# lyd405121/ti-raytrace

Measured on AMD Instinct MI355X. Metric: Mrays/s (primary+secondary) at 1024² 100k-tri, 1/2/4/8 GPU + HBM GB/s, higher is better.
Workload: dtype f32

## Files before the change

ti_raytrace_amd/csrc/tirt_api.hip:

```cpp
#include "tirt_internal.h"
#include "tirt_spectral.h"
#include <stddef.h>
#include <algorithm>
#include <mutex>
#include <string.h>

namespace tirt {

static thread_local std::string g_error;
void set_error(const std::string &msg) { g_error = msg; }

SceneView scene_view(const tirt_ctx *c)
{
    SceneView s;
    s.vertex = c->vertex.as<float>(); s.primitive = c->primitive.as<int>(); s.material = c->material.as<float>();
    s.shape = c->shape.as<float>(); s.light = c->light.as<int>(); s.env = c->env.as<int>();
    s.mat_lrgb = c->mat_lrgb.as<float>(); s.shade_rec = c->shade_rec.as<float4>(); s.light_rec = c->light_rec.as<float4>();
    s.tex = c->tex_count > 0 ? c->tex.as<int>() : nullptr;
    s.n = c->n; s.light_count = c->light_count; s.env_w = c->env_w; s.env_h = c->env_h; s.env_power = c->env_power;
    return s;
}
BvhView bvh_view(const tirt_ctx *c)
{
    BvhView b;
// ... 314 lines not shown
        float suc; v3 r = refract_(V(a[0], a[1], a[2]), V(a[3], a[4], a[5]), a[6], suc); o[0] = r.x; o[1] = r.y; o[2] = r.z; o[3] = suc;
    } else if (which == 12) {
        o[0] = schlick(a[0], a[1]);
    } else if (which == 13) {
        o[0] = gtr2(a[0], a[1]);
    } else if (which == 14) {
        o[0] = smithg_ggx(a[0], a[1]);
    } else if (which == 15) {
        o[0] = schlick_fresnel(a[0]);
    } else if (which == 16) {
        float fb; v3 r = glass_sample_lambda(V(a[0], a[1], a[2]), V(a[3], a[4], a[5]), a[6], a[7], fb); o[0] = r.x; o[1] = r.y; o[2] = r.z; o[3] = fb;
    } else if (which == 17) {
        CameraView cv; for (int k = 0; k < 12; k++) cv.view_inv[k] = a[k];
        cv.eye[0] = cv.eye[1] = cv.eye[2] = 0.0f; cv.fx = a[16]; cv.fy = a[17]; cv.cx = a[18]; cv.cy = a[19];
        v3 r = camera_ray_direction(cv, (int)a[20], (int)a[21], a[22], a[23]); o[0] = r.x; o[1] = r.y; o[2] = r.z;
    } else if (which == 18) {
        const RayCtx r = make_ray(V(a[0], a[1], a[2]), V(a[3], a[4], a[5])); float tn;
        const int full = slabs(r, a[6], a[7], a[8], a[9], a[10], a[11], tn);
        o[0] = (float)full;
        o[1] = ray_has_parallel_axis(r) ? (float)full : (float)slabs_fast(r, a[6], a[7], a[8], a[9], a[10], a[11], tn);
    }
}

__global__ void k_kat_shade_tables(SceneView s, int which, float *out, int n)
{
    const int i = blockIdx.x * blockDim.x + threadIdx.x;
    if (i >= n) return;
    if (which == 0) {
        float *o = out + (size_t)i * 4;
        v3 g = V(0.0f, 0.0f, 0.0f);
        if (s.primitive[(size_t)i * PRI_VEC] == PRIMITIVE_TRI) g = hit_attributes(s, g, V(0.0f, 0.0f, 1.0f), i, 1.0f, 0.25f, 0.25f).gnor;
        o[0] = g.x; o[1] = g.y; o[2] = g.z; o[3] = get_prim_area(s, i);
    } else {
        float *o = out + (size_t)i * 5;
        const int light_prim = s.light[i];
        const float *lm = s.material + (size_t)s.primitive[(size_t)light_prim * PRI_VEC + 2] * MAT_VEC;
        const float light_area = get_prim_area(s, light_prim);
        float light_choice_pdf = 1.0f / ((float)s.light_count * light_area);
        (void)light_shape_visible(s, light_prim, V(0.0f, 0.0f, 1.0f), V(0.0f, 0.0f, 1.0f), 1.0f, light_choice_pdf);
        o[0] = light_area; o[1] = light_choice_pdf; o[2] = lm[2]; o[3] = lm[3]; o[4] = lm[4];
    }
}
TD void kat_nee_store(float *o, v3 pos, v3 nor, v3 em, float area, float pdf, float dist)
{ o[0] = pos.x; o[1] = pos.y; o[2] = pos.z; o[3] = nor.x; o[4] = nor.y; o[5] = nor.z; o[6] = em.x; o[7] = em.y; o[8] = em.z; o[9] = area; o[10] = pdf; o[11] = dist; }
__global__ void k_kat_light_sample(SceneView s, const float *in, float *out, int n)
{
    const int i = blockIdx.x * blockDim.x + threadIdx.x;
    if (i >= n) return;
    const float *a = in + (size_t)i * 6;
    float *o = out + (size_t)i * 24;
    int lidx = (int)(a[0] * (float)s.light_count);
    if (lidx >= s.light_count) lidx = s.light_count - 1;
    if (lidx < 0) lidx = 0;
    const v3 p = V(a[3], a[4], a[5]);
    {
        const int light_prim = s.light[lidx];
        v3 light_pos, light_normal;
        get_prim_random_point_normal(s, light_prim, a[1], a[2], light_pos, light_normal);
        const float *lm = s.material + (size_t)s.primitive[(size_t)light_prim * PRI_VEC + 2] * MAT_VEC;
        const float light_area = get_prim_area(s, light_prim);
        float light_choice_pdf = 1.0f / ((float)s.light_count * light_area);
        light_normal = normalized(light_normal);
        v3 light_dir = p - light_pos;
        const float light_dist = norm(light_dir);
        light_dir = light_dir / light_dist;
        const v3 em = V(lm[2], lm[3], lm[4]) * light_shape_visible(s, light_prim, light_dir, light_normal, light_dist, light_choice_pdf);
        kat_nee_store(o, light_pos, light_normal, em, light_area, light_choice_pdf, light_dist);
    }
    {
        v3 light_pos, light_normal;
        const LightRec lr = light_sample_rec(s.light_rec, lidx, a[1], a[2], light_pos, light_normal);
        light_normal = normalized(light_normal);
        v3 light_dir = p - light_pos;
        const float light_dist = norm(light_dir);
        light_dir = light_dir / light_dist;
        const v3 em = lr.emission * light_shape_visible_rec(lr, light_dir, light_normal, light_dist);
        kat_nee_store(o + 12, light_pos, light_normal, em, lr.area, lr.choice_pdf, light_dist);
    }
}

TD uint32_t mg_mix(uint32_t x) { x ^= x >> 16; x *= 0x7feb352du; x ^= x >> 15; x *= 0x846ca68bu; x ^= x >> 16; return x; }
__global__ __launch_bounds__(256) void k_micro_gather(const float4 *rec, uint32_t nrec, int iters, float *out)
{
    uint32_t s = mg_mix(blockIdx.x * 256 + threadIdx.x + 1);
    float acc = 0.0f;
    for (int it = 0; it < iters; it++) {
        s = mg_mix(s + it);
        const uint32_t idx = (uint32_t)(((unsigned long long)s * nrec) >> 32);
        const float4 *p = rec + (size_t)idx * 4;
        const float4 a = p[0], b = p[1], c = p[2], d = p[3];
        acc += a.x + b.y + c.z + d.w;
    }
    out[blockIdx.x * 256 + threadIdx.x] = acc;
}

static int upload(DevBuf &b, const void *src, size_t bytes, hipStream_t st)
{
    if (b.ensure(bytes)) return TIRT_ERR_HIP;
    if (bytes) TIRT_HIP(hipMemcpyAsync(b.p, src, bytes, hipMemcpyHostToDevice, st));
    return 0;
}

static void drain_render_events(tirt_ctx *c)
{
    for (auto &pr : c->ev_pool) {
        float ms = 0.0f;
        if (hipEventElapsedTime(&ms, pr.first, pr.second) == hipSuccess) c->ms_render += ms;
        (void)hipEventDestroy(pr.first); (void)hipEventDestroy(pr.second);
    }
    c->ev_pool.clear();
}

__global__ void k_kat_texture(const int *tex, const float *in, int in_stride, float *out, int out_stride, int n)
{
    const int i = blockIdx.x * blockDim.x + threadIdx.x;
    if (i >= n) return;
    const float *a = in + (size_t)i * in_stride;
    float *o = out + (size_t)i * out_stride;
    const v3 c = tex_albedo(tex, __float_as_int(a[0]), a[1], a[2]);
    const v3 l = srgb_to_lrgb(c);
    o[0] = c.x; o[1] = c.y; o[2] = c.z; o[3] = l.x; o[4] = l.y; o[5] = l.z;
}

__global__ void k_kat_material_maps(SceneView sc, const float *in, int in_stride, float *out, int out_stride, int n)
{
    const int i = blockIdx.x * blockDim.x + threadIdx.x;
    if (i >= n) return;
    const float *a = in + (size_t)i * in_stride;
    float *o = out + (size_t)i * out_stride;
    const int prim = __float_as_int(a[0]);
    const int *pr = sc.primitive + (size_t)prim * PRI_VEC;
    const float *m = sc.material + (size_t)pr[2] * MAT_VEC;
    v3 uv = V(0.0f, 0.0f, 0.0f), N = uv;
    if (pr[0] == PRIMITIVE_TRI) {
        const int vi = pr[1];
        const float u = a[1], v = a[2], ba = 1.0f - u - v;
        uv = (vtx_uv(sc, vi) * ba + vtx_uv(sc, vi + 1) * u) + vtx_uv(sc, vi + 2) * v;
        N = normalized((vtx_nor(sc, vi) * ba + vtx_nor(sc, vi + 1) * u) + vtx_nor(sc, vi + 2) * v);
    }
    float rough = m[6], metal = m[5];
    const int ri = material_map(m, 7), mi = material_map(m, 8);
    if (ri >= 0) rough = tex_roughness(sc.tex, ri, uv.x, uv.y);
    if (mi >= 0) metal = tex_metallic(sc.tex, mi, uv.x, uv.y);
    const v3 Np = shading_normal_rows(sc, m, prim, uv, N);
    o[0] = uv.x; o[1] = uv.y; o[2] = rough; o[3] = metal; o[4] = Np.x; o[5] = Np.y; o[6] = Np.z; o[7] = 0.0f;
}

}

using namespace tirt;

extern "C" {

const char *tirt_last_error(void) { return g_error.c_str(); }
int tirt_version(void) { return 101; }

int tirt_device_count(int *out)
{
    TIRT_REQUIRE(out, "tirt_device_count: null out");
    TIRT_HIP(hipGetDeviceCount(out));
    return TIRT_OK;
}

int tirt_create(int device_id, tirt_ctx **out)
{
    TIRT_REQUIRE(out, "tirt_create: null out");
    int ndev = 0;
    TIRT_HIP(hipGetDeviceCount(&ndev));
    if (device_id < 0 || device_id >= ndev) { set_error("tirt_create: device " + std::to_string(device_id) + " of " + std::to_string(ndev)); return TIRT_ERR_ARG; }
    TIRT_HIP(hipSetDevice(device_id));
    tirt_ctx *c = new tirt_ctx();
    c->device = device_id;
    TIRT_HIP(hipStreamCreateWithFlags(&c->stream, hipStreamNonBlocking));
    TIRT_HIP(hipEventCreate(&c->ev0));
    TIRT_HIP(hipEventCreate(&c->ev1));
    TIRT_HIP(hipEventCreateWithFlags(&c->ev_main, hipEventDisableTiming));
    for (Lane &L : c->lanes) {
        TIRT_HIP(hipStreamCreateWithFlags(&L.stream, hipStreamNonBlocking));
        TIRT_HIP(hipEventCreateWithFlags(&L.film_done, hipEventDisableTiming));
        TIRT_HIP(hipEventCreateWithFlags(&L.aov_done, hipEventDisableTiming));
    }
    memset(&c->cam, 0, sizeof(c->cam));
    int optin = 0;
    if (hipDeviceGetAttribute(&optin, hipDeviceAttributeSharedMemPerBlockOptin, device_id) == hipSuccess && optin > 0) c->lds_optin = (size_t)optin;
    else { (void)hipGetLastError(); if (hipDeviceGetAttribute(&optin, hipDeviceAttributeMaxSharedMemoryPerBlock, device_id) == hipSuccess && optin > 0) c->lds_optin = (size_t)optin; }
    int cus = 0;
    if (hipDeviceGetAttribute(&cus, hipDeviceAttributeMultiprocessorCount, device_id) == hipSuccess && cus > 0) {
        const int g = 5 * cus < 2048 ? 5 * cus : 2048;
        c->tr_grid = g; c->tr_grid_alone = g; c->cu_count = cus;
    } else (void)hipGetLastError();
    *out = c;
    return TIRT_OK;
}

void tirt_destroy(tirt_ctx *c)
{
    if (!c) return;
    if (c->comm) { tirt_ctx *one[1] = {c}; (void)tirt_comm_destroy(one, 1); }
    (void)hipSetDevice(c->device);
    (void)sync_all(c);
    drain_render_events(c);
    DevBuf *bufs[] = {&c->vertex, &c->primitive, &c->material, &c->shape, &c->light, &c->env, &c->tex, &c->mat_lrgb, &c->shade_rec, &c->light_rec, &c->morton_unsorted, &c->keys_a,
                      &c->keys_b, &c->vals_a, &c->vals_b, &c->hist, &c->morton_sorted, &c->bvh_node, &c->compact, &c->parent,
                      &c->flag, &c->subtree, &c->build_status, &c->leaf_compact, &c->wnode, &c->tri, &c->prim_slot, &c->cnode, &c->cparent, &c->csize, &c->wide_queue, &c->wide_levels, &c->sah_compact, &c->sah_csize, &c->sah_parent, &c->wide_dp, &c->sah_box, &c->sah_idx, &c->sah_tasks, &c->sah_counts, &c->hdr, &c->rgb, &c->aov, &c->mom, &c->mom_cnt, &c->pixset, &c->pixset_tmp, &c->tp_mem, &c->mv_rec, &c->mv_snap, &c->dn_mem, &c->dn_out,
                      &c->counters_mem, &c->spill, &c->trace_stage, &c->debug_mem, &c->query_mem, &c->dyn_mem, &c->dev_counters, &c->bdpt_px, &c->timeline, &c->pvb_set[0].count, &c->pvb_set[0].cand, &c->pvb_set[0].bound, &c->pvb_set[1].count, &c->pvb_set[1].cand, &c->pvb_set[1].bound, &c->pvb_stat, &c->pvb_tmp};
    for (DevBuf *b : bufs) b->release();
    for (auto &bl : c->bd) {
        DevBuf *bb[] = {&bl.items, &bl.state, &bl.rays, &bl.hits, &bl.qidx, &bl.ctr, &bl.rad};
        for (DevBuf *b : bb) b->release();
        if (bl.delta_done) (void)hipEventDestroy(bl.delta_done);
        if (bl.film_done) (void)hipEventDestroy(bl.film_done);
    }
    for (Lane &L : c->lanes) {
        DevBuf *lb[] = {&L.path_mem, &L.counters_mem, &L.spill};
        for (DevBuf *b : lb) b->release();
        if (L.film_done) (void)hipEventDestroy(L.film_done);
        if (L.aov_done) (void)hipEventDestroy(L.aov_done);
        if (L.stream) (void)hipStreamDestroy(L.stream);
    }
    c->spec_mem.release(); c->spec_dev.release();
    if (c->spec_view) { delete (SpecView *)c->spec_view; c->spec_view = nullptr; }
    if (c->ev_main) (void)hipEventDestroy(c->ev_main);
    if (c->query_ev_in) (void)hipEventDestroy(c->query_ev_in);
    if (c->query_ev_out) (void)hipEventDestroy(c->query_ev_out);
    (void)hipEventDestroy(c->ev0); (void)hipEventDestroy(c->ev1);
    (void)hipStreamDestroy(c->stream);
    delete c;
}

#define AFTER_RENDER(c)                                                            \
    do { if ((c)->last_film) TIRT_HIP(hipStreamWaitEvent((c)->stream, (c)->last_film, 0)); } while (0)

#define AFTER_AOV(c)                                                               \
    do { if ((c)->last_aov) TIRT_HIP(hipStreamWaitEvent((c)->stream, (c)->last_aov, 0)); } while (0)

#define CTX_NOFLUSH(c)                                                             \
    TIRT_REQUIRE(c, "null context");                                               \
    TIRT_HIP(hipSetDevice((c)->device))
#define CTX(c)                                                                     \
    CTX_NOFLUSH(c);                                                                \
    do { if (int rc__ = flush_pending(c)) return rc__; } while (0)

int tirt_sync(tirt_ctx *c)
{
    CTX(c);
    if (sync_all(c)) return TIRT_ERR_HIP;
    TIRT_HIP(hipGetLastError());
    return TIRT_OK;
}

int tirt_set_option(tirt_ctx *c, const char *name, double value)
{
    CTX(c);
    TIRT_REQUIRE(name, "tirt_set_option: null name");
    if (!strcmp(name, "time_kernels")) { c->time_kernels = value != 0.0; return TIRT_OK; }
    if (!strcmp(name, "overlap_lanes")) { TIRT_REQUIRE(value >= 1.0 && value <= (double)TIRT_MAX_LANES, "overlap_lanes: 1..8"); if (sync_all(c)) return TIRT_ERR_HIP; c->n_lanes = (int)value; return TIRT_OK; }
#ifndef TIRT_EXPERIMENTS
    if (!strcmp(name, "wide_collapse")) {
        TIRT_REQUIRE(value == 0.0, "this option is an experiment (cost-optimal wide collapse): build with -DTIRT_EXPERIMENTS (make experiments)");
        return TIRT_OK;
    }
#endif
    if (!strcmp(name, "split_lone_batch")) { TIRT_REQUIRE(value >= 0.0 && value <= 8.0, "split_lone_batch: 0 (off) or the number of parts, 2..8"); c->split_lone = (int)value; return TIRT_OK; }
    if (!strcmp(name, "wide_collapse")) { TIRT_REQUIRE(value == 0.0 || value == 1.0, "wide_collapse: 0 (greedy) or 1 (cost-optimal)"); c->wide_dp_on = (int)value; return TIRT_OK; }
    if (!strcmp(name, "traversal_tree")) {
        TIRT_REQUIRE(value == 0.0 || value == 1.0, "traversal_tree: 0 (the reference's LBVH) or 1 (binned SAH)");
        c->use_sah = (int)value; return TIRT_OK;
    }
    if (!strcmp(name, "plan_batches")) { TIRT_REQUIRE(value >= 0.0 && value <= 64.0, "plan_batches: 0 (automatic) .. 64"); if (flush_pending(c)) return TIRT_ERR_HIP; c->plan_nb = (int)value; return TIRT_OK; }
    if (!strcmp(name, "plan_lanes")) { TIRT_REQUIRE(value >= 0.0 && value <= TIRT_MAX_LANES, "plan_lanes: 0 (automatic) .. the lane count"); if (flush_pending(c)) return TIRT_ERR_HIP; c->plan_lanes = (int)value; return TIRT_OK; }
    if (!strcmp(name, "job_frames")) { TIRT_REQUIRE(value >= 0.0 && value <= 1.0e9, "job_frames out of range"); c->job_frames = (long)value; return TIRT_OK; }
    if (!strcmp(name, "merge_paths")) { TIRT_REQUIRE(value >= 0.0 && value <= 1.0e9, "merge_paths out of range"); c->merge_paths = (size_t)value; c->merge_user = true; return TIRT_OK; }
    if (!strcmp(name, "batch_paths")) {
        TIRT_REQUIRE(value >= 1.0 && value <= 1.0e9, "tirt_set_option: batch_paths out of range");
        c->batch_paths = (size_t)value; c->batch_user = true; return TIRT_OK;
    }
    if (!strcmp(name, "trace_lds_depth")) {
        TIRT_REQUIRE(value >= 12 && value <= 64, "trace_lds_depth: 12..64");
        TIRT_REQUIRE(trace_lds_bytes((int)value) <= c->lds_optin, "trace_lds_depth: stacks + tree top exceed the LDS a block can have on this device");
        c->tr_lds_depth = (int)value; return TIRT_OK;
    }
    if (!strcmp(name, "bdpt_stack_size")) { TIRT_REQUIRE(value >= 16 && value <= 4096, "bdpt_stack_size: 16..4096"); c->bdpt_stack = (int)value; return TIRT_OK; }
    if (!strcmp(name, "trace_timeline")) { c->timeline_arm = (int)value; c->timeline_waves = 0; return TIRT_OK; }
    if (!strcmp(name, "trace_refill_min")) { TIRT_REQUIRE(value >= 1 && value <= 64, "trace_refill_min: 1..64"); c->tr_refill_min = (int)value; return TIRT_OK; }
    if (!strcmp(name, "trace_node_min")) { TIRT_REQUIRE(value >= 1 && value <= 64, "trace_node_min: 1..64"); c->tr_node_min = (int)value; return TIRT_OK; }
    if (!strcmp(name, "bdpt_bounded")) { c->bdpt_bounded = value != 0.0 ? 1 : 0; return TIRT_OK; }
    if (!strcmp(name, "bdpt_state_fill")) { TIRT_REQUIRE(value == 0.0 || value == 1.0 || value == 2.0, "bdpt_state_fill: 0 (none), 1 (zeros) or 2 (poison)"); c->bdpt_state_fill = (int)value; return TIRT_OK; }
    if (!strcmp(name, "primary_beams")) { TIRT_REQUIRE(value == 0.0 || value == 1.0, "primary_beams: 0 or 1"); if (flush_pending(c)) return TIRT_ERR_HIP; c->primary_beams = (int)value; return TIRT_OK; }
    if (!strcmp(name, "primary_beams_rebuild")) { if (flush_pending(c)) return TIRT_ERR_HIP; c->pvb_valid = false; return TIRT_OK; }
    if (!strcmp(name, "primary_beams_diag")) { if (flush_pending(c)) return TIRT_ERR_HIP; c->pvb_diag = value != 0.0; return TIRT_OK; }
    if (!strcmp(name, "primary_beams_min_frames")) { TIRT_REQUIRE(value >= 1.0 && value <= 1.0e6, "primary_beams_min_frames out of range"); if (flush_pending(c)) return TIRT_ERR_HIP; c->primary_beams_min_frames = (int)value; return TIRT_OK; }
    if (!strcmp(name, "bdpt_lanes")) { TIRT_REQUIRE(value >= 1.0 && value <= 4.0, "bdpt_lanes: 1..4"); if (sync_all(c)) return TIRT_ERR_HIP; c->bdpt_lanes = (int)value; return TIRT_OK; }
    if (!strcmp(name, "bdpt_batch_items")) { TIRT_REQUIRE(value >= 1.0 && value <= 1.0e9, "bdpt_batch_items out of range"); c->bdpt_batch_items = (size_t)value; return TIRT_OK; }
    if (!strcmp(name, "bdpt_mem_budget")) { TIRT_REQUIRE(value >= 0, "bdpt_mem_budget: bytes >= 0"); c->bdpt_mem_budget = (size_t)value; return TIRT_OK; }
    if (!strcmp(name, "trace_slices")) {
        const int iv = (int)value;
        TIRT_REQUIRE(iv >= 1 && iv <= 64 && (iv & (iv - 1)) == 0, "trace_slices: power of two, 1..64");
        int l = 0; while ((1 << l) < iv) l++;
        c->tr_slice_log2 = l; return TIRT_OK;
    }
    if (!strcmp(name, "shade_specialize")) { TIRT_REQUIRE(value == 0.0 || value == 1.0, "shade_specialize: 0 (generic kernel) or 1"); if (flush_pending(c)) return TIRT_ERR_HIP; c->shade_specialize = (int)value; return TIRT_OK; }
    if (!strcmp(name, "shade_grid")) { TIRT_REQUIRE(value >= 1 && value <= 65536, "shade_grid: 1..65536"); c->sh_grid = (int)value; c->grid_user = true; return TIRT_OK; }
    if (!strcmp(name, "path_order_blocks")) { c->path_order_blocks = value != 0.0; return TIRT_OK; }
    if (!strcmp(name, "slices_contiguous")) { c->slices_contiguous = value != 0.0; return TIRT_OK; }
    if (!strcmp(name, "trace_grid_alone")) { TIRT_REQUIRE(value >= 1 && value <= 16384, "trace_grid_alone: 1..16384"); c->tr_grid_alone = (int)value; return TIRT_OK; }
    if (!strcmp(name, "query_chunk_rays")) {
        TIRT_REQUIRE(value >= 256.0 && value <= (double)(1 << 27), "query_chunk_rays: 256 .. 2^27");
        c->query_chunk = (size_t)value; return TIRT_OK;
    }
    if (!strcmp(name, "trace_grid")) { TIRT_REQUIRE(value >= 1 && value <= 16384, "trace_grid: 1..16384"); c->tr_grid = (int)value; c->grid_user = true; return TIRT_OK; }
    set_error(std::string("tirt_set_option: unknown option ") + name);
    return TIRT_ERR_ARG;
}

int tirt_scene_upload(tirt_ctx *c, const float *vertex, int nv, const int32_t *primitive, int n, const float *material, int nm,
                      const float *shape, int ns, const int32_t *light, int nl, int light_count, const float bmin[3], const float bmax[3])
{
    CTX(c);
    if (sync_all(c)) return TIRT_ERR_HIP;
    TIRT_REQUIRE(n >= 1 && nv >= 0 && nm >= 1 && ns >= 1 && nl >= 1, "tirt_scene_upload: need n,nm,ns,nl >= 1");
    TIRT_REQUIRE(vertex && primitive && material && shape && light && bmin && bmax, "tirt_scene_upload: null pointer");
    TIRT_REQUIRE(light_count >= 0 && light_count <= nl, "tirt_scene_upload: light_count out of range");
    TIRT_REQUIRE((long long)2 * n - 1 < (1ll << 24), "tirt_scene_upload: node indices are stored as f32 (exact below 2^24 nodes)");
    for (int i = 0; i < n; i++) {
        const int32_t *pr = primitive + (size_t)i * 3;
        if (pr[0] == PRIMITIVE_TRI) { TIRT_REQUIRE(pr[1] >= 0 && pr[1] + 2 < nv, "tirt_scene_upload: vertex index out of range"); }
        else { TIRT_REQUIRE(pr[1] >= 0 && pr[1] < ns, "tirt_scene_upload: shape index out of range"); }
        TIRT_REQUIRE(pr[2] >= 0 && pr[2] < nm, "tirt_scene_upload: material index out of range");
    }
    for (int i = 0; i < nl; i++) TIRT_REQUIRE(light[i] >= 0 && light[i] < n, "tirt_scene_upload: light index out of range");
    if (int rc = check_material_textures("tirt_scene_upload", material, nm, c->tex_count)) return rc;
    c->sphere_prims.clear(); c->sphere_geom.clear();
    for (int i = 0; i < n; i++) {
        const int32_t *pr = primitive + (size_t)i * 3;
        if (pr[0] != PRIMITIVE_TRI && (int)shape[(size_t)pr[1] * 10] == SHAPE_SPHERE) {
            c->sphere_prims.push_back(i);
            for (int k = 1; k <= 4; k++) c->sphere_geom.push_back(shape[(size_t)pr[1] * 10 + k]);
        }
    }
    hipStream_t st = c->stream;
    c->built = false;
    c->tp_valid = false; c->mv_moved = false;
    if (upload(c->vertex, vertex, sizeof(float) * 9 * (size_t)nv, st)) return TIRT_ERR_HIP;
    if (upload(c->primitive, primitive, sizeof(int) * 3 * (size_t)n, st)) return TIRT_ERR_HIP;
    if (upload(c->material, material, sizeof(float) * 10 * (size_t)nm, st)) return TIRT_ERR_HIP;
    if (upload(c->shape, shape, sizeof(float) * 10 * (size_t)ns, st)) return TIRT_ERR_HIP;
    if (upload(c->light, light, sizeof(int) * (size_t)nl, st)) return TIRT_ERR_HIP;
    c->nv = nv; c->n = n; c->nm = nm; c->ns = ns; c->nl = nl; c->light_count = light_count; c->shade_rec_valid = false; c->light_rec_valid = false;
    for (int k = 0; k < 3; k++) { c->bmin[k] = bmin[k]; c->bmax[k] = bmax[k]; }
    if (refresh_material_table(c)) return TIRT_ERR_HIP;
    if (!c->env.p) {
        int32_t z = 0;
        if (upload(c->env, &z, sizeof(int32_t), st)) return TIRT_ERR_HIP;
        c->env_w = 1; c->env_h = 1; c->env_power = 0.0f; c->env_lit = false;
    }
    c->h_material.assign(material, material + (size_t)MAT_VEC * nm);
    light_kinds(primitive, shape, light, light_count, c->h_light_kind);
    refresh_shade_features(c);
    TIRT_HIP(hipStreamSynchronize(st));
    return TIRT_OK;
}

int tirt_material_upload(tirt_ctx *c, const float *material, int nm)
{
    CTX(c);
    if (sync_all(c)) return TIRT_ERR_HIP;
    TIRT_REQUIRE(material && nm == c->nm, "tirt_material_upload: material count differs from the uploaded scene");
    if (int rc = check_material_textures("tirt_material_upload", material, nm, c->tex_count)) return rc;
    if (upload(c->material, material, sizeof(float) * 10 * (size_t)nm, c->stream)) return TIRT_ERR_HIP;
    if (refresh_material_table(c)) return TIRT_ERR_HIP;
    c->light_rec_valid = false;
    c->shade_rec_valid = false;
    c->h_material.assign(material, material + (size_t)MAT_VEC * nm);
    refresh_shade_features(c);
    TIRT_HIP(hipStreamSynchronize(c->stream));
    return TIRT_OK;
}

int tirt_env_upload(tirt_ctx *c, const int32_t *rgb_packed, int w, int h, float power)
{
    CTX(c);
    if (sync_all(c)) return TIRT_ERR_HIP;
    TIRT_REQUIRE(rgb_packed && w >= 1 && h >= 1, "tirt_env_upload: bad image");
    if (upload(c->env, rgb_packed, sizeof(int32_t) * (size_t)w * h, c->stream)) return TIRT_ERR_HIP;
    c->env_w = w; c->env_h = h; c->env_power = power;
    c->env_lit = env_is_lit(rgb_packed, (size_t)w * h, power);
    refresh_shade_features(c);
    TIRT_HIP(hipStreamSynchronize(c->stream));
    return TIRT_OK;
}

int tirt_texture_upload(tirt_ctx *c, int count, const int32_t *texels, int64_t total, const int64_t *offset, const int32_t *w, const int32_t *h, const int32_t *wrap)
{
    TIRT_REQUIRE(count >= 0 && count <= (1 << 20), "tirt_texture_upload: count outside 0 .. 2^20");
    TIRT_REQUIRE(count == 0 || (texels && offset && w && h && wrap), "tirt_texture_upload: null pointer");
    TIRT_REQUIRE(total >= 0 && total < ((int64_t)1 << 31) - 4 * (int64_t)count, "tirt_texture_upload: total outside 0 .. 2^31 - 4 * count (texels are indexed by int)");
    std::vector<std::pair<int64_t, int64_t>> span((size_t)count);
    for (int i = 0; i < count; i++) {
        const std::string t = "tirt_texture_upload: texture " + std::to_string(i);
        TIRT_REQUIRE(w[i] >= 1 && h[i] >= 1, t + ": w and h must be >= 1");
        TIRT_REQUIRE(wrap[i] == 0 || wrap[i] == 1, t + ": wrap is 0 (clamp) or 1 (repeat)");
        const int64_t sz = (int64_t)w[i] * h[i];
        TIRT_REQUIRE(offset[i] >= 0 && offset[i] <= total && sz <= total - offset[i], t + ": its texels run past `total`");
        span[(size_t)i] = {offset[i], offset[i] + sz};
    }
    std::sort(span.begin(), span.end());
    for (int i = 1; i < count; i++) TIRT_REQUIRE(span[(size_t)i].first >= span[(size_t)i - 1].second, "tirt_texture_upload: two textures overlap");
    CTX(c);
    if (sync_all(c)) return TIRT_ERR_HIP;
    if (!c->h_material.empty())
        if (int rc = check_material_textures("tirt_texture_upload", c->h_material.data(), c->nm, count)) return rc;
    if (count > 0) {
        std::vector<int32_t> table(4 * (size_t)count);
        for (int i = 0; i < count; i++) {
            table[4 * (size_t)i] = (int32_t)(4 * (int64_t)count + offset[i]); table[4 * (size_t)i + 1] = w[i];
            table[4 * (size_t)i + 2] = h[i]; table[4 * (size_t)i + 3] = wrap[i];
        }
        const size_t tb = sizeof(int32_t) * table.size(), xb = sizeof(int32_t) * (size_t)total;
        if (c->tex.ensure(tb + xb)) return TIRT_ERR_HIP;
        TIRT_HIP(hipMemcpyAsync(c->tex.p, table.data(), tb, hipMemcpyHostToDevice, c->stream));
        if (xb) TIRT_HIP(hipMemcpyAsync((char *)c->tex.p + tb, texels, xb, hipMemcpyHostToDevice, c->stream));
        TIRT_HIP(hipStreamSynchronize(c->stream));
    } else c->tex.release();
    c->tex_count = count;
    c->shade_rec_valid = false;
    refresh_shade_features(c);
    return TIRT_OK;
}

int tirt_kat_texture(tirt_ctx *c, const float *in, int in_stride, float *out, int out_stride, int n)
{
    TIRT_REQUIRE(in && out && n >= 0, "tirt_kat_texture: null pointer or negative n");
    TIRT_REQUIRE(in_stride >= 3 && out_stride >= 6, "tirt_kat_texture: stride too small (3 words in, 6 out)");
    CTX(c);
    TIRT_REQUIRE(c->tex_count > 0, "tirt_kat_texture: no textures uploaded (tirt_texture_upload)");
    for (int i = 0; i < n; i++) {
        const int32_t id = ((const int32_t *)in)[(size_t)i * in_stride];
        TIRT_REQUIRE(id >= 0 && id < c->tex_count, "tirt_kat_texture: row " + std::to_string(i) + ": texture number outside [0, count)");
    }
    if (n == 0) return TIRT_OK;
    DevBuf din, dout;
    int rc = TIRT_OK;
    if (upload(din, in, sizeof(float) * (size_t)n * in_stride, c->stream) || dout.ensure(sizeof(float) * (size_t)n * out_stride)) rc = TIRT_ERR_HIP;
    if (rc == TIRT_OK) {
        hipError_t e = hipMemsetAsync(dout.p, 0, sizeof(float) * (size_t)n * out_stride, c->stream);
        if (e == hipSuccess) {
            hipLaunchKernelGGL(k_kat_texture, dim3((n + 255) / 256), dim3(256), 0, c->stream, c->tex.as<int>(), din.as<float>(), in_stride, dout.as<float>(), out_stride, n);
            e = hipMemcpyAsync(out, dout.p, sizeof(float) * (size_t)n * out_stride, hipMemcpyDeviceToHost, c->stream);
        }
        if (e == hipSuccess) e = hipStreamSynchronize(c->stream);
        if (e != hipSuccess) { set_error(std::string("tirt_kat_texture: ") + hipGetErrorString(e)); rc = TIRT_ERR_HIP; }
    }
    din.release(); dout.release();
    return rc;
}

int tirt_kat_material_maps(tirt_ctx *c, const float *in, int in_stride, float *out, int out_stride, int n)
{
    TIRT_REQUIRE(in && out && n >= 0, "tirt_kat_material_maps: null pointer or negative n");
    TIRT_REQUIRE(in_stride >= 3 && out_stride >= 8, "tirt_kat_material_maps: stride too small (3 words in, 8 out)");
    CTX(c);
    TIRT_REQUIRE(c->n >= 1, "tirt_kat_material_maps: no scene");
    TIRT_REQUIRE(c->tex_count > 0, "tirt_kat_material_maps: no textures uploaded (tirt_texture_upload)");
    for (int i = 0; i < n; i++) {
        const int32_t prim = ((const int32_t *)in)[(size_t)i * in_stride];
        TIRT_REQUIRE(prim >= 0 && prim < c->n, "tirt_kat_material_maps: row " + std::to_string(i) + ": prim outside [0, n_prims)");
    }
    if (n == 0) return TIRT_OK;
    if (sync_all(c)) return TIRT_ERR_HIP;
    DevBuf din, dout;
    int rc = TIRT_OK;
    if (upload(din, in, sizeof(float) * (size_t)n * in_stride, c->stream) || dout.ensure(sizeof(float) * (size_t)n * out_stride)) rc = TIRT_ERR_HIP;
    if (rc == TIRT_OK) {
        hipError_t e = hipMemsetAsync(dout.p, 0, sizeof(float) * (size_t)n * out_stride, c->stream);
        if (e == hipSuccess) {
            hipLaunchKernelGGL(k_kat_material_maps, dim3((n + 255) / 256), dim3(256), 0, c->stream, scene_view(c), din.as<float>(), in_stride, dout.as<float>(), out_stride, n);
            e = hipMemcpyAsync(out, dout.p, sizeof(float) * (size_t)n * out_stride, hipMemcpyDeviceToHost, c->stream);
        }
        if (e == hipSuccess) e = hipStreamSynchronize(c->stream);
        if (e != hipSuccess) { set_error(std::string("tirt_kat_material_maps: ") + hipGetErrorString(e)); rc = TIRT_ERR_HIP; }
    }
    din.release(); dout.release();
    return rc;
}

int tirt_shade_features(tirt_ctx *c, uint32_t *out)
{
    TIRT_REQUIRE(c, "null context");
    TIRT_REQUIRE(out, "tirt_shade_features: null pointer");
    out[0] = c->shade_features;
    out[1] = c->shade_specialize ? 1u : 0u;
    return TIRT_OK;
}

int tirt_shade_features_host(const float *material, int nm, const int32_t *primitive, int n, const float *shape, int ns,
                             const int32_t *light, int light_count, const int32_t *env, int env_w, int env_h, float env_power, uint32_t *out)
{
    TIRT_REQUIRE(material && primitive && shape && out && nm >= 1 && n >= 1 && ns >= 1, "tirt_shade_features_host: null pointer or empty table");
    TIRT_REQUIRE(light_count >= 0 && (light_count == 0 || light), "tirt_shade_features_host: bad light list");
    for (int i = 0; i < light_count; i++) {
        TIRT_REQUIRE(light[i] >= 0 && light[i] < n, "tirt_shade_features_host: light index out of range");
        const int32_t *pr = primitive + (size_t)light[i] * 3;
        TIRT_REQUIRE(pr[0] == PRIMITIVE_TRI || (pr[1] >= 0 && pr[1] < ns), "tirt_shade_features_host: shape index out of range");
    }
    std::vector<int> kind;
    light_kinds(primitive, shape, light, light_count, kind);
    const bool lit = env ? env_is_lit(env, (size_t)(env_w > 0 ? env_w : 0) * (size_t)(env_h > 0 ? env_h : 0), env_power) : env_power != 0.0f;
    *out = shade_features_core(material, nm, kind.data(), light_count, lit);
    return TIRT_OK;
}

int tirt_lbvh_build(tirt_ctx *c)
{
    CTX(c);
    if (sync_all(c)) return TIRT_ERR_HIP;
    return lbvh_build(c);
}

#ifdef TIRT_EXPERIMENTS
int tirt_exp_download(tirt_ctx *c, int which, void *out, uint64_t bytes)
{
    CTX(c);
    if (sync_all(c)) return TIRT_ERR_HIP;
    DevBuf *b = which == 0 ? &c->tri : which == 1 ? &c->prim_slot : which == 2 ? &c->leaf_compact : which == 3 ? &c->cnode : which == 5 ? &c->bd[0].qidx : &c->cparent;
    TIRT_REQUIRE(bytes <= b->bytes, "tirt_exp_download: too many bytes");
    TIRT_HIP(hipMemcpy(out, b->p, bytes, hipMemcpyDeviceToHost));
    return TIRT_OK;
}
int tirt_exp_wide_from_tree(tirt_ctx *c, const float *compact_host, const int32_t *csize_host)
{
    CTX(c);
    TIRT_REQUIRE(c->built && c->n >= 2, "tirt_exp_wide_from_tree: LBVH not built");
    if (sync_all(c)) return TIRT_ERR_HIP;
    return exp_wide_from_tree(c, compact_host, csize_host);
}
#endif

int tirt_lbvh_download(tirt_ctx *c, int32_t *morton_sorted, float *bvh_node, float *compact_node)
{
    CTX(c);
    TIRT_REQUIRE(c->built, "tirt_lbvh_download: LBVH not built");
    const size_t n = c->n, N = 2 * n - 1;
    if (morton_sorted) TIRT_HIP(hipMemcpyAsync(morton_sorted, c->morton_sorted.p, sizeof(int) * 2 * n, hipMemcpyDeviceToHost, c->stream));
    if (bvh_node) TIRT_HIP(hipMemcpyAsync(bvh_node, c->bvh_node.p, sizeof(float) * NOD_VEC * N, hipMemcpyDeviceToHost, c->stream));
    if (compact_node) TIRT_HIP(hipMemcpyAsync(compact_node, c->compact.p, sizeof(float) * CPN_VEC * N, hipMemcpyDeviceToHost, c->stream));
    TIRT_HIP(hipStreamSynchronize(c->stream));
    return TIRT_OK;
}

int tirt_traversal_tree_download(tirt_ctx *c, float *rows)
{
    CTX(c);
    TIRT_REQUIRE(c->built && rows, "tirt_traversal_tree_download: LBVH not built / null pointer");
    const size_t N = 2 * (size_t)c->n - 1;
    const bool sah = c->built_sah != 0;
    TIRT_HIP(hipMemcpyAsync(rows, sah ? c->sah_compact.p : c->compact.p, sizeof(float) * N * CPN_VEC, hipMemcpyDeviceToHost, c->stream));
    TIRT_HIP(hipStreamSynchronize(c->stream));
    return TIRT_OK;
}

int tirt_wide_tree_download(tirt_ctx *c, uint32_t *cnode, float *tri, float *wnode, int32_t *prim_slot, float grid[19], int32_t info[6])
{
    CTX(c);
    TIRT_REQUIRE(c->built && grid && info, "tirt_wide_tree_download: LBVH not built / null pointer");
    const size_t n = c->n, N = 2 * n - 1, nodes = (size_t)c->wide_nodes + (size_t)c->n_far_nodes;
    if (cnode && nodes) TIRT_HIP(hipMemcpyAsync(cnode, c->cnode.p, 64 * nodes, hipMemcpyDeviceToHost, c->stream));
    if (tri) TIRT_HIP(hipMemcpyAsync(tri, c->tri.p, sizeof(float4) * TRI_STRIDE * n, hipMemcpyDeviceToHost, c->stream));
    if (wnode) TIRT_HIP(hipMemcpyAsync(wnode, c->wnode.p, sizeof(float4) * 4 * N, hipMemcpyDeviceToHost, c->stream));
    if (prim_slot) TIRT_HIP(hipMemcpyAsync(prim_slot, c->prim_slot.p, sizeof(int) * n, hipMemcpyDeviceToHost, c->stream));
    TIRT_HIP(hipStreamSynchronize(c->stream));
    const BvhView b = bvh_view(c);
    for (int k = 0; k < 3; k++) {
        grid[k] = b.grid_min[k]; grid[3 + k] = b.cell[k]; grid[6 + k] = b.inv_cell[k]; grid[9 + k] = b.inv_extent[k];
        grid[12 + k] = b.root_min[k]; grid[15 + k] = b.root_max[k];
    }
    grid[18] = c->wide_pad;
    info[0] = c->wide_nodes; info[1] = c->n_far_nodes; info[2] = b.root_code; info[3] = b.far_qcode; info[4] = c->built_sah; info[5] = c->shapes_boxed;
    return TIRT_OK;
}

int tirt_morton_download(tirt_ctx *c, int32_t *out)
{
    CTX(c);
    TIRT_REQUIRE(c->built && out, "tirt_morton_download: LBVH not built");
    TIRT_HIP(hipMemcpyAsync(out, c->morton_unsorted.p, sizeof(int) * 2 * (size_t)c->n, hipMemcpyDeviceToHost, c->stream));
    TIRT_HIP(hipStreamSynchronize(c->stream));
    return TIRT_OK;
}

int tirt_process_normal(tirt_ctx *c, const int32_t *vertex_index)
{
    CTX(c);
    if (sync_all(c)) return TIRT_ERR_HIP;
    TIRT_REQUIRE(c->built && vertex_index, "tirt_process_normal: LBVH not built");
    if (c->nv == 0) return TIRT_OK;
    for (int i = 0; i < c->nv; i++) TIRT_REQUIRE(vertex_index[i] >= 0 && vertex_index[i] < c->n, "tirt_process_normal: vertex_index out of range");
    DevBuf vi, smooth;
    if (upload(vi, vertex_index, sizeof(int) * (size_t)c->nv, c->stream)) return TIRT_ERR_HIP;
    if (smooth.ensure(sizeof(float) * 3 * (size_t)c->nv)) { vi.release(); return TIRT_ERR_HIP; }
    const int B = 128, G = (c->nv + B - 1) / B;
    hipLaunchKernelGGL(k_smooth_normal, dim3(G), dim3(B), 0, c->stream, scene_view(c), c->nv, c->compact.as<float>(), vi.as<int>(), smooth.as<float>());
    hipLaunchKernelGGL(k_write_normal, dim3(G), dim3(B), 0, c->stream, c->vertex.as<float>(), c->nv, smooth.as<float>());
    c->shade_rec_valid = false; c->light_rec_valid = false;
    hipError_t e = hipStreamSynchronize(c->stream);
    vi.release(); smooth.release();
    TIRT_HIP(e);
// ... 606 lines not shown
```

ti_raytrace_amd/csrc/tirt_internal.h:

```cpp
#pragma once
#include <hip/hip_runtime.h>
#include <stdint.h>
#include <stdio.h>
#include <string>
#include <vector>
#include "../../include/tirt.h"
#include "tirt_device.h"

namespace tirt {

void set_error(const std::string &msg);

#define TIRT_HIP(call)                                                                          \
    do {                                                                                        \
        hipError_t e__ = (call);                                                                \
        if (e__ != hipSuccess) {                                                                \
            tirt::set_error(std::string(#call) + ": " + hipGetErrorString(e__));                \
            return TIRT_ERR_HIP;                                                                \
        }                                                                                       \
    } while (0)

#define TIRT_REQUIRE(cond, msg)                                                                 \
    do {                                                                                        \
        if (!(cond)) { tirt::set_error(msg); return TIRT_ERR_ARG; }                             \
    } while (0)

struct DevBuf {
    void *p = nullptr; size_t bytes = 0;
    int ensure(size_t want)
    {
        if (want <= bytes && p) return 0;
        if (p) (void)hipFree(p);
        p = nullptr; bytes = 0;
        if (want == 0) want = 16;
        hipError_t e = hipMalloc(&p, want);
        if (e != hipSuccess) { set_error(std::string("hipMalloc: ") + hipGetErrorString(e)); p = nullptr; return TIRT_ERR_HIP; }
        bytes = want;
        return 0;
    }
    void release() { if (p) (void)hipFree(p); p = nullptr; bytes = 0; }
    template <class T> T *as() const { return (T *)p; }
};

#ifndef TRI_STRIDE_N
#define TRI_STRIDE_N 3
#endif
constexpr int TRI_STRIDE = TRI_STRIDE_N;
constexpr int TR_EMPTY = (int)0x80000001;
#ifndef TR_TOP_LEVELS_N
#define TR_TOP_LEVELS_N 5
#endif
constexpr int TR_TOP_LEVELS = TR_TOP_LEVELS_N;
#ifndef TR_TOP_CAP
#define TR_TOP_CAP 224
#endif
constexpr int TR_TOP_FULL = ((1 << (2 * TR_TOP_LEVELS)) - 1) / 3;
constexpr int TR_TOP_SLOTS = TR_TOP_FULL < TR_TOP_CAP ? TR_TOP_FULL : TR_TOP_CAP;
constexpr float TR_GRID_HALF = 30000.0f;
constexpr unsigned TR_H_POS = 0x7b53u, TR_H_NEG = 0xfb53u;
#ifndef TR_BLOCK_SIZE
#define TR_BLOCK_SIZE 256
#endif
constexpr int TR_BLOCK = TR_BLOCK_SIZE;
constexpr int TIRT_MAX_DEVICES = 64;
#ifdef TR_PADG
constexpr size_t TR_LADDER_LDS = 4 * TR_BLOCK;
#else
constexpr size_t TR_LADDER_LDS = 0;
#endif
inline size_t trace_lds_bytes(int depth) { return sizeof(int) * (size_t)depth * TR_BLOCK + (size_t)TR_TOP_SLOTS * 64 + TR_LADDER_LDS; }
struct BvhView {
    const float4 *wnode;
    const float4 *tri;
    const uint4 *cnode;
    int top_count;
    const float *compact;
    const int *cparent;
    float grid_min[3], cell[3], inv_cell[3], inv_extent[3];
    float root_min[3], root_max[3];
    int root_code;
    int root_qcode;
    int far_qcode;
};

constexpr float TR_FAR_RHO = 8.0f;
constexpr float TR_MARGIN_CELLS = 0.25f, TR_MARGIN_PER_RHO = 0.25f, TR_MARGIN_BEAM_EXTRA = 0.05f;
TD float trace_origin_rho(const BvhView &b, float ox, float oy, float oz)
{ return maxf(maxf(absf(b.grid_min[0] - ox) * b.inv_extent[0], absf(b.grid_min[1] - oy) * b.inv_extent[1]), absf(b.grid_min[2] - oz) * b.inv_extent[2]); }
TD float trace_margin_cells(float rho) { return TR_MARGIN_CELLS + TR_MARGIN_PER_RHO * rho; }

template <bool VERIFY>
TD bool trace_leaf_step(const BvhView &b, const RayCtx &r, const bool par, const int code, float &hit_t, float &hit_u, float &hit_v, int &hit_prim, int &hit_leaf)
{
    const float4 *tp = b.tri + (size_t)(code & 0x3fffffff) * TRI_STRIDE;
    const float4 ta = tp[0], tb = tp[1], tc = tp[2];
    int prim = __float_as_int(tc.w);
    const v3 o = V(r.ox, r.oy, r.oz), d = V(r.dx, r.dy, r.dz);
    const bool is_tri = ((code >> 30) & 1) == 0;
    const v3 pa = V(ta.x, ta.y, ta.z), pb = V(tb.x, tb.y, tb.z), pc = V(tc.x, tc.y, tc.z);
    float t, u, v;
    bool sph = false;
    if (is_tri) {
        t = intersect_tri_packed(o, d, pa, pb - pa, pc - pa, u, v);
    } else {
        u = 0.0f; v = 0.0f; t = INF_VALUE;
        if ((int)tb.y == SHAPE_SPHERE) { const v3 oc = pa - o; sph = dot(d, oc) > 0.0f; }
    }
    if (__builtin_amdgcn_ballot_w64(sph) != 0ull) { if (sph) { float cc; t = intersect_sphere(o, d, pa, tb.x, cc); } }
    const int leaf = __float_as_int(ta.w);
    bool cand = (t > 0.0f) & ((t < hit_t) | ((t == hit_t) & (hit_leaf >= 0) & (leaf > hit_leaf)));
    if (VERIFY && cand) {
        v3 bmn, bmx;
        if (is_tri) {
            bmn = V(__builtin_fminf(__builtin_fminf(pa.x, pb.x), pc.x), __builtin_fminf(__builtin_fminf(pa.y, pb.y), pc.y), __builtin_fminf(__builtin_fminf(pa.z, pb.z), pc.z));
            bmx = V(__builtin_fmaxf(__builtin_fmaxf(pa.x, pb.x), pc.x), __builtin_fmaxf(__builtin_fmaxf(pa.y, pb.y), pc.y), __builtin_fmaxf(__builtin_fmaxf(pa.z, pb.z), pc.z));
        } else {
            bmn = V(pa.x - tb.x, pa.y - tb.x, pa.z - tb.x); bmx = V(pa.x + tb.x, pa.y + tb.x, pa.z + tb.x);
        }
        float tn_;
        const int inside = par ? slabs(r, bmn.x, bmn.y, bmn.z, bmx.x, bmx.y, bmx.z, tn_) : slabs_fast(r, bmn.x, bmn.y, bmn.z, bmx.x, bmx.y, bmx.z, tn_);
        if (!inside) {
            for (int an = b.cparent[leaf]; an >= 0; an = b.cparent[an]) {
                const float *ab = b.compact + (size_t)an * CPN_VEC + 2;
                if (!slabs(r, ab[0], ab[1], ab[2], ab[3], ab[4], ab[5], tn_)) { cand = false; break; }
            }
            prim = (int)b.compact[(size_t)leaf * CPN_VEC + 1];
        }
    }
    if (cand) { hit_t = t; hit_u = u; hit_v = v; hit_prim = prim; hit_leaf = leaf; }
    return cand;
}

struct PathSoA {
    float *ox, *oy, *oz, *dx, *dy, *dz;
    float *tr, *tg, *tb;
    float *rr, *rg, *rb;
    float *brdf_pdf; uint32_t *flags;
    int *slot;
};
struct PathState {
    PathSoA st[2];
    float4 *hit;
    float *sox, *soy, *soz, *sdx, *sdy, *sdz;
    float *scr, *scg, *scb; int *sprim;
    float *sdist;
    int *sdst;
    float *fr, *fg, *fb;
    float *scw, *fw;
};

struct TileMap { int tile_rank, tile_count, tile_size, H, blocked, F; const int *pixels; };
TD void slot_to_frame_pixel(const TileMap &m, int P, int slot, int &f, int &k)
{
    if (m.F > 0) { const int c = slot >> 6, kb = c / m.F; f = c - kb * m.F; k = (kb << 6) | (slot & 63); }
    else { f = slot / P; k = slot - f * P; }
}
TD int frame_pixel_to_slot(const TileMap &m, int P, int f, int k)
{ return m.F > 0 ? ((((k >> 6) * m.F + f) << 6) | (k & 63)) : f * P + k; }
TD int local_to_pixel(const TileMap &m, int k)
{
    int lt = k / m.tile_size, within = k - lt * m.tile_size;
    if (m.blocked) {
        const int rows = m.H >> 3;
        const int b = within >> 6, l = within & 63;
        const int bc = b / rows, bj = b - bc * rows;
        within = ((bc << 3) + (l >> 3)) * m.H + (bj << 3) + (l & 7);
    }
    return (lt * m.tile_count + m.tile_rank) * m.tile_size + within;
}

template <bool LIST> TD int mapped_pixel(const TileMap &m, int k) { if constexpr (LIST) return m.pixels[k]; else return local_to_pixel(m, k); }

struct DevCounters {
    unsigned long long rays_closest, rays_shadow, box_closest, leaf_closest, box_shadow, leaf_shadow;
    unsigned long long shaded, paths, stack_overflow;
    unsigned long long it_node, lanes_node, it_leaf, lanes_leaf, refills, it_outer;
    unsigned long long wave_ticks, drain_ticks, waves;
};

#define TIRT_MAX_LANES 8
struct Lane {
    hipStream_t stream = nullptr;
    hipEvent_t film_done = nullptr; bool film_recorded = false;
    hipEvent_t aov_done = nullptr;
    size_t path_capacity = 0;
    DevBuf path_mem, counters_mem, spill;
    PathState ps;
};

}

struct tirt_ctx {
    int device = 0;
    hipStream_t stream = nullptr;
    hipEvent_t ev0 = nullptr, ev1 = nullptr;

    int nv = 0, n = 0, nm = 0, ns = 0, nl = 0, light_count = 0;
    float bmin[3] = {0, 0, 0}, bmax[3] = {0, 0, 0};
    tirt::DevBuf vertex, primitive, material, shape, light, env, mat_lrgb, shade_rec, light_rec;
    bool shade_rec_valid = false;
    bool light_rec_valid = false;
    int env_w = 0, env_h = 0; float env_power = 0.0f;
    tirt::DevBuf tex; int tex_count = 0;
    std::vector<float> h_material; std::vector<int> h_light_kind; bool env_lit = false;
    unsigned shade_features = 127u;
    int shade_specialize = 1;

    bool built = false;
    tirt::DevBuf morton_unsorted;
    tirt::DevBuf keys_a, keys_b, vals_a, vals_b;
    tirt::DevBuf hist;
    tirt::DevBuf morton_sorted;
    tirt::DevBuf bvh_node, compact;
    tirt::DevBuf parent, flag, subtree, build_status, leaf_compact;
    tirt::DevBuf wnode, tri, prim_slot;
    tirt::DevBuf cnode, cparent, csize, wide_queue, wide_levels;
    int wide_nodes = 0;
    tirt::DevBuf sah_compact, sah_csize, sah_parent, wide_dp, sah_box, sah_idx, sah_tasks, sah_counts;
    int use_sah = 1, sah_levels = 0, built_sah = 0;
    std::vector<int> sphere_prims;
    std::vector<float> sphere_geom;
    tirt::DevBuf timeline; int timeline_arm = -1, timeline_waves = 0;
    int n_far_nodes = 0;
    int wide_dp_on = 0;
    float grid_min[3] = {0, 0, 0}, grid_cell[3] = {1, 1, 1}, grid_inv_cell[3] = {1, 1, 1}, grid_inv_extent[3] = {1, 1, 1};
    size_t lds_optin = 65536;
    float root_min[3], root_max[3]; int root_code = 0;
    float wide_pad = 0.0f; int shapes_boxed = 0;

    tirt::CameraView cam; float view[16]; bool cam_set = false;

    int W = 0, H = 0, tile_rank = 0, tile_count = 1, tile_size = 4096, tile_blocked = 0;
    long npix_local = 0;
    tirt::DevBuf hdr, rgb;
    tirt::DevBuf aov;
    hipEvent_t last_aov = nullptr;
    tirt::DevBuf mom, mom_cnt;
    tirt::DevBuf pixset, pixset_tmp; long pixset_n = -1;
    tirt::DevBuf tp_mem; int tp_cur = 0; bool tp_valid = false; tirt_temporal_camera_t tp_cam = {};
    tirt::DevBuf mv_rec, mv_snap; bool mv_moved = false, mv_rec_valid = false;
    tirt::DevBuf dn_mem, dn_out;

    tirt::Lane lanes[TIRT_MAX_LANES];
    int n_lanes = 4;
    unsigned lane_cursor = 0;
    hipEvent_t ev_main = nullptr;
    hipEvent_t last_film = nullptr;
    size_t batch_paths = (size_t)32 << 20;
    size_t merge_paths = (size_t)32 << 20;
    unsigned batches_since_sync = 0;
    int split_lone = 0;
    bool grid_user = false;
    int plan_nb = 0, plan_lanes = 0;
    bool batch_user = false, merge_user = false;
    long job_frames = 0;
    struct { bool valid = false; uint32_t begin = 0; int count = 0; uint32_t seed = 0; int max_depth = 0, stack_size = 0, flags = 0; bool spectral = false; } pend;
    int tr_lds_depth = 16, tr_refill_min = 18, tr_node_min = 38, tr_grid = 1280, tr_slice_log2 = 5, sh_grid = 1024;
    int path_order_blocks = 1, slices_contiguous = 0;
    int tr_grid_alone = 1280;
    tirt::DevBuf counters_mem, spill;
    int cu_count = 256;

    tirt::DevBuf bdpt_px;
    struct BdLane { tirt::DevBuf items, state, rays, hits, qidx, ctr, rad; hipEvent_t delta_done = nullptr, film_done = nullptr; } bd[4];
    int bdpt_lanes = 2;
    int bdpt_state_fill = 0;
    size_t bdpt_batch_items = (size_t)16 << 20;
    size_t bdpt_mem_budget = 0;
    int bdpt_stack = 64;
    int bdpt_bounded = 1;

    struct PvbKey { tirt::CameraView cam; unsigned long long build; int W, H, tile_rank, tile_count, tile_size, tile_blocked, P; } pvb_key;
    bool pvb_valid = false; int primary_beams = 1, primary_beams_min_frames = 16;
    unsigned long long build_serial = 0;
    struct PvbSet { tirt::DevBuf count, cand, bound; hipEvent_t busy = nullptr; } pvb_set[2];
    int pvb_cur = 0;
    int pvb_diag = 0;
    std::vector<std::pair<hipEvent_t, hipEvent_t>> pvb_ev;
    unsigned long long pvb_builds = 0, pvb_build_ns = 0, pvb_skipped = 0;
    tirt::DevBuf pvb_stat, pvb_tmp;

    tirt::DevBuf spec_dev;
    tirt::DevBuf spec_mem; bool spec_set = false; void *spec_view = nullptr;

    tirt::DevBuf trace_stage;
    tirt::DevBuf debug_mem;
    tirt::DevBuf query_mem; size_t query_chunk = (size_t)1 << 21;
    hipEvent_t query_ev_in = nullptr, query_ev_out = nullptr;
    tirt::DevBuf dyn_mem;

    void *comm = nullptr; int comm_rank = 0, comm_size = 0;

    tirt::DevBuf dev_counters;
    double ms_build = 0, ms_render = 0, ms_trace_closest = 0, ms_trace_shadow = 0, ms_shade = 0;
    uint64_t launches_trace_closest = 0, launches_trace_shadow = 0, launches_shade = 0;
    bool time_kernels = false;
    std::vector<std::pair<hipEvent_t, hipEvent_t>> ev_pool;
};

namespace tirt {
SceneView scene_view(const tirt_ctx *c);
BvhView bvh_view(const tirt_ctx *c);
int lbvh_build(tirt_ctx *c);
struct BatchPlan { size_t batch; int lanes; };
inline BatchPlan plan_batches(const tirt_ctx *c)
{
    BatchPlan p = {c->batch_paths, c->n_lanes};
    if (!c->batch_user && c->job_frames > 0 && c->npix_local > 0) {
        const size_t P = (size_t)c->npix_local, J = (size_t)c->job_frames * P, MAXB = (size_t)128 << 20;
        if (J >= ((size_t)24 << 20)) {
            const size_t nb_min = (J + MAXB - 1) / MAXB, L = (size_t)(c->n_lanes > 0 ? c->n_lanes : 1);
            size_t nb = nb_min <= 2 ? 2 : nb_min;
            if (c->plan_nb > 0 && (size_t)c->plan_nb >= nb_min) nb = (size_t)c->plan_nb;
            size_t frames = ((size_t)c->job_frames + nb - 1) / nb;
            p.batch = frames * P;
            p.lanes = (int)(L < 2 ? L : 2);
            if (c->plan_lanes > 0) p.lanes = (int)(L < (size_t)c->plan_lanes ? L : (size_t)c->plan_lanes);
        }
    }
    return p;
}
inline size_t effective_batch_paths(const tirt_ctx *c) { return plan_batches(c).batch; }
inline size_t effective_merge_paths(const tirt_ctx *c) { return (c->merge_user || c->merge_paths == 0) ? c->merge_paths : effective_batch_paths(c); }
int sah_build(tirt_ctx *c, const int *sorted_prims, float sphere_pad_abs);
inline float sphere_pad_abs(float diag) { const float R = 16.0f * diag; return 2.4e-7f * R * R; }
TD float sphere_pad(float r, float pad_abs) { return 1.0e-3f * r + pad_abs / (r > 1.0e-20f ? r : 1.0e-20f); }
#ifdef TIRT_EXPERIMENTS
int exp_wide_from_tree(tirt_ctx *c, const float *compact_host, const int *csize_host);
#endif
struct SpecView;
int pt_render(tirt_ctx *c, uint32_t frame_begin, int frame_count, uint32_t seed, int max_depth, int stack_size, int flags, const SpecView *spec = nullptr);
int bdpt_render(tirt_ctx *c, uint32_t frame_begin, int frame_count, uint32_t seed, bool spectral = false);
struct TraceJob {
    int lane = -1;
    int stack_size = 64;
    int flags = 0;
    bool query = false;
    const float4 *ray4 = nullptr;
    const int *ray_index = nullptr;
    const float *dx = nullptr, *dy = nullptr, *dz = nullptr;
    int count = 0; const int *count_ptr = nullptr;
    float4 *hit = nullptr;
    int2 *per_ray_counts = nullptr;
    bool count_rays = true;
    int grid_cap = 0;
};
int trace_rays(tirt_ctx *c, const TraceJob &j);
int trace_rays_prepare(tirt_ctx *c, int lane);
int debug_render(tirt_ctx *c, uint32_t frame, uint32_t seed, int mode, int stack_size, int flags);
struct DebugRays { float4 *hit; float *dx, *dy, *dz; TileMap tm; };
int debug_trace(tirt_ctx *c, uint32_t frame, uint32_t seed, int stack_size, int flags, DebugRays &r);
inline int render_pixels(const tirt_ctx *c) { return (int)(c->pixset_n >= 0 ? c->pixset_n : c->npix_local); }
inline TileMap render_tile_map(const tirt_ctx *c)
{ return TileMap{c->tile_rank, c->tile_count, c->tile_size, c->H, c->tile_blocked, 0, c->pixset_n >= 0 ? c->pixset.as<int>() : nullptr}; }
int pixel_set_upload(tirt_ctx *c, const int32_t *pixels, int64_t n);
int pixel_set_select(tirt_ctx *c, float t2, int min_samples, int max_samples, long expect_total, int64_t *count, int64_t check[2]);
int pixel_set_clear(tirt_ctx *c);
int render_adaptive(tirt_ctx *c, uint32_t frame_begin, uint32_t seed, int max_depth, int stack_size, int flags, const tirt_adaptive_t *a, tirt_adaptive_result_t *out);
int aov_launch(tirt_ctx *c, Lane &L, const TileMap &tm, int P, int F, uint32_t frame_begin);
int moments_launch(tirt_ctx *c, Lane &L, const TileMap &tm, int P, int F);
int moments_converged(tirt_ctx *c, float t2, uint64_t out[3]);
int query_closest(tirt_ctx *c, const float *rays, int64_t nr, int64_t ray_stride, int stack_size, int flags, float *out_t, int32_t *out_prim,
                  float *out_hit, int64_t hit_stride, int32_t *counts, void *stream);
int query_occluded(tirt_ctx *c, const float *rays, int64_t nr, int64_t ray_stride, const float *tmax, int64_t tmax_stride, float tmax_all,
                   int stack_size, int flags, uint8_t *out_occluded, void *stream);
int require_device_ptr(tirt_ctx *c, const void *p, const char *what);
int query_begin(tirt_ctx *c, void *stream);
int query_end(tirt_ctx *c, void *stream);
int denoise_film(tirt_ctx *c, const tirt_denoise_t *prm, bool var);
int denoise_device(tirt_ctx *c, bool var, const float *hdr, const float *aov, const float *mom, float *out, int W, int H, const tirt_denoise_t *prm, void *stream);
int denoise_into_film_buffer(tirt_ctx *c, const std::string &fn, const float *hdr, const float *aov, const float *mom, const tirt_denoise_t *prm);
int temporal_device(tirt_ctx *c, const float *hdr_c, const float *aov_c, const float *mom_c, const float *hdr_h, const float *aov_h, const float *mom_h,
                    const tirt_temporal_camera_t *cur, const tirt_temporal_camera_t *prev, float *hdr_o, float *mom_o, int W, int H,
                    const tirt_temporal_t *prm, const float *motion, void *stream);
int temporal_enable(tirt_ctx *c, int on);
int motion_enable(tirt_ctx *c, int on);
int motion_copy_out(tirt_ctx *c, const char *fn, void *dst, hipMemcpyKind kind);
int temporal_accumulate(tirt_ctx *c, const tirt_temporal_t *prm);
int temporal_copy_out(tirt_ctx *c, const char *fn, void *hdr_dst, void *mom_dst, hipMemcpyKind kind);
int temporal_denoise_var(tirt_ctx *c, const tirt_denoise_var_t *prm);
int trace_host(tirt_ctx *c, const float *rays, int nr, int stack_size, int flags, bool shadow, float *out_f, int32_t *out_prim, int32_t *counts);
int pvb_prepare(tirt_ctx *c);
void pvb_launch_cand(tirt_ctx *c, hipStream_t st, const BvhView &bv, const float *dx, const float *dy, const float *dz, const TileMap &tm, int P, int S,
                     float4 *hit, int *fb_count, int *fb_slot, float *fb_dx, float *fb_dy, float *fb_dz, DevCounters *ctr);
void pvb_launch_scatter(hipStream_t st, const int *fb_count, const int *fb_slot, const float4 *fb_hit, float4 *hit);
int ensure_counters(tirt_ctx *c);
int ensure_shade_records(tirt_ctx *c);
void refresh_shade_features(tirt_ctx *c);
int sync_all(tirt_ctx *c);
int flush_pending(tirt_ctx *c);
bool kat_shade_step_has_inst(unsigned feat);
int kat_shade_step(tirt_ctx *c, unsigned feat, const float *in, int in_stride, float *out, int out_stride, int n);
}
```

ti_raytrace_amd/csrc/tirt_math.h:

```cpp
#ifndef TIRT_MATH_H
#define TIRT_MATH_H

#include <stdint.h>

#if defined(__HIPCC__)
#define TM_HD __host__ __device__ static inline
#else
#define TM_HD static inline
#endif

TM_HD uint32_t tm_f2u(float f)  { union { float f; uint32_t u; } c; c.f = f; return c.u; }
TM_HD float    tm_u2f(uint32_t u){ union { float f; uint32_t u; } c; c.u = u; return c.f; }
TM_HD uint64_t tm_d2u(double d) { union { double d; uint64_t u; } c; c.d = d; return c.u; }
TM_HD double   tm_u2d(uint64_t u){ union { double d; uint64_t u; } c; c.u = u; return c.d; }

TM_HD float tm_nan(void) { return tm_u2f(0x7fc00000u); }

TM_HD float  tm_sqrt(float x)   { return __builtin_sqrtf(x); }
TM_HD double tm_sqrtd(double x) { return __builtin_sqrt(x); }

TM_HD double tm_pow2i(int k) { return tm_u2d((uint64_t)(k + 1023) << 52); }

TM_HD double tm_expd(double x)
{
    if (x != x) return x;
    if (x > 709.0)  return tm_u2d(0x7ff0000000000000ull);
    if (x < -745.0) return 0.0;
    double kf = x * 1.4426950408889634;
    int k = (int)(kf + (kf >= 0.0 ? 0.5 : -0.5));
    double r = (x - (double)k * 0.6931471803691238) - (double)k * 1.9082149292705877e-10;
    double p = 1.6059043836821613e-10;
    p = p * r + 2.08767569878681e-09;
    p = p * r + 2.505210838544172e-08;
    p = p * r + 2.755731922398589e-07;
    p = p * r + 2.7557319223985893e-06;
    p = p * r + 2.48015873015873e-05;
    p = p * r + 0.0001984126984126984;
    p = p * r + 0.001388888888888889;
    p = p * r + 0.008333333333333333;
    p = p * r + 0.041666666666666664;
    p = p * r + 0.16666666666666666;
    p = p * r + 0.5;
    p = p * r + 1.0;
    p = p * r + 1.0;
    if (k < -1000) return (p * tm_pow2i(k + 1000)) * tm_pow2i(-1000);
    if (k > 1000)  return (p * tm_pow2i(k - 1000)) * tm_pow2i(1000);
    return p * tm_pow2i(k);
}

TM_HD double tm_logd(double x)
{
    uint64_t u = tm_d2u(x);
    int e = (int)((u >> 52) & 0x7ff) - 1023;
    double m = tm_u2d((u & 0x000fffffffffffffull) | 0x3ff0000000000000ull);
    if (m > 1.4142135623730951) { m = m * 0.5; e = e + 1; }
    double s = (m - 1.0) / (m + 1.0);
    double s2 = s * s;
    double p = 0.05263157894736842;
    p = p * s2 + 0.058823529411764705;
    p = p * s2 + 0.06666666666666667;
    p = p * s2 + 0.07692307692307693;
    p = p * s2 + 0.09090909090909091;
    p = p * s2 + 0.1111111111111111;
    p = p * s2 + 0.14285714285714285;
    p = p * s2 + 0.2;
    p = p * s2 + 0.3333333333333333;
    p = p * s2 + 1.0;
    double lm = 2.0 * s * p;
    return ((double)e * 0.6931471803691238 + lm) + (double)e * 1.9082149292705877e-10;
}

TM_HD float tm_exp(float x) { return (float)tm_expd((double)x); }

TM_HD float tm_log(float x)
{
    if (x != x) return x;
    if (x < 0.0f) return tm_nan();
    if (x == 0.0f) return tm_u2f(0xff800000u);
    if (x > 3.4028234e38f) return x;
    return (float)tm_logd((double)x);
}

TM_HD float tm_pow(float x, float y)
{
    if (x != x || y != y) return tm_nan();
    if (y == 0.0f) return 1.0f;
    if (x == 0.0f) return (y > 0.0f) ? 0.0f : tm_u2f(0x7f800000u);
    float ax = x < 0.0f ? -x : x;
    double r;
    if (ax > 3.4028234e38f) r = (y > 0.0f) ? (double)ax : 0.0;
    else r = tm_expd((double)y * tm_logd((double)ax));
    if (x < 0.0f) {
        float ay = y < 0.0f ? -y : y;
        if (ay >= 16777216.0f) return (float)r;
        int iy = (int)ay;
        if ((float)iy != ay) return tm_nan();
        if (iy & 1) r = -r;
    }
    return (float)r;
}

TM_HD double tm_ksin(double r)
{
    double r2 = r * r;
    double p = 2.8114572543455206e-15;
    p = p * r2 + -7.647163731819816e-13;
    p = p * r2 + 1.6059043836821613e-10;
    p = p * r2 + -2.505210838544172e-08;
    p = p * r2 + 2.7557319223985893e-06;
    p = p * r2 + -0.0001984126984126984;
    p = p * r2 + 0.008333333333333333;
    p = p * r2 + -0.16666666666666666;
    return r + r * (r2 * p);
}
TM_HD double tm_kcos(double r)
{
    double r2 = r * r;
    double p = -1.5619206968586225e-16;
    p = p * r2 + 4.779477332387385e-14;
    p = p * r2 + -1.1470745597729725e-11;
    p = p * r2 + 2.08767569878681e-09;
    p = p * r2 + -2.755731922398589e-07;
    p = p * r2 + 2.48015873015873e-05;
    p = p * r2 + -0.001388888888888889;
    p = p * r2 + 0.041666666666666664;
    p = p * r2 + -0.5;
    return 1.0 + r2 * p;
}
TM_HD int tm_reduce(double x, double *r)
{
    double kf = x * 0.6366197723675814;
    int k = (int)(kf + (kf >= 0.0 ? 0.5 : -0.5));
    *r = (x - (double)k * 1.5707963267341256) - (double)k * 6.077100506506192e-11;
    return k;
}
TM_HD float tm_sin(float x)
{
    if (x != x || x > 1.0e6f || x < -1.0e6f) return tm_nan();
    double r; int q = tm_reduce((double)x, &r) & 3;
    double v = (q & 1) ? tm_kcos(r) : tm_ksin(r);
    return (float)((q & 2) ? -v : v);
}
TM_HD float tm_cos(float x)
{
    if (x != x || x > 1.0e6f || x < -1.0e6f) return tm_nan();
    double r; int q = tm_reduce((double)x, &r) & 3;
    double v = (q & 1) ? tm_ksin(r) : tm_kcos(r);
    return (float)(((q + 1) & 2) ? -v : v);
}

TM_HD float tm_tan(float x) { return tm_sin(x) / tm_cos(x); }
TM_HD void tm_sincos(float x, float *s, float *c)
{
    if (x != x || x > 1.0e6f || x < -1.0e6f) { *s = tm_nan(); *c = tm_nan(); return; }
    double r; int q = tm_reduce((double)x, &r) & 3;
    double ks = tm_ksin(r), kc = tm_kcos(r);
    double sv = (q & 1) ? kc : ks;
    double cv = (q & 1) ? ks : kc;
    *s = (float)((q & 2) ? -sv : sv);
    *c = (float)(((q + 1) & 2) ? -cv : cv);
}

TM_HD double tm_atan01(double z)
{
    int k = (int)(z * 8.0 + 0.5);
    double c = (double)k * 0.125;
    double t = (z - c) / (1.0 + z * c);
    double t2 = t * t;
    double p = 0.06666666666666667;
    p = p * t2 + -0.07692307692307693;
    p = p * t2 + 0.09090909090909091;
    p = p * t2 + -0.1111111111111111;
    p = p * t2 + 0.14285714285714285;
    p = p * t2 + -0.2;
    p = p * t2 + 0.3333333333333333;
    double at = t - t * (t2 * p);
    double base;
    switch (k) {
        case 0: base = 0.0; break;
        case 1: base = 0.12435499454676144; break;
        case 2: base = 0.24497866312686414; break;
        case 3: base = 0.35877067027057225; break;
        case 4: base = 0.4636476090008061; break;
        case 5: base = 0.5585993153435624; break;
        case 6: base = 0.6435011087932844; break;
        case 7: base = 0.7188299996216245; break;
        default: base = 0.7853981633974483; break;
    }
    return base + at;
}
TM_HD double tm_atan2d(double y, double x)
{
    double ay = y < 0.0 ? -y : y, ax = x < 0.0 ? -x : x;
    double a;
    if (ax == 0.0 && ay == 0.0) a = 0.0;
    else if (ay <= ax) a = tm_atan01(ay / ax);
    else a = 1.5707963267948966 - tm_atan01(ax / ay);
    if (x < 0.0) a = 3.141592653589793 - a;
    return y < 0.0 ? -a : a;
}
TM_HD float tm_atan2(float y, float x)
{
    if (x != x || y != y) return tm_nan();
    return (float)tm_atan2d((double)y, (double)x);
}
TM_HD float tm_acos(float x)
{
    if (x != x || x > 1.0f || x < -1.0f) return tm_nan();
    double xd = (double)x;
    return (float)tm_atan2d(tm_sqrtd((1.0 - xd) * (1.0 + xd)), xd);
}

TM_HD float tm_floor(float x)
{
    float t = (float)(int)x;
    return (t > x) ? t - 1.0f : t;
}

#define TM_DIM_JX 0
#define TM_DIM_JY 1
#define TM_DIM_BOUNCE0 2
#define TM_DIMS_PER_BOUNCE 8
#define TM_SLOT_LIGHT 0
#define TM_SLOT_GLASS 0
#define TM_SLOT_LA 1
#define TM_SLOT_LB 2
#define TM_SLOT_LOBE 3
#define TM_SLOT_R1 4
#define TM_SLOT_R2 5
#define TM_SLOT_EXT 6

TM_HD uint32_t tm_mix32(uint32_t x)
{
    x ^= x >> 16; x *= 0x7feb352du;
    x ^= x >> 15; x *= 0x846ca68bu;
    x ^= x >> 16;
    return x;
}
TM_HD uint32_t tm_rand_u32(uint32_t seed, uint32_t pixel, uint32_t frame, uint32_t dim)
{
    uint32_t h = tm_mix32(seed ^ 0x9e3779b9u);
    h = tm_mix32(h ^ pixel);
    h = tm_mix32(h + frame * 0x85ebca6bu + 0x68bc21ebu);
    h = tm_mix32(h ^ (dim * 0xc2b2ae35u + 0x02e5be93u));
    return h;
}
TM_HD float tm_rand(uint32_t seed, uint32_t pixel, uint32_t frame, uint32_t dim)
{
    return (float)(tm_rand_u32(seed, pixel, frame, dim) >> 8) * 5.9604644775390625e-08f;
}

#endif
```

ti_raytrace_amd/csrc/tirt_render.hip:

```cpp
#include "tirt_internal.h"
#include "tirt_spectral.h"

namespace tirt {

constexpr int TR_GRID_MAX = 2048;

enum { KIND_CLOSEST = 0, KIND_SHADOW_ACC = 1, KIND_MIXED = 2, KIND_QUERY = 3 };
#if !defined(TIRT_EXPERIMENTS) && (defined(TR_PAD) || defined(TR_PADG))
#error "the bound ladder (TR_PAD / TR_PADG) needs an experiments build: add -DTIRT_EXPERIMENTS"
#endif
struct TraceArgs {
    BvhView bvh;
    const float *ox, *oy, *oz, *dx, *dy, *dz;
    float eye[3];
    const int *count_ptr; int count_fixed;
    float4 *hit;
    const int *sprim, *sdst; const float *sdist, *scr, *scg, *scb; float *rr, *rg, *rb, *fr, *fg, *fb;
    const float *scw; float *rw, *fw;
    int *spill; int spill_depth;
    const float *sox, *soy, *soz, *sdx, *sdy, *sdz; const int *scount_ptr;
    int *fetch; int slice_log2;
    int slices_contig;
    int lds_depth;
    int refill_min;
    int node_min;
    DevCounters *ctr; int2 *per_ray_counts;
    unsigned long long *timeline;
    int no_ray_count;
    const float4 *ray4;
    const int *ray_index;
};

struct ShadeStep {
    bool want_next = false, want_shadow = false, shaded = false;
    v3 next_o = V(0.0f, 0.0f, 0.0f), next_d = next_o, next_thr = next_o, sh_o = next_o, sh_d = next_o, sh_c = next_o;
    float next_pdf = 0.0f, sh_dist = 0.0f; int next_spec = 0, sh_expect = -2;
};
template <unsigned FEAT, bool LIST = false>
TD void shade_path(const SceneView &sc, const TileMap &tm, int P, uint32_t frame_begin, uint32_t seed, int bounce, int last_bounce, int slot,
                   const v3 origin, const v3 direction, const float4 hrec, v3 throughout, v3 &radiance, float brdf_pdf, int perfect_spec, ShadeStep &s)
{
    int f, k; slot_to_frame_pixel(tm, P, slot, f, k);
    const uint32_t pixel = (uint32_t)mapped_pixel<LIST>(tm, k);
    const uint32_t frame = frame_begin + (uint32_t)f;
    const uint32_t dim0 = TM_DIM_BOUNCE0 + TM_DIMS_PER_BOUNCE * (uint32_t)bounce;
    const float t = hrec.x;
    if (t < INF_VALUE) {
        const int prim_id = __float_as_int(hrec.w);
        int mat_id;
        const HitAttr h = hit_attributes_rec<(FEAT & (SF_TEXTURE | SF_TEXTURE_PARAM)) != 0u>(sc.shade_rec, origin, direction, prim_id, t, hrec.y, hrec.z, mat_id);
        v3 normal = h.nor;
        if constexpr ((FEAT & SF_TEXTURE_PARAM) != 0u) {
            const int nor_id = material_map(sc.material + (size_t)mat_id * MAT_VEC, 9);
            if (nor_id >= 0) normal = tex_normal_rec(sc.tex, sc.shade_rec, nor_id, prim_id, h.tex, normal);
        }
        const v3 fnormal = normal * signf(dot(-direction, h.gnor));
        const float *m = sc.material + (size_t)mat_id * MAT_VEC;
        const v3 mat_color = V(m[2], m[3], m[4]);
        const int mat_type = (int)m[0];
        if (mat_type == MAT_LIGHT) {
            const float fCosTheta = absf(dot(direction, h.gnor));
            if (perfect_spec == 1) {
                radiance = radiance + throughout * mat_color;
            } else {
                const float area = h.area * (float)sc.light_count;
                const float light_pdf = (t * t) / (area * fCosTheta);
                radiance = radiance + (throughout * power_heuristic(brdf_pdf, light_pdf)) * mat_color;
            }
        } else {
            s.shaded = true;
            v3 reflect_color;
            const int tex_id = (FEAT & SF_TEXTURE) ? material_texture(m) : -1;
            if ((FEAT & SF_TEXTURE) && tex_id >= 0) reflect_color = srgb_to_lrgb(tex_albedo(sc.tex, tex_id, h.tex.x, h.tex.y));
            else reflect_color = V(sc.mat_lrgb[mat_id * 3], sc.mat_lrgb[mat_id * 3 + 1], sc.mat_lrgb[mat_id * 3 + 2]);
            v3 next_dir; float f_or_b = 1.0f, brdf = 1.0f;
            if ((FEAT & SF_GLASS) && mat_type == MAT_GLASS) {
                perfect_spec = 1;
                next_dir = glass_sample(m, direction, normal, tm_rand(seed, pixel, frame, dim0 + TM_SLOT_GLASS), f_or_b);
                brdf = 1.0f; brdf_pdf = 1.0f;
            } else {
                perfect_spec = 0;
                float mp[MAT_VEC];
                const float *md = m;
                if constexpr ((FEAT & SF_TEXTURE_PARAM) != 0u) {
                    for (int w = 0; w < MAT_VEC; w++) mp[w] = m[w];
                    const int metal_id = material_map(m, 8), rough_id = material_map(m, 7);
                    if (metal_id >= 0) mp[5] = tex_metallic(sc.tex, metal_id, h.tex.x, h.tex.y);
                    if (rough_id >= 0) mp[6] = tex_roughness(sc.tex, rough_id, h.tex.x, h.tex.y);
                    md = mp;
                }
                constexpr bool SHARE_SETUP = !(FEAT & SF_GLASS);
                DisneySetup ds;
                if (SHARE_SETUP) ds = disney_setup(md, fnormal, -direction);
                if (!(FEAT & SF_NO_LIGHT) || sc.light_count > 0) {
                int lidx = (int)(tm_rand(seed, pixel, frame, dim0 + TM_SLOT_LIGHT) * (float)sc.light_count);
                if (lidx >= sc.light_count) lidx = sc.light_count - 1;
                const float ra = tm_rand(seed, pixel, frame, dim0 + TM_SLOT_LA);
                const float rb = tm_rand(seed, pixel, frame, dim0 + TM_SLOT_LB);
                v3 light_pos, light_normal;
                const LightRec lr = light_sample_rec<FEAT>(sc.light_rec, lidx, ra, rb, light_pos, light_normal);
                const float light_choice_pdf = lr.choice_pdf;
                light_normal = normalized(light_normal);
                v3 light_dir = h.pos - light_pos;
                const float light_dist = norm(light_dir);
                light_dir = light_dir / light_dist;
                const v3 light_emission = lr.emission * light_shape_visible_rec<FEAT>(lr, light_dir, light_normal, light_dist);
                const float NdotL_surface = dot(fnormal, light_dir);
                const float NdotL_light = dot(light_normal, light_dir);
                if ((NdotL_surface < 0.0f) & (NdotL_light > 0.0f)) {
                    s.want_shadow = true;
                    float e_pdf;
                    const float e_brdf = SHARE_SETUP ? disney_evaluate_pdf_set(ds, fnormal, -direction, -light_dir, e_pdf)
                                                     : disney_evaluate_pdf(md, fnormal, -direction, -light_dir, e_pdf);
                    const float light_pdf = light_dist * light_dist * light_choice_pdf / NdotL_light;
                    v3 c = V(0.0f, 0.0f, 0.0f);
                    int expect = -2;
                    if (e_pdf > 0.0f) {
                        const float w = power_heuristic(light_pdf, e_pdf) / maxf(0.0001f, light_pdf);
                        c = light_emission * w;
                        c = c * throughout;
                        c = c * reflect_color;
                        c = c * e_brdf;
                        c = c * absf(NdotL_surface);
                        expect = prim_id;
                    }
                    s.sh_o = light_pos; s.sh_d = light_dir; s.sh_c = c; s.sh_expect = expect; s.sh_dist = light_dist;
                }
                }
                const float r_lobe = tm_rand(seed, pixel, frame, dim0 + TM_SLOT_LOBE), r_1 = tm_rand(seed, pixel, frame, dim0 + TM_SLOT_R1),
                            r_2 = tm_rand(seed, pixel, frame, dim0 + TM_SLOT_R2);
                next_dir = SHARE_SETUP ? disney_sample_set(ds, direction, fnormal, r_lobe, r_1, r_2) : disney_sample(md, direction, fnormal, r_lobe, r_1, r_2);
                f_or_b = 1.0f;
                brdf = SHARE_SETUP ? disney_evaluate_pdf_set(ds, fnormal, -direction, next_dir, brdf_pdf)
                                   : disney_evaluate_pdf(md, fnormal, -direction, next_dir, brdf_pdf);
                brdf *= absf(dot(normal, next_dir));
            }
            const v3 next_origin = offset_ray(h.pos, fnormal * signf(f_or_b));
            if (brdf_pdf > 0.0f) {
                bool alive = true;
                if ((FEAT & SF_GLASS) && f_or_b < 0.0f) {
                    const float extinction = m[6];
                    const float R = tm_exp(-t / extinction);
                    if (tm_rand(seed, pixel, frame, dim0 + TM_SLOT_EXT) >= R) alive = false;
                }
                if (alive) {
                    throughout = throughout * (reflect_color * (brdf / brdf_pdf));
                    s.want_next = !last_bounce;
                    s.next_o = next_origin; s.next_d = next_dir; s.next_thr = throughout;
                    s.next_pdf = brdf_pdf; s.next_spec = perfect_spec;
                }
            }
        }
    } else if ((!(FEAT & SF_ENV) || sc.env_power == 0.0f) && (direction.x - direction.x == 0.0f) && (direction.y - direction.y == 0.0f) &&
               (direction.z - direction.z == 0.0f)) {
        radiance = radiance + throughout * sc.env_power;
    } else if (!(FEAT & SF_ENV)) {
        const float dis = tm_sqrt(direction.x * direction.x + direction.z * direction.z);
        const float big = 3.4028234e38f;
        const bool e_nan = direction.x != direction.x || direction.y != direction.y || direction.z != direction.z ||
                           (absf(direction.x) > big && absf(direction.z) > big) || (absf(direction.y) > big && dis > big);
        const float e1 = e_nan ? tm_nan() : 0.0f;
        radiance = radiance + (V(e1, e1, e1) * throughout) * sc.env_power;
    } else {
        const float dis = tm_sqrt(direction.x * direction.x + direction.z * direction.z);
        const float tx = (tm_atan2(direction.z, direction.x) + PI_SCENE) / PI_SCENE / 2.0f;
        const float ty = tm_atan2(direction.y, dis) / PI_SCENE + 0.5f;
        const v3 e = srgb_to_lrgb(texture2d(sc.env, sc.env_w, sc.env_h, tx, ty));
        radiance = radiance + (e * throughout) * sc.env_power;
    }
}

constexpr int TR_FETCH_STRIDE = 32;
constexpr int TR_SLICES_MAX = 64;
constexpr int TR_FETCH_LINES = TR_SLICES_MAX + 1;
typedef float f2 __attribute__((ext_vector_type(2)));
typedef _Float16 h2v __attribute__((ext_vector_type(2)));
typedef __attribute__((address_space(3))) int lds_int;
constexpr int TR_PAGE = 8;
constexpr int TR_SENT = (int)0x80000000;

TD unsigned long long ballot64(bool p) { return __builtin_amdgcn_ballot_w64(p); }
TD bool wave_any(bool p) { return __builtin_amdgcn_ballot_w64(p) != 0ull; }

TD unsigned long long wave_sum(unsigned long long v)
{
#pragma unroll
    for (int o = 32; o > 0; o >>= 1) v += __shfl_down(v, o, 64);
    return v;
}

constexpr int TR_MIN_WAVES = 6;
typedef const __attribute__((address_space(4))) TraceArgs *cold_args_t;
#define TR_COLD(ca) cold_args_t ca = (cold_args_t)__builtin_amdgcn_kernarg_segment_ptr(); asm volatile("" : "+s"(ca))

#if defined(TR_PAD) || defined(TR_PADG)
#ifndef TR_PAD
#define TR_PAD 0
#endif
#ifndef TR_PADG
#define TR_PADG 0
#endif
#ifdef TR_PAD_LATE
#define TR_PAD_WHERE 1
#else
#define TR_PAD_WHERE 0
#endif
#ifdef TR_PAD_MAX
#define TR_PAD1(reg) asm volatile("v_max_f32 %0, %0, %0" : "+v"(reg))
#else
#define TR_PAD1(reg) asm volatile("v_fma_f32 %0, %0, 1.0, 0" : "+v"(reg))
#endif
#define TR_LADDER_PADS(where)                                                                        \
    do {                                                                                             \
        if ((where) == TR_PAD_WHERE) {                                                               \
            _Pragma("unroll") for (int p__ = 0; p__ < TR_PAD; p__++) {                               \
                switch (p__ % 9) {                                                                   \
                case 0: TR_PAD1(gAx); break; case 1: TR_PAD1(gAy); break; case 2: TR_PAD1(gAz); break;      \
                case 3: TR_PAD1(gBnx); break; case 4: TR_PAD1(gBny); break; case 5: TR_PAD1(gBnz); break;   \
                case 6: TR_PAD1(gBfx); break; case 7: TR_PAD1(gBfy); break; default: TR_PAD1(gBfz); break;  \
                }                                                                                    \
            }                                                                                        \
        }                                                                                            \
        if ((where) == 0) {                                                                          \
            _Pragma("unroll") for (int g__ = 0; g__ < TR_PADG; g__++) {                              \
                const unsigned dn__ = ((unsigned)cur + 977u * (unsigned)(g__ + 1)) & 32767u;         \
                __builtin_amdgcn_global_load_lds((const __attribute__((address_space(1))) void *)((const char *)b.cnode + (dn__ << 6)), \
                    (__attribute__((address_space(3))) void *)(size_t)(top_base + (unsigned)TR_TOP_SLOTS * 64u + (unsigned)(tid & ~63) * 4u), 4, 0, 0); \
            }                                                                                        \
        }                                                                                            \
    } while (0)
#else
#define TR_LADDER_PADS(where) do { } while (0)
#endif

template <int MODE, bool COUNT, int KIND>
__global__ __launch_bounds__(TR_BLOCK, TR_MIN_WAVES) void k_trace(TraceArgs a)
{
    extern __shared__ __attribute__((aligned(16))) int lds_stack[];
    const int TR_LDS_DEPTH = a.lds_depth;
    constexpr bool MAY_SHADOW = (KIND != KIND_CLOSEST);
    constexpr bool STASH = (MODE != TIRT_TRAVERSE_EXHAUSTIVE);
    constexpr bool BOUNDED = MAY_SHADOW && (MODE != TIRT_TRAVERSE_EXHAUSTIVE);
    const int count_c = (KIND == KIND_SHADOW_ACC || KIND == KIND_QUERY) ? 0 : (a.count_ptr ? *a.count_ptr : a.count_fixed);
    const int count_s = (KIND == KIND_CLOSEST) ? 0 : (KIND == KIND_MIXED ? *a.scount_ptr : (a.count_ptr ? *a.count_ptr : a.count_fixed));
    const int count = count_c + count_s;
    const int tid = threadIdx.x, lane = tid & 63;
    const size_t gstride = (size_t)gridDim.x * TR_BLOCK, gtid = (size_t)blockIdx.x * TR_BLOCK + tid;
    const unsigned long long lt_mask = (lane == 0) ? 0ull : (~0ull >> (64 - lane));
    const BvhView &b = a.bvh;

    bool have = false, par = false, is_sh = (KIND == KIND_SHADOW_ACC || KIND == KIND_QUERY);
    int q = 0, cur = TR_SENT, hit_prim = -1, hit_leaf = -1, expect = -3;
    int pend = 0;
    unsigned n_overflow = 0;
    float hit_t = INF_VALUE, hit_u = 0.0f, hit_v = 0.0f, cull_far = 3.0e38f, settle = -1.0f;
    float lim = INF_VALUE;
    unsigned nbox = 0, nleaf = 0;
    RayCtx r = {};
    float gAx = 0.0f, gAy = 0.0f, gAz = 0.0f, gBnx = 0.0f, gBny = 0.0f, gBnz = 0.0f, gBfx = 0.0f, gBfy = 0.0f, gBfz = 0.0f;
    int grotx = 0, groty = 0, grotz = 0;
    bool exhausted = false;
    unsigned long long tk_start = 0, tk_exh = 0;
    if (COUNT) tk_start = wall_clock64();
    const int S_LOG = a.slice_log2, S_MASK = (1 << S_LOG) - 1;
    int home = (int)((blockIdx.x * (TR_BLOCK / 64) + (tid >> 6)) & S_MASK), tried = 0;
    const int full_chunks = count >> 6;
    unsigned long long sum_box = 0, sum_leaf = 0, sum_box_s = 0, sum_leaf_s = 0, n_over = 0;
    unsigned long long d_it_node = 0, d_lanes_node = 0, d_it_leaf = 0, d_lanes_leaf = 0, d_refills = 0, d_outer = 0;

    constexpr unsigned ENTRY = TR_BLOCK * 4u;
    const unsigned sa_bottom = (unsigned)(size_t)(lds_int *)lds_stack + (unsigned)tid * 4u;
    const unsigned sa_hi = (unsigned)(TR_LDS_DEPTH - 3) * ENTRY + sa_bottom;
    unsigned sa = sa_bottom;
    int paged = 0;
#define LDS_AT(addr) (*(lds_int *)(size_t)(addr))
    LDS_AT(sa_bottom) = TR_SENT;
    const unsigned top_base = (unsigned)(size_t)(lds_int *)lds_stack + (unsigned)TR_LDS_DEPTH * ENTRY;
    typedef unsigned u4v __attribute__((ext_vector_type(4)));
    typedef __attribute__((address_space(3))) u4v lds_u4;
    if (MODE != TIRT_TRAVERSE_EXHAUSTIVE) {
        for (int k = tid; k < b.top_count * 4; k += TR_BLOCK)
        { const uint4 g = b.cnode[k]; *(lds_u4 *)(size_t)(top_base + (unsigned)k * 16u) = u4v{g.x, g.y, g.z, g.w}; }
        __syncthreads();
    }
#define TR_PAGE_OUT()                                                                                \
    do {                                                                                             \
        TR_COLD(ca);                                                                                 \
        if ((paged + 1) * TR_PAGE <= ca->spill_depth) {                                                \
            for (int k__ = 0; k__ < TR_PAGE; k__++)                                                  \
                ca->spill[(size_t)(paged * TR_PAGE + k__) * gstride + gtid] = LDS_AT(sa_bottom + (unsigned)(k__ + 1) * ENTRY); \
            for (unsigned e__ = sa_bottom + (TR_PAGE + 1) * ENTRY; e__ <= sa; e__ += ENTRY)          \
                LDS_AT(e__ - TR_PAGE * ENTRY) = LDS_AT(e__);                                         \
            sa -= TR_PAGE * ENTRY; paged++;                                                          \
        } else { n_overflow++; sa -= ENTRY; }       \
    } while (0)
#define TR_PAGE_IN()                                                                                 \
    do {                                                                                             \
        TR_COLD(ca);                                                                                 \
        paged--;                                                                                     \
        for (int k__ = 0; k__ < TR_PAGE; k__++)                                                      \
            LDS_AT(sa_bottom + (unsigned)(k__ + 1) * ENTRY) = ca->spill[(size_t)(paged * TR_PAGE + k__) * gstride + gtid]; \
        sa = sa_bottom + TR_PAGE * ENTRY;                                                            \
    } while (0)
#define TR_POP(dst) do { dst = LDS_AT(sa); sa -= ENTRY; } while (0)

    for (;;) {
        const unsigned long long idle = ballot64(!have);
        if (idle != 0ull && !exhausted && (__popcll(idle) >= a.refill_min || idle == ~0ull)) {
            TR_COLD(ca);
            int *const c_fetch = ca->fetch;
            const float *const c_ox = ca->ox, *const c_oy = ca->oy, *const c_oz = ca->oz, *const c_dx = ca->dx, *const c_dy = ca->dy, *const c_dz = ca->dz;
            const float *const c_sox = MAY_SHADOW ? ca->sox : nullptr, *const c_soy = MAY_SHADOW ? ca->soy : nullptr, *const c_soz = MAY_SHADOW ? ca->soz : nullptr;
            const float *const c_sdx = MAY_SHADOW ? ca->sdx : nullptr, *const c_sdy = MAY_SHADOW ? ca->sdy : nullptr, *const c_sdz = MAY_SHADOW ? ca->sdz : nullptr;
            const int *const c_sprim = MAY_SHADOW ? ca->sprim : nullptr; const float *const c_sdist = MAY_SHADOW ? ca->sdist : nullptr;
            const float4 *const c_ray4 = (KIND == KIND_CLOSEST || KIND == KIND_QUERY) ? ca->ray4 : nullptr;
            const int *const c_rindex = (KIND == KIND_QUERY) ? ca->ray_index : nullptr;
            const float c_gm0 = ca->bvh.grid_min[0], c_gm1 = ca->bvh.grid_min[1], c_gm2 = ca->bvh.grid_min[2];
            const float c_ie0 = ca->bvh.inv_extent[0], c_ie1 = ca->bvh.inv_extent[1], c_ie2 = ca->bvh.inv_extent[2];
            const float c_ic0 = ca->bvh.inv_cell[0], c_ic1 = ca->bvh.inv_cell[1], c_ic2 = ca->bvh.inv_cell[2];
            const float c_ce0 = ca->bvh.cell[0], c_ce1 = ca->bvh.cell[1], c_ce2 = ca->bvh.cell[2];
            const float c_rn0 = ca->bvh.root_min[0], c_rn1 = ca->bvh.root_min[1], c_rn2 = ca->bvh.root_min[2];
            const float c_rx0 = ca->bvh.root_max[0], c_rx1 = ca->bvh.root_max[1], c_rx2 = ca->bvh.root_max[2];
            const int c_root = ca->bvh.root_code, c_rootq = ca->bvh.root_qcode, c_farq = ca->bvh.far_qcode;
            asm volatile("" :: "s"(c_fetch), "s"(c_ox), "s"(c_oy), "s"(c_oz), "s"(c_dx), "s"(c_dy), "s"(c_dz), "s"(c_gm0), "s"(c_gm1), "s"(c_gm2), "s"(c_ie0), "s"(c_ie1), "s"(c_ie2),
                         "s"(c_ic0), "s"(c_ic1), "s"(c_ic2), "s"(c_ce0), "s"(c_ce1), "s"(c_ce2), "s"(c_rn0), "s"(c_rn1), "s"(c_rn2), "s"(c_rx0), "s"(c_rx1), "s"(c_rx2));
            if (MAY_SHADOW) asm volatile("" :: "s"(c_sox), "s"(c_soy), "s"(c_soz), "s"(c_sdx), "s"(c_sdy), "s"(c_sdz), "s"(c_sprim), "s"(c_sdist));
            if (KIND == KIND_CLOSEST || KIND == KIND_QUERY) asm volatile("" :: "s"(c_ray4), "s"(c_rindex));
            const unsigned long long fm = idle;
            int my = count;
            if (fm != 0ull && !exhausted) {
            const int n_idle = __popcll(fm);
            if (COUNT) d_refills++;
            const int leader = __ffsll((long long)fm) - 1;
            const bool contig = ca->slices_contig != 0;
            const int Lc__ = ((((count_c + 63) >> 6) + S_MASK) >> S_LOG) << 6, Ls__ = ((((count_s + 63) >> 6) + S_MASK) >> S_LOG) << 6;
            int lenc__ = count_c - home * Lc__; lenc__ = lenc__ < 0 ? 0 : (lenc__ > Lc__ ? Lc__ : lenc__);
            int lens__ = count_s - home * Ls__; lens__ = lens__ < 0 ? 0 : (lens__ > Ls__ ? Ls__ : lens__);
            const int len = contig ? lenc__ + lens__
                                   : (((full_chunks >> S_LOG) + (home < (full_chunks & S_MASK) ? 1 : 0)) << 6) + (home == (full_chunks & S_MASK) ? (count & 63) : 0);
            int base = 0;
            if (lane == leader) base = atomicAdd(c_fetch + home * TR_FETCH_STRIDE, n_idle);
            base = __shfl(base, leader, 64);
            const int v = base + __popcll(fm & lt_mask);
            if (contig) my = v < lenc__ ? home * Lc__ + v : (v < len ? count_c + home * Ls__ + (v - lenc__) : count);
            else my = v < len ? (((((v >> 6) << S_LOG) + home) << 6) | (v & 63)) : count;
            if (base + n_idle >= len) {
                int *const c_drained = c_fetch + TR_SLICES_MAX * TR_FETCH_STRIDE;
                if (lane == leader && base < (len > 0 ? len : 1)) atomicAdd(c_drained, 1);
                if (__hip_atomic_load(c_drained, __ATOMIC_RELAXED, __HIP_MEMORY_SCOPE_AGENT) > S_MASK) tried = S_MASK;
                home = (home + 1) & S_MASK;
                if (++tried > S_MASK) { exhausted = true; if (COUNT) tk_exh = wall_clock64(); }
            }
            }
            const bool setup_now = !have && my < count;
            if (setup_now) {
                q = my;
                if (KIND == KIND_MIXED) { is_sh = my >= count_c; if (is_sh) q = my - count_c; }
                const bool mixed_sh = (KIND == KIND_MIXED) && is_sh;
                v3 o, d; int rec_expect = -3; float rec_bound = -1.0f;
                const bool from_rec = (KIND == KIND_CLOSEST || KIND == KIND_QUERY) && c_ray4 != nullptr;
                if (from_rec) {
                    const size_t ri = (KIND == KIND_QUERY && c_rindex) ? (size_t)c_rindex[q] : (size_t)q;
                    const float4 r0 = c_ray4[2 * ri], r1 = c_ray4[2 * ri + 1];
                    o = V(r0.x, r0.y, r0.z); d = V(r0.w, r1.x, r1.y); rec_expect = __float_as_int(r1.z); rec_bound = r1.w;
                } else {
#define TR_LDS_(p) __builtin_nontemporal_load(&(p))
                    o = mixed_sh ? V(TR_LDS_(c_sox[q]), TR_LDS_(c_soy[q]), TR_LDS_(c_soz[q]))
                                 : ((KIND == KIND_CLOSEST && c_ox == nullptr) ? V(ca->eye[0], ca->eye[1], ca->eye[2]) : V(TR_LDS_(c_ox[q]), TR_LDS_(c_oy[q]), TR_LDS_(c_oz[q])));
                    d = mixed_sh ? V(TR_LDS_(c_sdx[q]), TR_LDS_(c_sdy[q]), TR_LDS_(c_sdz[q])) : V(TR_LDS_(c_dx[q]), TR_LDS_(c_dy[q]), TR_LDS_(c_dz[q]));
                }
                r = make_ray(o, d);
                par = ray_has_parallel_axis(r);
                hit_t = INF_VALUE; hit_u = 0.0f; hit_v = 0.0f; hit_prim = -1; hit_leaf = -1;
                nbox = 1; nleaf = 0; sa = sa_bottom; paged = 0; n_overflow = 0; pend = 0;
                cull_far = 3.0e38f; settle = -1.0f; expect = -3;
                float t_bound = -1.0f;
                if (MAY_SHADOW && is_sh) {
                    expect = from_rec ? rec_expect : TR_LDS_(c_sprim[q]);
                    if (BOUNDED) t_bound = from_rec ? rec_bound : TR_LDS_(c_sdist[q]);
                }
                if (MODE != TIRT_TRAVERSE_EXHAUSTIVE) {
                    const float relx__ = c_gm0 - o.x, rely__ = c_gm1 - o.y, relz__ = c_gm2 - o.z;
                    const float rho__ = maxf(maxf(absf(relx__) * c_ie0, absf(rely__) * c_ie1), absf(relz__) * c_ie2);
                    const float mc__ = trace_margin_cells(rho__);
                    if (rho__ > TR_FAR_RHO) cull_far = -3.0e38f;
#define TR_GRID_AXIS(rel, dd, idd, k, gA, gBn, gBf, grot)                                            \
                    do {                                                                             \
                        if (absf(dd) < 0.000001f) {       \
                            const float og__ = -(rel) * (k == 0 ? c_ic0 : (k == 1 ? c_ic1 : c_ic2));                               \
                            gA = 1.0e30f; gBn = (-og__ - (mc__ + 1.0f)) * 1.0e30f; gBf = (-og__ + (mc__ + 1.0f)) * 1.0e30f; grot = 0; \
                        } else {                                                                     \
                            gA = (k == 0 ? c_ce0 : (k == 1 ? c_ce1 : c_ce2)) * (idd);                                                  \
                            const float gB__ = (rel) * (idd);                                        \
                            const float m__ = mc__ * absf(gA);                                       \
                            gBn = gB__ - m__; gBf = gB__ + m__; grot = gA < 0.0f ? 16 : 0;           \
                        }                                                                            \
                    } while (0)
                    TR_GRID_AXIS(relx__, d.x, r.idx, 0, gAx, gBnx, gBfx, grotx);
                    TR_GRID_AXIS(rely__, d.y, r.idy, 1, gAy, gBny, gBfy, groty);
                    TR_GRID_AXIS(relz__, d.z, r.idz, 2, gAz, gBnz, gBfz, grotz);
                }
                if (BOUNDED && t_bound > 0.0f && cull_far > 0.0f) { cull_far = t_bound * 1.01f; settle = t_bound * 0.99f; }
                lim = __builtin_fminf(__builtin_fminf(hit_t * 1.0001f, __builtin_fabsf(cull_far)), INF_VALUE);
                cur = (MODE == TIRT_TRAVERSE_EXHAUSTIVE) ? c_root : (cull_far < 0.0f ? c_farq : c_rootq);
                if ((MODE == TIRT_TRAVERSE_EXHAUSTIVE || KIND == KIND_CLOSEST) && cur >= 0) {
                    float tn;
                    if (!slabs(r, c_rn0, c_rn1, c_rn2, c_rx0, c_rx1, c_rx2, tn)) cur = TR_SENT;
                }
                if (MODE != TIRT_TRAVERSE_EXHAUSTIVE &&
                    !((o.x == o.x) & (o.y == o.y) & (o.z == o.z) & (d.x == d.x) & (d.y == d.y) & (d.z == d.z))) cur = TR_SENT;
                have = true;
            }
        }
        if (ballot64(have) == 0ull) { if (exhausted) break; continue; }

        if (STASH) { if (have && cur < 0 && cur != TR_SENT && pend == 0) { pend = cur; TR_POP(cur); } }
        const int lim_i = __float_as_int(lim);
        constexpr int TR_NODE_FRAC = 6;
        int node_min_w = (__popcll(ballot64(have)) * TR_NODE_FRAC) >> 3; node_min_w = node_min_w < a.node_min ? node_min_w : a.node_min;
        for (;;) {
            const bool act = cur >= 0;
            const unsigned long long am = ballot64(act);
            if (am == 0ull) break;
            const int n_act = __popcll(am);
            if (n_act < node_min_w && ballot64(have && cur < 0) != 0ull) break;
            if (wave_any((int)sa >= (int)sa_hi)) break;
            if (COUNT) { d_it_node++; d_lanes_node += (unsigned long long)n_act; }
            if (act) {
                if (MODE == TIRT_TRAVERSE_EXHAUSTIVE) {
                    const float4 *w = (const float4 *)((const char *)b.wnode + ((unsigned)cur << 6));
                    const float4 q0 = w[0], q1 = w[1], q2 = w[2], q3 = w[3];
                    const int cl = __float_as_int(q3.x), cr = __float_as_int(q3.y);
                    if (COUNT) nbox += 2;
                    float tl, tr;
                    int pl, pr;
                    if (!par) {
                        pl = slabs_fast(r, q0.x, q0.y, q0.z, q0.w, q1.x, q1.y, tl);
                        pr = slabs_fast(r, q1.z, q1.w, q2.x, q2.y, q2.z, q2.w, tr);
                    } else {
                        pl = slabs(r, q0.x, q0.y, q0.z, q0.w, q1.x, q1.y, tl);
                        pr = slabs(r, q1.z, q1.w, q2.x, q2.y, q2.z, q2.w, tr);
                    }
                    const bool hl = (pl != 0) || (cl < 0), hr = (pr != 0) || (cr < 0);
                    if (hl && hr) { sa += ENTRY; LDS_AT(sa) = cr; }
                    int next = hl ? cl : cr;
                    if (!(hl || hr)) TR_POP(next);
                    cur = next;
                } else {
                    uint4 q0, q1, q2, q3;
#define TR_U4(v) make_uint4((v).x, (v).y, (v).z, (v).w)
                    const unsigned top_addr = top_base + ((unsigned)cur << 6);
                    {
                        u4v r0__, r1__, r2__, r3__;
                        unsigned long long sv__;
                        const unsigned long long topm__ = ballot64(cur < TR_TOP_SLOTS);
                        const unsigned goff__ = (unsigned)cur << 6;
                        asm volatile(
                            "s_mov_b64 %4, exec\n\t"
                            "s_and_b64 exec, %4, %8\n\t"
                            "s_cbranch_execz .Ltr_fetch_g%=\n\t"
                            "ds_read_b128 %0, %5\n\t"
                            "ds_read_b128 %1, %5 offset:16\n\t"
                            "ds_read_b128 %2, %5 offset:32\n\t"
                            "ds_read_b128 %3, %5 offset:48\n"
                            ".Ltr_fetch_g%=:\n\t"
                            "s_andn2_b64 exec, %4, %8\n\t"
                            "s_cbranch_execz .Ltr_fetch_e%=\n\t"
                            "global_load_dwordx4 %0, %6, %7\n\t"
                            "global_load_dwordx4 %1, %6, %7 offset:16\n\t"
                            "global_load_dwordx4 %2, %6, %7 offset:32\n\t"
                            "global_load_dwordx4 %3, %6, %7 offset:48\n"
                            ".Ltr_fetch_e%=:\n\t"
                            "s_mov_b64 exec, %4\n\t"
                            "s_waitcnt vmcnt(0) lgkmcnt(0)"
                            : "=&v"(r0__), "=&v"(r1__), "=&v"(r2__), "=&v"(r3__), "=&s"(sv__)
                            : "v"(top_addr), "v"(goff__), "s"(b.cnode), "s"(topm__)
                            : "memory");
                        q0 = TR_U4(r0__); q1 = TR_U4(r1__); q2 = TR_U4(r2__); q3 = TR_U4(r3__);
                        if (COUNT) { if (cur < TR_TOP_SLOTS) d_outer++; }
                    }
                    TR_LADDER_PADS(0);
                    int c0 = (int)q3.x, c1 = (int)q3.y, c2 = (int)q3.z, c3 = (int)q3.w;
                    if (COUNT) nbox += 4;
                    constexpr float MISS = 3.0e38f;
                    float d0, d1, d2, d3;
#define TR_CBOX(X, Y, Z, dist)                                                                       \
                    do {                                                                             \
                        const unsigned ux__ = __builtin_amdgcn_alignbit((X), (X), grotx);            \
                        const unsigned uy__ = __builtin_amdgcn_alignbit((Y), (Y), groty);            \
                        const unsigned uz__ = __builtin_amdgcn_alignbit((Z), (Z), grotz);            \
                        const h2v hx__ = __builtin_bit_cast(h2v, ux__), hy__ = __builtin_bit_cast(h2v, uy__), hz__ = __builtin_bit_cast(h2v, uz__); \
                        const float nx__ = __builtin_fmaf((float)hx__.x, gAx, gBnx), fx__ = __builtin_fmaf((float)hx__.y, gAx, gBfx); \
                        const float ny__ = __builtin_fmaf((float)hy__.x, gAy, gBny), fy__ = __builtin_fmaf((float)hy__.y, gAy, gBfy); \
                        const float nz__ = __builtin_fmaf((float)hz__.x, gAz, gBnz), fz__ = __builtin_fmaf((float)hz__.y, gAz, gBfz); \
                        const float tn__ = __builtin_fmaxf(__builtin_fmaxf(nx__, ny__), __builtin_fmaxf(nz__, 0.0f)); \
                              \
                        const int tfi__ = min(min(__float_as_int(fx__), __float_as_int(fy__)), min(__float_as_int(fz__), lim_i));     \
                        const float tf__ = __int_as_float(tfi__);                                    \
                        dist = (tn__ <= tf__) ? tn__ : MISS;                                         \
                    } while (0)
                    TR_CBOX(q0.x, q0.y, q0.z, d0);
                    TR_CBOX(q0.w, q1.x, q1.y, d1);
                    TR_CBOX(q1.z, q1.w, q2.x, d2);
                    TR_CBOX(q2.y, q2.z, q2.w, d3);
#define TR_CE(da, ca, db, cb)                                                                        \
                    do {                                                                             \
                        const bool s__ = (db) < (da);                                                \
                        const float lo__ = s__ ? (db) : (da), hi__ = s__ ? (da) : (db);              \
                        const int clo__ = s__ ? (cb) : (ca), chi__ = s__ ? (ca) : (cb);              \
                        da = lo__; db = hi__; ca = clo__; cb = chi__;                                \
                    } while (0)
                    TR_CE(d0, c0, d1, c1); TR_CE(d2, c2, d3, c3); TR_CE(d0, c0, d2, c2); TR_CE(d1, c1, d3, c3); TR_CE(d1, c1, d2, c2);
                    TR_LADDER_PADS(1);
                    if (d3 < MISS) { sa += ENTRY; LDS_AT(sa) = c3; }
                    if (d2 < MISS) { sa += ENTRY; LDS_AT(sa) = c2; }
                    if (d1 < MISS) { sa += ENTRY; LDS_AT(sa) = c1; }
                    int next = c0;
                    if (!(d0 < MISS)) TR_POP(next);
                    if (STASH) { if ((next < 0) & (next != TR_SENT) & (pend == 0)) { pend = next; TR_POP(next); } }
                    cur = next;
                }
            }
        }

        if (wave_any(have && (int)sa >= (int)sa_hi)) {
            if (have && (int)sa >= (int)sa_hi) TR_PAGE_OUT();
        }

        const bool from_pend = STASH && pend != 0;
        const bool leaf_now = have && (from_pend || (cur < 0 && cur != TR_SENT));
        if (COUNT) {
            const int n_l = __popcll(ballot64(leaf_now));
            if (n_l) { d_it_leaf++; d_lanes_leaf += (unsigned long long)n_l; }
        }
        if (leaf_now) {
            const int code = ~(from_pend ? pend : cur);
            if (COUNT) nleaf += 1;
            const bool accepted = trace_leaf_step<MODE != TIRT_TRAVERSE_EXHAUSTIVE>(b, r, par, code, hit_t, hit_u, hit_v, hit_prim, hit_leaf);
            if (from_pend) pend = 0; else TR_POP(cur);
            if (accepted) {
                lim = __builtin_fminf(__builtin_fminf(cull_far < 0.0f ? INF_VALUE : hit_t * 1.0001f, __builtin_fabsf(cull_far)), INF_VALUE);
                if (BOUNDED && hit_prim != expect && hit_t < settle) { cur = TR_SENT; paged = 0; pend = 0; }
            }
        }

        if (ballot64(have && cur == TR_SENT && paged > 0) != 0ull) {
            if (have && cur == TR_SENT && paged > 0) { TR_PAGE_IN(); TR_POP(cur); }
        }

        if (have && cur == TR_SENT && pend == 0) {
            TR_COLD(ca);
            float4 *const c_hit = ca->hit;
            const int *const c_sdst = MAY_SHADOW ? ca->sdst : nullptr;
            float *const c_rr = MAY_SHADOW ? ca->rr : nullptr, *const c_rg = MAY_SHADOW ? ca->rg : nullptr, *const c_rb = MAY_SHADOW ? ca->rb : nullptr;
            float *const c_fr = MAY_SHADOW ? ca->fr : nullptr, *const c_fg = MAY_SHADOW ? ca->fg : nullptr, *const c_fb = MAY_SHADOW ? ca->fb : nullptr;
            const float *const c_scr = MAY_SHADOW ? ca->scr : nullptr, *const c_scg = MAY_SHADOW ? ca->scg : nullptr, *const c_scb = MAY_SHADOW ? ca->scb : nullptr;
            const float *const c_scw = MAY_SHADOW ? ca->scw : nullptr;
            if (MAY_SHADOW) asm volatile("" :: "s"(c_hit), "s"(c_sdst), "s"(c_rr), "s"(c_rg), "s"(c_rb), "s"(c_fr), "s"(c_fg), "s"(c_fb), "s"(c_scr), "s"(c_scg), "s"(c_scb), "s"(c_scw));
            if (!(MAY_SHADOW && is_sh) || KIND == KIND_QUERY) {
                { typedef float f4n __attribute__((ext_vector_type(4))); f4n hv__ = {hit_t, hit_u, hit_v, __int_as_float(hit_prim)}; __builtin_nontemporal_store(hv__, (f4n *)&c_hit[q]); }
            } else if (hit_prim == expect) {
                const int dst = TR_LDS_(c_sdst[q]);
                float *pr = dst >= 0 ? c_rr + dst : c_fr + ~dst;
                float *pg = dst >= 0 ? c_rg + dst : c_fg + ~dst;
                float *pb = dst >= 0 ? c_rb + dst : c_fb + ~dst;
                *pr = *pr + TR_LDS_(c_scr[q]); *pg = *pg + TR_LDS_(c_scg[q]); *pb = *pb + TR_LDS_(c_scb[q]);
                if (c_scw) { float *pw = dst >= 0 ? ca->rw + dst : ca->fw + ~dst; *pw = *pw + c_scw[q]; }
            }
            if (COUNT) {
                if (MAY_SHADOW && is_sh) { sum_box_s += nbox; sum_leaf_s += nleaf; }
                else { sum_box += nbox; sum_leaf += nleaf; }
                if (ca->per_ray_counts) ca->per_ray_counts[q] = make_int2((int)nbox, (int)nleaf);
            }
            if (n_overflow) n_over++;
            have = false; sa = sa_bottom;
        }
    }
    TR_COLD(ca);
    if (ca->ctr) {
        if (COUNT) {
            sum_box = wave_sum(sum_box); sum_leaf = wave_sum(sum_leaf);
            sum_box_s = wave_sum(sum_box_s); sum_leaf_s = wave_sum(sum_leaf_s);
            if (lane == 0 && (sum_box | sum_leaf)) { atomicAdd(&ca->ctr->box_closest, sum_box); atomicAdd(&ca->ctr->leaf_closest, sum_leaf); }
            if (lane == 0 && (sum_box_s | sum_leaf_s)) { atomicAdd(&ca->ctr->box_shadow, sum_box_s); atomicAdd(&ca->ctr->leaf_shadow, sum_leaf_s); }
        }
        if (COUNT) { d_outer = wave_sum(d_outer); if (lane == 0) atomicAdd(&ca->ctr->it_outer, d_outer); }
        if (COUNT && lane == 0) {
            atomicAdd(&ca->ctr->it_node, d_it_node); atomicAdd(&ca->ctr->lanes_node, d_lanes_node);
            atomicAdd(&ca->ctr->it_leaf, d_it_leaf); atomicAdd(&ca->ctr->lanes_leaf, d_lanes_leaf);
            atomicAdd(&ca->ctr->refills, d_refills);
            const unsigned long long tk_end = wall_clock64();
            atomicAdd(&ca->ctr->wave_ticks, tk_end - tk_start); atomicAdd(&ca->ctr->drain_ticks, tk_end - (tk_exh ? tk_exh : tk_end)); atomicAdd(&ca->ctr->waves, 1ull);
            if (ca->timeline) {
                const unsigned hw = __builtin_amdgcn_s_getreg((31 << 11) | 4), xcc = __builtin_amdgcn_s_getreg((31 << 11) | 20);
                unsigned long long *rec = ca->timeline + (size_t)(gtid >> 6) * 4;
                rec[0] = tk_start; rec[1] = tk_exh; rec[2] = tk_end; rec[3] = (unsigned long long)hw | ((unsigned long long)xcc << 32);
            }
        }
        if (n_over) atomicAdd(&ca->ctr->stack_overflow, n_over);
        if (gtid == 0 && !ca->no_ray_count) {
            if (count_c) atomicAdd(&ca->ctr->rays_closest, (unsigned long long)count_c);
            if (count_s) atomicAdd(&ca->ctr->rays_shadow, (unsigned long long)count_s);
        }
    }
}

static unsigned long long *timeline_for(tirt_ctx *c, int flags, int grid)
{
    if (c->timeline_arm < 0 || !(flags & TIRT_COUNT_NODES)) return nullptr;
    if (c->timeline_arm-- != 0) return nullptr;
    c->timeline_waves = grid * (TR_BLOCK / 64);
    if (c->timeline.ensure(sizeof(unsigned long long) * 4 * (size_t)c->timeline_waves)) { c->timeline_waves = 0; return nullptr; }
    if (hipMemsetAsync(c->timeline.p, 0, sizeof(unsigned long long) * 4 * (size_t)c->timeline_waves, c->stream) != hipSuccess ||
        hipStreamSynchronize(c->stream) != hipSuccess) { (void)hipGetLastError(); c->timeline_waves = 0; return nullptr; }
    return c->timeline.as<unsigned long long>();
}

template <int MODE, bool COUNT, int KIND>
static int launch_trace_as(tirt_ctx *c, hipStream_t stream, const TraceArgs &a, dim3 g, dim3 b, size_t lds)
{
    static size_t allowed[TIRT_MAX_DEVICES] = {};
    TIRT_REQUIRE(lds <= c->lds_optin, "k_trace: trace_lds_depth needs more LDS than the device has per block");
    const int dev = (c->device >= 0 && c->device < TIRT_MAX_DEVICES) ? c->device : 0;
    if (lds > allowed[dev] || c->device >= TIRT_MAX_DEVICES) {
        TIRT_HIP(hipFuncSetAttribute(reinterpret_cast<const void *>(&k_trace<MODE, COUNT, KIND>), hipFuncAttributeMaxDynamicSharedMemorySize, (int)lds));
        allowed[dev] = lds;
    }
    hipLaunchKernelGGL((k_trace<MODE, COUNT, KIND>), g, b, lds, stream, a);
    return TIRT_OK;
}
template <int KIND>
static int launch_trace(tirt_ctx *c, hipStream_t stream, const TraceArgs &a, int flags, int grid)
{
    const bool exh = (flags & TIRT_TRAVERSE_EXHAUSTIVE) != 0, cnt = (flags & TIRT_COUNT_NODES) != 0;
    dim3 g(grid), b(TR_BLOCK);
    const size_t lds = trace_lds_bytes(a.lds_depth);
    if (exh && cnt) return launch_trace_as<TIRT_TRAVERSE_EXHAUSTIVE, true, KIND>(c, stream, a, g, b, lds);
    if (exh) return launch_trace_as<TIRT_TRAVERSE_EXHAUSTIVE, false, KIND>(c, stream, a, g, b, lds);
    if (cnt) return launch_trace_as<TIRT_TRAVERSE_ORDERED, true, KIND>(c, stream, a, g, b, lds);
    return launch_trace_as<TIRT_TRAVERSE_ORDERED, false, KIND>(c, stream, a, g, b, lds);
}

static int ensure_spill(tirt_ctx *c, DevBuf &spill, int stack_size, int &spill_depth)
{
    int cap = stack_size > 64 ? stack_size : 64;
    spill_depth = cap - (c->tr_lds_depth - 1);
    if (spill_depth < 0) spill_depth = 0;
    spill_depth = (spill_depth + TR_PAGE - 1) / TR_PAGE * TR_PAGE;
    return spill.ensure(sizeof(int) * (size_t)(spill_depth > 0 ? spill_depth : 1) * TR_GRID_MAX * TR_BLOCK);
}
static void fill_tunables(const tirt_ctx *c, TraceArgs &a)
{ a.lds_depth = c->tr_lds_depth; a.refill_min = c->tr_refill_min; a.node_min = c->tr_node_min; a.slice_log2 = c->tr_slice_log2; a.slices_contig = c->slices_contiguous; }

static int trace_buffers(tirt_ctx *c, int lane, int stack_size, TraceArgs &a)
{
    DevBuf &spill = lane < 0 ? c->spill : c->lanes[lane].spill;
    DevBuf &fetch = lane < 0 ? c->counters_mem : c->lanes[lane].counters_mem;
    if (ensure_spill(c, spill, stack_size, a.spill_depth)) return TIRT_ERR_HIP;
    if (fetch.ensure(sizeof(int) * TR_FETCH_STRIDE * TR_FETCH_LINES)) return TIRT_ERR_HIP;
    a.spill = spill.as<int>(); a.fetch = fetch.as<int>();
    return TIRT_OK;
}

int trace_rays_prepare(tirt_ctx *c, int lane)
{
    TraceArgs a = {};
    return trace_buffers(c, lane, c->bdpt_stack, a);
}

int trace_rays(tirt_ctx *c, const TraceJob &j)
{
    if (j.count <= 0) return TIRT_OK;
    hipStream_t st = j.lane < 0 ? c->stream : c->lanes[j.lane].stream;
    TraceArgs a = {};
    if (int rc = trace_buffers(c, j.lane, j.stack_size, a)) return rc;
    TIRT_HIP(hipMemsetAsync(a.fetch, 0, sizeof(int) * TR_FETCH_STRIDE * TR_FETCH_LINES, st));
    a.bvh = bvh_view(c);
    a.ray4 = j.ray4; a.ray_index = j.ray_index;
    if (!j.ray4) { a.dx = j.dx; a.dy = j.dy; a.dz = j.dz; for (int k = 0; k < 3; k++) a.eye[k] = c->cam.eye[k]; }
    a.count_ptr = j.count_ptr; a.count_fixed = j.count; a.hit = j.hit;
    a.ctr = c->dev_counters.as<DevCounters>(); a.no_ray_count = j.count_rays ? 0 : 1;
    a.per_ray_counts = (j.flags & TIRT_COUNT_NODES) ? j.per_ray_counts : nullptr;
    fill_tunables(c, a);
    int grid = (j.count + TR_BLOCK - 1) / TR_BLOCK; if (grid > j.grid_cap) grid = j.grid_cap;
    a.timeline = timeline_for(c, j.flags, grid);
    if (!j.query) return launch_trace<KIND_CLOSEST>(c, st, a, j.flags, grid);
    return launch_trace<KIND_QUERY>(c, st, a, j.flags, grid);
}

template <bool LIST>
__global__ void k_generate(PathSoA ps, CameraView cam, TileMap tm, int P, int S, uint32_t frame_begin, uint32_t seed,
                           DevCounters *ctr)
{
    int s = blockIdx.x * blockDim.x + threadIdx.x;
    if (s >= S) return;
    int f, k; slot_to_frame_pixel(tm, P, s, f, k);
    int p = mapped_pixel<LIST>(tm, k);
    int i = p / tm.H, j = p - i * tm.H;
    uint32_t frame = frame_begin + (uint32_t)f;
    float jx = 0.0f, jy = 0.0f;
    if (frame != 0) {
        jx = tm_rand(seed, (uint32_t)p, frame, TM_DIM_JX) - 0.5f;
        jy = tm_rand(seed, (uint32_t)p, frame, TM_DIM_JY) - 0.5f;
    }
    v3 d = camera_ray_direction(cam, i, j, jx, jy);
    __builtin_nontemporal_store(d.x, &ps.dx[s]); __builtin_nontemporal_store(d.y, &ps.dy[s]); __builtin_nontemporal_store(d.z, &ps.dz[s]);
    if (s == 0) atomicAdd(&ctr->paths, (unsigned long long)S);
}

#ifndef SH_BLOCK
#define SH_BLOCK 256
#endif
#ifndef SH_MIN_WAVES
#define SH_MIN_WAVES 5
#endif
#ifndef SH_MIN_WAVES_NARROW
#define SH_MIN_WAVES_NARROW 5
#endif
#ifndef SH_MIN_WAVES_MAPS
#define SH_MIN_WAVES_MAPS 4
#endif
struct ShadeArgs { PathState ps; PathSoA in, out; };
typedef const __attribute__((address_space(4))) ShadeArgs *cold_shade_t;
#define SH_COLD(ca) cold_shade_t ca = (cold_shade_t)__builtin_amdgcn_kernarg_segment_ptr(); asm volatile("" : "+s"(ca))
#define SH_LD(x) __builtin_nontemporal_load(&(x))
#define SH_ST(x, v) __builtin_nontemporal_store((v), &(x))
template <unsigned FEAT, int MIN_WAVES, bool LIST = false>
__global__ __launch_bounds__(SH_BLOCK, MIN_WAVES) void k_shade(ShadeArgs paths_in_kernarg_segment, SceneView sc, TileMap tm, int P,
                                                   uint32_t frame_begin, uint32_t seed, int bounce, int last_bounce,
                                                   const int *count_ptr, int count_fixed, unsigned long long *append_ctr,
                                                   DevCounters *ctr, v3 eye)
{
    __shared__ unsigned s_wcnt[2][SH_BLOCK / 64];
    __shared__ unsigned long long s_base[2];
    const int lane = threadIdx.x & 63, wid = threadIdx.x >> 6;
    const unsigned long long lt_mask = (lane == 0) ? 0ull : (~0ull >> (64 - lane));
    const int count = count_ptr ? *count_ptr : count_fixed;
    const int total = gridDim.x * blockDim.x;
    const int rounds = (count + total - 1) / total;
    unsigned long long n_shaded = 0;
    for (int it = 0; it < rounds; it++) {
        const int q = it * total + blockIdx.x * blockDim.x + threadIdx.x;
        bool live = q < count, want_next = false, want_shadow = false;
        int slot = 0;
        v3 radiance = V(0.0f, 0.0f, 0.0f), next_o = radiance, next_d = radiance, next_thr = radiance;
        v3 sh_o = radiance, sh_d = radiance, sh_c = radiance;
        float next_pdf = 0.0f, sh_dist = 0.0f; int next_spec = 0, sh_expect = -2;
        if (live) {
            const bool first = bounce == 0;
            SH_COLD(ca);
            const int *const c_slot = ca->in.slot; const uint32_t *const c_flags = ca->in.flags; const float4 *const c_hit = ca->ps.hit;
            const float *const c_ox = ca->in.ox, *const c_oy = ca->in.oy, *const c_oz = ca->in.oz, *const c_dx = ca->in.dx, *const c_dy = ca->in.dy, *const c_dz = ca->in.dz;
            const float *const c_tr = ca->in.tr, *const c_tg = ca->in.tg, *const c_tb = ca->in.tb, *const c_rr = ca->in.rr, *const c_rg = ca->in.rg, *const c_rb = ca->in.rb;
            const float *const c_pdf = ca->in.brdf_pdf;
            asm volatile("" :: "s"(c_slot), "s"(c_flags), "s"(c_hit), "s"(c_ox), "s"(c_oy), "s"(c_oz), "s"(c_dx), "s"(c_dy), "s"(c_dz), "s"(c_tr), "s"(c_tg), "s"(c_tb),
                         "s"(c_rr), "s"(c_rg), "s"(c_rb), "s"(c_pdf));
            slot = first ? q : SH_LD(c_slot[q]);
            const v3 origin = first ? eye : V(SH_LD(c_ox[q]), SH_LD(c_oy[q]), SH_LD(c_oz[q]));
            const v3 direction = V(SH_LD(c_dx[q]), SH_LD(c_dy[q]), SH_LD(c_dz[q]));
            typedef float f4nt__ __attribute__((ext_vector_type(4)));
            const f4nt__ hnt__ = __builtin_nontemporal_load((const f4nt__ *)&c_hit[q]);
            const float4 hrec = make_float4(hnt__.x, hnt__.y, hnt__.z, hnt__.w);
            v3 throughout = first ? V(1.0f, 1.0f, 1.0f) : V(SH_LD(c_tr[q]), SH_LD(c_tg[q]), SH_LD(c_tb[q]));
            radiance = first ? V(0.0f, 0.0f, 0.0f) : V(SH_LD(c_rr[q]), SH_LD(c_rg[q]), SH_LD(c_rb[q]));
            float brdf_pdf = first ? 1.0f : SH_LD(c_pdf[q]);
            int perfect_spec = first ? 1 : (int)(SH_LD(c_flags[q]) & 1u);
            ShadeStep ss;
            shade_path<FEAT, LIST>(sc, tm, P, frame_begin, seed, bounce, last_bounce, slot, origin, direction, hrec, throughout, radiance, brdf_pdf, perfect_spec, ss);
            want_next = ss.want_next; want_shadow = ss.want_shadow; if (ss.shaded) n_shaded++;
            next_o = ss.next_o; next_d = ss.next_d; next_thr = ss.next_thr; next_pdf = ss.next_pdf; next_spec = ss.next_spec;
            sh_o = ss.sh_o; sh_d = ss.sh_d; sh_c = ss.sh_c; sh_expect = ss.sh_expect; sh_dist = ss.sh_dist;
        }
        const int par = it & 1;
        const unsigned long long nmask = __ballot(want_next), smask = __ballot(want_shadow);
        if (lane == 0) s_wcnt[par][wid] = (unsigned)__popcll(nmask) | ((unsigned)__popcll(smask) << 16);
        __syncthreads();
        if (threadIdx.x == 0) {
            unsigned tn = 0, tsd = 0;
#pragma unroll
            for (int w = 0; w < SH_BLOCK / 64; w++) { tn += s_wcnt[par][w] & 0xffffu; tsd += s_wcnt[par][w] >> 16; }
            s_base[par] = (tn | tsd) ? atomicAdd(append_ctr, (unsigned long long)tn | ((unsigned long long)tsd << 32)) : 0ull;
        }
        __syncthreads();
        unsigned pn = 0, psd = 0;
#pragma unroll
        for (int w = 0; w < SH_BLOCK / 64; w++) if (w < wid) { pn += s_wcnt[par][w] & 0xffffu; psd += s_wcnt[par][w] >> 16; }
        const unsigned long long bb = s_base[par];
        const int qn = (int)(unsigned)(bb & 0xffffffffull) + (int)pn + __popcll(nmask & lt_mask);
        const int qs = (int)(unsigned)(bb >> 32) + (int)psd + __popcll(smask & lt_mask);
        if (want_next) {
            SH_COLD(ca);
            float *const o_ox = ca->out.ox, *const o_oy = ca->out.oy, *const o_oz = ca->out.oz, *const o_dx = ca->out.dx, *const o_dy = ca->out.dy, *const o_dz = ca->out.dz;
            float *const o_tr = ca->out.tr, *const o_tg = ca->out.tg, *const o_tb = ca->out.tb, *const o_rr = ca->out.rr, *const o_rg = ca->out.rg, *const o_rb = ca->out.rb;
            float *const o_pdf = ca->out.brdf_pdf; uint32_t *const o_flags = ca->out.flags; int *const o_slot = ca->out.slot;
            asm volatile("" :: "s"(o_ox), "s"(o_oy), "s"(o_oz), "s"(o_dx), "s"(o_dy), "s"(o_dz), "s"(o_tr), "s"(o_tg), "s"(o_tb), "s"(o_rr), "s"(o_rg), "s"(o_rb),
                         "s"(o_pdf), "s"(o_flags), "s"(o_slot));
            SH_ST(o_ox[qn], next_o.x); SH_ST(o_oy[qn], next_o.y); SH_ST(o_oz[qn], next_o.z);
            SH_ST(o_dx[qn], next_d.x); SH_ST(o_dy[qn], next_d.y); SH_ST(o_dz[qn], next_d.z);
            SH_ST(o_tr[qn], next_thr.x); SH_ST(o_tg[qn], next_thr.y); SH_ST(o_tb[qn], next_thr.z);
            SH_ST(o_rr[qn], radiance.x); SH_ST(o_rg[qn], radiance.y); SH_ST(o_rb[qn], radiance.z);
            SH_ST(o_pdf[qn], next_pdf); SH_ST(o_flags[qn], (uint32_t)next_spec); SH_ST(o_slot[qn], slot);
        } else if (live) {
            SH_COLD(ca);
            float *const f_r = ca->ps.fr, *const f_g = ca->ps.fg, *const f_b = ca->ps.fb;
            asm volatile("" :: "s"(f_r), "s"(f_g), "s"(f_b));
            SH_ST(f_r[slot], radiance.x); SH_ST(f_g[slot], radiance.y); SH_ST(f_b[slot], radiance.z);
        }
        if (want_shadow) {
            SH_COLD(ca);
            float *const s_ox = ca->ps.sox, *const s_oy = ca->ps.soy, *const s_oz = ca->ps.soz, *const s_dx = ca->ps.sdx, *const s_dy = ca->ps.sdy, *const s_dz = ca->ps.sdz;
            float *const s_cr = ca->ps.scr, *const s_cg = ca->ps.scg, *const s_cb = ca->ps.scb, *const s_dist = ca->ps.sdist;
            int *const s_prim = ca->ps.sprim, *const s_dst = ca->ps.sdst;
            asm volatile("" :: "s"(s_ox), "s"(s_oy), "s"(s_oz), "s"(s_dx), "s"(s_dy), "s"(s_dz), "s"(s_cr), "s"(s_cg), "s"(s_cb), "s"(s_dist), "s"(s_prim), "s"(s_dst));
            SH_ST(s_ox[qs], sh_o.x); SH_ST(s_oy[qs], sh_o.y); SH_ST(s_oz[qs], sh_o.z);
            SH_ST(s_dx[qs], sh_d.x); SH_ST(s_dy[qs], sh_d.y); SH_ST(s_dz[qs], sh_d.z);
            SH_ST(s_cr[qs], sh_c.x); SH_ST(s_cg[qs], sh_c.y); SH_ST(s_cb[qs], sh_c.z);
            SH_ST(s_prim[qs], sh_expect); SH_ST(s_dist[qs], sh_dist);
            SH_ST(s_dst[qs], want_next ? qn : ~slot);
        }
    }
    __shared__ unsigned long long s_shaded;
    if (threadIdx.x == 0) s_shaded = 0ull;
    __syncthreads();
    n_shaded = wave_sum(n_shaded);
    if ((threadIdx.x & 63) == 0 && n_shaded) atomicAdd(&s_shaded, n_shaded);
    __syncthreads();
    if (threadIdx.x == 0 && s_shaded) atomicAdd(&ctr->shaded, s_shaded);
}

template <bool LIST>
__global__ void k_film(PathState ps, TileMap tm, int P, int F, uint32_t frame_begin, float *hdr)
{
    int k = blockIdx.x * blockDim.x + threadIdx.x;
    if (k >= P) return;
    int p = mapped_pixel<LIST>(tm, k);
    float *px = hdr + (size_t)p * 3;
    float r = px[0], g = px[1], b = px[2];
    for (int f = 0; f < F; f++) {
        int s = frame_pixel_to_slot(tm, P, f, k);
        float frame = (float)(int)(frame_begin + (uint32_t)f);
        float coff = 1.0f / (frame + 1.0f);
        r = __builtin_nontemporal_load(&ps.fr[s]) * coff + r * (1.0f - coff);
        g = __builtin_nontemporal_load(&ps.fg[s]) * coff + g * (1.0f - coff);
        b = __builtin_nontemporal_load(&ps.fb[s]) * coff + b * (1.0f - coff);
    }
    px[0] = r; px[1] = g; px[2] = b;
}

template <unsigned FEAT>
__global__ __launch_bounds__(SH_BLOCK, 4) void k_shade_spec(ShadeArgs paths_in_kernarg_segment, SceneView sc, SpecView sp, TileMap tm, int P,
                                                   uint32_t frame_begin, uint32_t seed, int bounce, int last_bounce,
                                                   const int *count_ptr, int count_fixed, unsigned long long *append_ctr,
                                                   DevCounters *ctr, v3 eye)
{
    __shared__ unsigned s_wcnt[2][SH_BLOCK / 64];
    __shared__ unsigned long long s_base[2];
    const int lane = threadIdx.x & 63, wid = threadIdx.x >> 6;
    const unsigned long long lt_mask = (lane == 0) ? 0ull : (~0ull >> (64 - lane));
    const int count = count_ptr ? *count_ptr : count_fixed;
    const int total = gridDim.x * blockDim.x;
    const int rounds = (count + total - 1) / total;
    unsigned long long n_shaded = 0;
    for (int it = 0; it < rounds; it++) {
        const int q = it * total + blockIdx.x * blockDim.x + threadIdx.x;
        bool live = q < count, want_next = false, want_shadow = false;
        int slot = 0;
        f4s radiance = f4_set(0.0f), next_thr = radiance, sh_c = radiance;
        v3 next_o = V(0.0f, 0.0f, 0.0f), next_d = next_o, sh_o = next_o, sh_d = next_o;
        float sh_dist = 0.0f; int sh_expect = -2;
        if (live) {
            const bool first = bounce == 0;
            SH_COLD(ca);
            const int *const c_slot = ca->in.slot; const float4 *const c_hit = ca->ps.hit;
            const float *const c_ox = ca->in.ox, *const c_oy = ca->in.oy, *const c_oz = ca->in.oz, *const c_dx = ca->in.dx, *const c_dy = ca->in.dy, *const c_dz = ca->in.dz;
            const float *const c_tr = ca->in.tr, *const c_tg = ca->in.tg, *const c_tb = ca->in.tb, *const c_rr = ca->in.rr, *const c_rg = ca->in.rg, *const c_rb = ca->in.rb;
            const float *const c_tw = ca->in.brdf_pdf, *const c_rw = (const float *)ca->in.flags;
            asm volatile("" :: "s"(c_slot), "s"(c_hit), "s"(c_ox), "s"(c_oy), "s"(c_oz), "s"(c_dx), "s"(c_dy), "s"(c_dz), "s"(c_tr), "s"(c_tg), "s"(c_tb),
                         "s"(c_rr), "s"(c_rg), "s"(c_rb), "s"(c_tw), "s"(c_rw));
            slot = first ? q : c_slot[q];
            int f, k; slot_to_frame_pixel(tm, P, slot, f, k);
            const uint32_t pixel = (uint32_t)local_to_pixel(tm, k);
            const uint32_t frame = frame_begin + (uint32_t)f;
            const uint32_t dim0 = TM_DIM_BOUNCE0 + TM_DIMS_PER_BOUNCE * (uint32_t)bounce;
            const float Lambda = HERO_LAMBDA_MIN + HERO_LAMBDA_STEP * tm_rand(seed, pixel, frame, TM_DIM_SPEC_LAMBDA);
            const v3 origin = first ? eye : V(c_ox[q], c_oy[q], c_oz[q]);
            const v3 direction = V(c_dx[q], c_dy[q], c_dz[q]);
            typedef float f4nt__ __attribute__((ext_vector_type(4)));
            const f4nt__ hnt__ = __builtin_nontemporal_load((const f4nt__ *)&c_hit[q]);
            const float4 hrec = make_float4(hnt__.x, hnt__.y, hnt__.z, hnt__.w);
            const float t = hrec.x;
            f4s throughout = f4_set(1.0f);
            if (!first) {
                throughout.v[0] = c_tr[q]; throughout.v[1] = c_tg[q]; throughout.v[2] = c_tb[q]; throughout.v[3] = c_tw[q];
                radiance.v[0] = c_rr[q]; radiance.v[1] = c_rg[q]; radiance.v[2] = c_rb[q]; radiance.v[3] = c_rw[q];
            }
            const f4s light_rad = hero_sample(sp.spd[0], Lambda);
            if (t < INF_VALUE) {
                const int prim_id = __float_as_int(hrec.w);
                int mat_id;
                const HitAttr h = hit_attributes_rec(sc.shade_rec, origin, direction, prim_id, t, hrec.y, hrec.z, mat_id);
                const v3 normal = h.nor;
                const v3 fnormal = normal * signf(dot(-direction, h.gnor));
                const float *m = sc.material + (size_t)mat_id * MAT_VEC;
                const v3 mat_color = V(m[2], m[3], m[4]);
                const int mat_type = (int)m[0];
                const f4s light_tint = emission_to_rad(sp, mat_color, Lambda);
                if (mat_type == MAT_LIGHT) {
                    const float fCosTheta = dot(direction, normal);
                    if (fCosTheta < 0.0f) radiance = radiance + ((throughout * light_rad) * light_tint);
                } else {
                    n_shaded++;
                    const f4s reflect_spec = get_spec_power(sp, m, Lambda);
                    v3 next_dir; float f_or_b = 1.0f, brdf = 1.0f, brdf_pdf = 1.0f;
                    if ((FEAT & SF_GLASS) && mat_type == MAT_GLASS) {
                        const int index = (int)(tm_rand(seed, pixel, frame, dim0 + TM_SLOT_HERO) * (float)HERO_N);
                        const float rnd_lambda = Lambda + (float)index * HERO_LAMBDA_STEP;
                        next_dir = glass_sample_lambda(direction, normal, rnd_lambda, tm_rand(seed, pixel, frame, dim0 + TM_SLOT_GLASS), f_or_b);
                    } else {
                        if (!(FEAT & SF_NO_LIGHT) || sc.light_count > 0) {
                            int lidx = (int)(tm_rand(seed, pixel, frame, dim0 + TM_SLOT_LIGHT) * (float)sc.light_count);
                            if (lidx >= sc.light_count) lidx = sc.light_count - 1;
                            const float ra = tm_rand(seed, pixel, frame, dim0 + TM_SLOT_LA);
                            const float rb = tm_rand(seed, pixel, frame, dim0 + TM_SLOT_LB);
                            v3 light_pos, light_normal;
                            const LightRec lr = light_sample_rec<FEAT>(sc.light_rec, lidx, ra, rb, light_pos, light_normal);
                            const float light_choice_pdf = lr.choice_pdf;
                            light_normal = normalized(light_normal);
                            v3 light_dir = h.pos - light_pos;
                            const float light_dist = norm(light_dir);
                            light_dir = light_dir / light_dist;
                            const float NdotL_surface = dot(fnormal, light_dir);
                            const float NdotL_light = dot(light_normal, light_dir);
                            if ((NdotL_surface < 0.0f) & (NdotL_light > 0.0f)) {
                                want_shadow = true;
                                float e_pdf;
                                const float e_brdf = disney_evaluate_pdf(m, fnormal, -direction, -light_dir, e_pdf);
                                const float light_pdf = light_dist * light_dist * light_choice_pdf / NdotL_light;
                                f4s c = f4_set(0.0f);
                                int expect = -2;
                                if (e_pdf > 0.0f) {
                                    const float w = power_heuristic(light_pdf, e_pdf) / maxf(0.0001f, light_pdf);
                                    c = light_rad * w;
                                    c = c * light_tint;
                                    c = c * throughout;
                                    c = c * reflect_spec;
                                    c = c * e_brdf;
                                    c = c * absf(NdotL_surface);
                                    expect = prim_id;
                                }
                                sh_o = light_pos; sh_d = light_dir; sh_c = c; sh_expect = expect; sh_dist = light_dist;
                            }
                        }
                        next_dir = disney_sample(m, direction, fnormal, tm_rand(seed, pixel, frame, dim0 + TM_SLOT_LOBE),
                                                 tm_rand(seed, pixel, frame, dim0 + TM_SLOT_R1), tm_rand(seed, pixel, frame, dim0 + TM_SLOT_R2));
                        f_or_b = 1.0f;
                        brdf = disney_evaluate_pdf(m, fnormal, next_dir, -direction, brdf_pdf);
                        brdf *= absf(dot(normal, next_dir));
                    }
                    const v3 next_origin = offset_ray(h.pos, fnormal * signf(f_or_b));
                    if ((brdf_pdf > 0.0f) & (maxf(throughout.v[2], maxf(throughout.v[0], throughout.v[1])) > 0.0f)) {
                        throughout = throughout * ((reflect_spec * brdf) / brdf_pdf);
                        want_next = !last_bounce;
                        next_o = next_origin; next_d = next_dir; next_thr = throughout;
                    }
                }
            } else {
                const float dis = tm_sqrt(direction.x * direction.x + direction.z * direction.z);
                const float beta = tm_atan2(direction.y, dis);
                const float gamma = tm_acos(dot(direction, V(sp.sun_dir[0], sp.sun_dir[1], sp.sun_dir[2])));
                const float theta = clampf(0.5f * PI_SCENE - beta, 0.0f, 0.5f * PI_SCENE);
                f4s ibl;
                for (int w = 0; w < HERO_N; w++) ibl.v[w] = sky_radiance(sp, theta, gamma, Lambda + (float)w * HERO_LAMBDA_STEP);
                radiance = radiance + ((throughout * ibl) * light_rad);
            }
        }
        const int par = it & 1;
        const unsigned long long nmask = __ballot(want_next), smask = __ballot(want_shadow);
        if (lane == 0) s_wcnt[par][wid] = (unsigned)__popcll(nmask) | ((unsigned)__popcll(smask) << 16);
        __syncthreads();
        if (threadIdx.x == 0) {
            unsigned tn = 0, tsd = 0;
#pragma unroll
            for (int w = 0; w < SH_BLOCK / 64; w++) { tn += s_wcnt[par][w] & 0xffffu; tsd += s_wcnt[par][w] >> 16; }
            s_base[par] = (tn | tsd) ? atomicAdd(append_ctr, (unsigned long long)tn | ((unsigned long long)tsd << 32)) : 0ull;
        }
        __syncthreads();
        unsigned pn = 0, psd = 0;
#pragma unroll
        for (int w = 0; w < SH_BLOCK / 64; w++) if (w < wid) { pn += s_wcnt[par][w] & 0xffffu; psd += s_wcnt[par][w] >> 16; }
        const unsigned long long bb = s_base[par];
        const int qn = (int)(unsigned)(bb & 0xffffffffull) + (int)pn + __popcll(nmask & lt_mask);
        const int qs = (int)(unsigned)(bb >> 32) + (int)psd + __popcll(smask & lt_mask);
        if (want_next) {
            SH_COLD(ca);
            float *const o_ox = ca->out.ox, *const o_oy = ca->out.oy, *const o_oz = ca->out.oz, *const o_dx = ca->out.dx, *const o_dy = ca->out.dy, *const o_dz = ca->out.dz;
            float *const o_tr = ca->out.tr, *const o_tg = ca->out.tg, *const o_tb = ca->out.tb, *const o_rr = ca->out.rr, *const o_rg = ca->out.rg, *const o_rb = ca->out.rb;
            float *const o_tw = ca->out.brdf_pdf, *const o_rw = (float *)ca->out.flags; int *const o_slot = ca->out.slot;
            asm volatile("" :: "s"(o_ox), "s"(o_oy), "s"(o_oz), "s"(o_dx), "s"(o_dy), "s"(o_dz), "s"(o_tr), "s"(o_tg), "s"(o_tb), "s"(o_rr), "s"(o_rg), "s"(o_rb),
                         "s"(o_tw), "s"(o_rw), "s"(o_slot));
            o_ox[qn] = next_o.x; o_oy[qn] = next_o.y; o_oz[qn] = next_o.z;
            o_dx[qn] = next_d.x; o_dy[qn] = next_d.y; o_dz[qn] = next_d.z;
            o_tr[qn] = next_thr.v[0]; o_tg[qn] = next_thr.v[1]; o_tb[qn] = next_thr.v[2]; o_tw[qn] = next_thr.v[3];
            o_rr[qn] = radiance.v[0]; o_rg[qn] = radiance.v[1]; o_rb[qn] = radiance.v[2]; o_rw[qn] = radiance.v[3];
            o_slot[qn] = slot;
        } else if (live) {
            SH_COLD(ca);
            float *const f_r = ca->ps.fr, *const f_g = ca->ps.fg, *const f_b = ca->ps.fb, *const f_w = ca->ps.fw;
            asm volatile("" :: "s"(f_r), "s"(f_g), "s"(f_b), "s"(f_w));
            f_r[slot] = radiance.v[0]; f_g[slot] = radiance.v[1]; f_b[slot] = radiance.v[2]; f_w[slot] = radiance.v[3];
        }
        if (want_shadow) {
            SH_COLD(ca);
            float *const s_ox = ca->ps.sox, *const s_oy = ca->ps.soy, *const s_oz = ca->ps.soz, *const s_dx = ca->ps.sdx, *const s_dy = ca->ps.sdy, *const s_dz = ca->ps.sdz;
            float *const s_cr = ca->ps.scr, *const s_cg = ca->ps.scg, *const s_cb = ca->ps.scb, *const s_cw = ca->ps.scw, *const s_dist = ca->ps.sdist;
            int *const s_prim = ca->ps.sprim, *const s_dst = ca->ps.sdst;
            asm volatile("" :: "s"(s_ox), "s"(s_oy), "s"(s_oz), "s"(s_dx), "s"(s_dy), "s"(s_dz), "s"(s_cr), "s"(s_cg), "s"(s_cb), "s"(s_cw), "s"(s_dist), "s"(s_prim), "s"(s_dst));
            s_ox[qs] = sh_o.x; s_oy[qs] = sh_o.y; s_oz[qs] = sh_o.z;
            s_dx[qs] = sh_d.x; s_dy[qs] = sh_d.y; s_dz[qs] = sh_d.z;
            s_cr[qs] = sh_c.v[0]; s_cg[qs] = sh_c.v[1]; s_cb[qs] = sh_c.v[2]; s_cw[qs] = sh_c.v[3];
            s_prim[qs] = sh_expect; s_dist[qs] = sh_dist;
            s_dst[qs] = want_next ? qn : ~slot;
        }
    }
    __shared__ unsigned long long s_shaded;
    if (threadIdx.x == 0) s_shaded = 0ull;
    __syncthreads();
    n_shaded = wave_sum(n_shaded);
    if ((threadIdx.x & 63) == 0 && n_shaded) atomicAdd(&s_shaded, n_shaded);
    __syncthreads();
    if (threadIdx.x == 0 && s_shaded) atomicAdd(&ctr->shaded, s_shaded);
}

typedef void (*shade_fn_t)(ShadeArgs, SceneView, TileMap, int, uint32_t, uint32_t, int, int, const int *, int, unsigned long long *, DevCounters *, v3);
typedef void (*shade_spec_fn_t)(ShadeArgs, SceneView, SpecView, TileMap, int, uint32_t, uint32_t, int, int, const int *, int, unsigned long long *, DevCounters *, v3);
struct ShadeInst { unsigned feat; shade_fn_t fn, fn_list; };
struct ShadeSpecInst { unsigned feat; shade_spec_fn_t fn; };
constexpr unsigned SF_I_SPHERE = SF_LIGHT_SPHERE;
constexpr unsigned SF_I_MESH = SF_LIGHT_TRI;
constexpr unsigned SF_I_MAPS = SF_ALL | SF_TEXTURE | SF_TEXTURE_PARAM;
static const ShadeInst SHADE_INST[] = {
    {SF_I_SPHERE, k_shade<SF_I_SPHERE, SH_MIN_WAVES_NARROW>, k_shade<SF_I_SPHERE, SH_MIN_WAVES_NARROW, true>},
    {SF_I_MESH, k_shade<SF_I_MESH, SH_MIN_WAVES_NARROW>, k_shade<SF_I_MESH, SH_MIN_WAVES_NARROW, true>},
    {SF_ALL, k_shade<SF_ALL, SH_MIN_WAVES>, k_shade<SF_ALL, SH_MIN_WAVES, true>},
    {SF_ALL | SF_TEXTURE, k_shade<SF_ALL | SF_TEXTURE, SH_MIN_WAVES>, k_shade<SF_ALL | SF_TEXTURE, SH_MIN_WAVES, true>},
    {SF_I_MAPS, k_shade<SF_I_MAPS, SH_MIN_WAVES_MAPS>, k_shade<SF_I_MAPS, SH_MIN_WAVES_MAPS, true>}};
static const ShadeSpecInst SHADE_SPEC_INST[] = {
    {SF_I_SPHERE, k_shade_spec<SF_I_SPHERE>}, {SF_I_MESH, k_shade_spec<SF_I_MESH>}, {SF_ALL, k_shade_spec<SF_ALL>}};
template <class T, size_t N>
static const T &pick_shade_inst(const T (&tab)[N], const tirt_ctx *c)
{
    size_t k = 0;
    if (!c->shade_specialize) while (k + 1 < N && tab[k].feat != SF_ALL) k++;
    for (; k + 1 < N; k++) if ((c->shade_features & ~tab[k].feat) == 0u) return tab[k];
    return tab[N - 1];
}

[[maybe_unused]] constexpr int KAT_STEP_IN = 23, KAT_STEP_OUT = 28;
template <unsigned FEAT, int MIN_WAVES>
__global__ __launch_bounds__(SH_BLOCK, MIN_WAVES) void k_kat_shade_step(SceneView sc, const float *in, int in_stride, float *out, int out_stride, int n)
{
    const int i = blockIdx.x * blockDim.x + threadIdx.x;
    if (i >= n) return;
    const float *a = in + (size_t)i * in_stride;
    float *o = out + (size_t)i * out_stride;
    const TileMap tm = {0, 1, 0x7fffffff, 1, 0, 0};
    v3 radiance = V(a[18], a[19], a[20]);
    ShadeStep ss;
    shade_path<FEAT>(sc, tm, 0x7fffffff, (uint32_t)__float_as_int(a[2]), (uint32_t)__float_as_int(a[0]), __float_as_int(a[3]), __float_as_int(a[4]) != 0, __float_as_int(a[1]),
                     V(a[5], a[6], a[7]), V(a[8], a[9], a[10]), make_float4(a[11], a[12], a[13], a[14]), V(a[15], a[16], a[17]), radiance, a[21], __float_as_int(a[22]), ss);
    o[0] = radiance.x; o[1] = radiance.y; o[2] = radiance.z; o[3] = __int_as_float(ss.shaded ? 1 : 0); o[4] = __int_as_float(ss.want_next ? 1 : 0);
    o[5] = ss.next_o.x; o[6] = ss.next_o.y; o[7] = ss.next_o.z; o[8] = ss.next_d.x; o[9] = ss.next_d.y; o[10] = ss.next_d.z;
    o[11] = ss.next_thr.x; o[12] = ss.next_thr.y; o[13] = ss.next_thr.z; o[14] = ss.next_pdf; o[15] = __int_as_float(ss.next_spec); o[16] = __int_as_float(ss.want_shadow ? 1 : 0);
    o[17] = ss.sh_o.x; o[18] = ss.sh_o.y; o[19] = ss.sh_o.z; o[20] = ss.sh_d.x; o[21] = ss.sh_d.y; o[22] = ss.sh_d.z;
    o[23] = ss.sh_c.x; o[24] = ss.sh_c.y; o[25] = ss.sh_c.z; o[26] = __int_as_float(ss.sh_expect); o[27] = ss.sh_dist;
}
typedef void (*kat_step_fn_t)(SceneView, const float *, int, float *, int, int);
struct KatStepInst { unsigned feat; kat_step_fn_t fn; };
static const KatStepInst KAT_STEP_INST[] = {
    {SF_I_SPHERE, k_kat_shade_step<SF_I_SPHERE, SH_MIN_WAVES_NARROW>}, {SF_I_MESH, k_kat_shade_step<SF_I_MESH, SH_MIN_WAVES_NARROW>},
    {SF_ALL, k_kat_shade_step<SF_ALL, SH_MIN_WAVES>}, {SF_ALL | SF_TEXTURE, k_kat_shade_step<SF_ALL | SF_TEXTURE, SH_MIN_WAVES>},
    {SF_I_MAPS, k_kat_shade_step<SF_I_MAPS, SH_MIN_WAVES_MAPS>}};
static_assert(sizeof(KAT_STEP_INST) / sizeof(KAT_STEP_INST[0]) == sizeof(SHADE_INST) / sizeof(SHADE_INST[0]), "one known-answer kernel per instantiation of k_shade");

static kat_step_fn_t kat_step_inst(unsigned feat)
{
    for (const KatStepInst &k : KAT_STEP_INST) if (k.feat == feat) return k.fn;
    return nullptr;
}
bool kat_shade_step_has_inst(unsigned feat) { return kat_step_inst(feat) != nullptr; }
int kat_shade_step(tirt_ctx *c, unsigned feat, const float *in, int in_stride, float *out, int out_stride, int n)
{
    TIRT_REQUIRE(c->n >= 1, "tirt_kat_shade_step: no scene");
    TIRT_REQUIRE((c->shade_features & ~feat) == 0u, "tirt_kat_shade_step: feat does not cover the scene's feature word (tirt_shade_features)");
    const kat_step_fn_t fn = kat_step_inst(feat);
    TIRT_REQUIRE(fn, "tirt_kat_shade_step: feat is not an instantiation of k_shade");
    TIRT_REQUIRE(!(feat & (SF_TEXTURE | SF_TEXTURE_PARAM)) || c->tex_count > 0, "tirt_kat_shade_step: the textured instantiation needs uploaded textures (tirt_texture_upload): without them no material row's slot is checked");
    for (int i = 0; i < n; i++) {
        const float *a = in + (size_t)i * in_stride;
        const int32_t *w = (const int32_t *)a; const int32_t prim = w[14], pixel = w[1];
        TIRT_REQUIRE(!(a[11] < INF_VALUE) || (prim >= 0 && prim < c->n), "tirt_kat_shade_step: row " + std::to_string(i) + ": prim outside [0, n_prims) of a hit (t < INF)");
        TIRT_REQUIRE(pixel >= 0 && pixel < 0x7fffffff, "tirt_kat_shade_step: row " + std::to_string(i) + ": pixel outside [0, 2^31 - 1)");
    }
    if (n == 0) return TIRT_OK;
    if (sync_all(c)) return TIRT_ERR_HIP;
    if (ensure_shade_records(c)) return TIRT_ERR_HIP;
    DevBuf din, dout;
    int rc = TIRT_OK;
    const size_t in_bytes = sizeof(float) * (size_t)n * in_stride, out_bytes = sizeof(float) * (size_t)n * out_stride;
    if (din.ensure(in_bytes) || dout.ensure(out_bytes)) rc = TIRT_ERR_HIP;
    if (rc == TIRT_OK) {
        hipError_t e = hipMemcpyAsync(din.p, in, in_bytes, hipMemcpyHostToDevice, c->stream);
        if (e == hipSuccess) e = hipMemsetAsync(dout.p, 0, out_bytes, c->stream);
        if (e == hipSuccess) {
            hipLaunchKernelGGL(fn, dim3((n + SH_BLOCK - 1) / SH_BLOCK), dim3(SH_BLOCK), 0, c->stream, scene_view(c), din.as<float>(), in_stride, dout.as<float>(), out_stride, n);
            e = hipGetLastError();
        }
        if (e == hipSuccess) e = hipMemcpyAsync(out, dout.p, out_bytes, hipMemcpyDeviceToHost, c->stream);
        if (e == hipSuccess) e = hipStreamSynchronize(c->stream);
        if (e != hipSuccess) { set_error(std::string("tirt_kat_shade_step: ") + hipGetErrorString(e)); rc = TIRT_ERR_HIP; }
    }
    din.release(); dout.release();
    return rc;
}

__global__ void k_film_spec(PathState ps, const float *fw, SpecView sp, TileMap tm, int P, int F, uint32_t frame_begin, uint32_t seed, float *hdr)
{
    int k = blockIdx.x * blockDim.x + threadIdx.x;
    if (k >= P) return;
    const int p = local_to_pixel(tm, k);
    float *px = hdr + (size_t)p * 3;
    float r = px[0], g = px[1], b = px[2];
    for (int f = 0; f < F; f++) {
        const int s = frame_pixel_to_slot(tm, P, f, k);
        const uint32_t frame = frame_begin + (uint32_t)f;
        const float coff = 1.0f / ((float)(int)frame + 1.0f);
        const float Lambda = HERO_LAMBDA_MIN + HERO_LAMBDA_STEP * tm_rand(seed, (uint32_t)p, frame, TM_DIM_SPEC_LAMBDA);
        f4s spec; spec.v[0] = ps.fr[s]; spec.v[1] = ps.fg[s]; spec.v[2] = ps.fb[s]; spec.v[3] = fw[s];
        spec_add_splat(sp, spec, Lambda, coff, r, g, b);
    }
    px[0] = r; px[1] = g; px[2] = b;
}

constexpr size_t LINE = 128;
static size_t lane_counter_bytes(int max_depth)
{ return LINE * (size_t)(max_depth + 1) + sizeof(int) * TR_FETCH_STRIDE * TR_FETCH_LINES * (size_t)(max_depth + 1); }

constexpr int PATH_WORDS = 2 * 15 + 4 + 12 + 3 + 2;
static size_t path_state_bytes(size_t S) { return sizeof(float) * PATH_WORDS * ((S + 3) & ~(size_t)3); }
static int ensure_paths(Lane &L, size_t S, int max_depth)
{
    if (S > L.path_capacity || !L.path_mem.p) {
        if (L.path_mem.ensure(path_state_bytes(S))) return TIRT_ERR_HIP;
        const size_t S_user = S;
        S = (S + 3) & ~(size_t)3;
        float *w = L.path_mem.as<float>();
        PathState &p = L.ps;
        auto nxt = [&]() { float *r = w; w += S; return r; };
        for (int k = 0; k < 2; k++) {
            PathSoA &q = p.st[k];
            q.ox = nxt(); q.oy = nxt(); q.oz = nxt(); q.dx = nxt(); q.dy = nxt(); q.dz = nxt();
            q.tr = nxt(); q.tg = nxt(); q.tb = nxt(); q.rr = nxt(); q.rg = nxt(); q.rb = nxt();
            q.brdf_pdf = nxt(); q.flags = (uint32_t *)nxt(); q.slot = (int *)nxt();
        }
        p.hit = (float4 *)w; w += 4 * S;
        p.sox = nxt(); p.soy = nxt(); p.soz = nxt(); p.sdx = nxt(); p.sdy = nxt(); p.sdz = nxt();
        p.scr = nxt(); p.scg = nxt(); p.scb = nxt(); p.sprim = (int *)nxt(); p.sdist = nxt(); p.sdst = (int *)nxt();
        p.fr = nxt(); p.fg = nxt(); p.fb = nxt();
        p.scw = nxt(); p.fw = nxt();
        L.path_capacity = S_user;
    }
    if (L.counters_mem.ensure(lane_counter_bytes(max_depth))) return TIRT_ERR_HIP;
    return 0;
}

int pt_render(tirt_ctx *c, uint32_t frame_begin, int frame_count, uint32_t seed, int max_depth, int stack_size, int flags, const SpecView *spec)
{
    TIRT_REQUIRE(c->built, "tirt_pt_rgb_render: LBVH not built");
    TIRT_REQUIRE(c->cam_set, "tirt_pt_rgb_render: camera not set");
    TIRT_REQUIRE(c->hdr.p && c->npix_local >= 0, "tirt_pt_rgb_render: film not created");
    TIRT_REQUIRE(frame_count >= 0 && max_depth >= 1 && max_depth <= 4096, "tirt_pt_rgb_render: bad frame_count/max_depth");
    const bool list = c->pixset_n >= 0;
    TIRT_REQUIRE(!(list && spec), "tirt_pt_spec_render: a pixel set is installed (PT_RGB only): tirt_pixel_set_clear first");
    if (frame_count == 0 || c->npix_local == 0 || c->pixset_n == 0) return TIRT_OK;
    if (ensure_counters(c)) return TIRT_ERR_HIP;
    if (ensure_shade_records(c)) return TIRT_ERR_HIP;
    const int P = render_pixels(c);
    const size_t batch_paths = effective_batch_paths(c), merge_paths = effective_merge_paths(c);
    int FB;
    { size_t nb = ((size_t)frame_count * P + batch_paths / 2) / batch_paths; if (nb < 1) nb = 1; FB = (int)((frame_count + nb - 1) / nb); }
    if (c->split_lone >= 2 && c->tile_count >= 6 && c->batches_since_sync == 0 && FB == frame_count && frame_count >= 2 && c->n_lanes >= 2 &&
        !c->time_kernels && (size_t)frame_count * P >= ((size_t)12 << 20))
        { int parts = c->split_lone < c->n_lanes ? c->split_lone : c->n_lanes; if (parts > frame_count) parts = frame_count; FB = (frame_count + parts - 1) / parts; }
    const SceneView sv = scene_view(c);
    const BvhView bv = bvh_view(c);
    TileMap tm = render_tile_map(c);
    DevCounters *ctr = c->dev_counters.as<DevCounters>();
    const int B = 256;
    bool beams_ready = false;
    if (!list && c->primary_beams && FB >= c->primary_beams_min_frames && !(flags & TIRT_TRAVERSE_EXHAUSTIVE)) {
        if (int rc = pvb_prepare(c)) return rc;
        beams_ready = c->pvb_valid;
    }
    TIRT_HIP(hipEventRecord(c->ev_main, c->stream));
    int n_lanes = c->time_kernels ? 1 : c->n_lanes;
    { const int need = plan_batches(c).lanes + 1; if (need < n_lanes) n_lanes = need; }

    int spill_depth = 0;
    size_t cap = (size_t)FB * P;
    if (merge_paths > 0 && P >= 65536) {
        size_t want = batch_paths + batch_paths / 2;
        if (c->job_frames > 0 && want > (size_t)c->job_frames * P) want = (size_t)c->job_frames * P;
        want = (want / P) * P;
        if (want > cap) cap = want;
    }
    for (int k = 0; k < n_lanes; k++) {
        if (k > 0 && cap > c->lanes[k].path_capacity) {
            size_t free_b = 0, total_b = 0;
            if (hipMemGetInfo(&free_b, &total_b) == hipSuccess && free_b < path_state_bytes(cap) + ((size_t)2 << 30)) { n_lanes = k; break; }
        }
        if (ensure_paths(c->lanes[k], cap, max_depth)) return TIRT_ERR_HIP;
        if (ensure_spill(c, c->lanes[k].spill, stack_size, spill_depth)) return TIRT_ERR_HIP;
    }

    for (int fb = 0; fb < frame_count; fb += FB) {
        Lane &L = c->lanes[n_lanes == 1 ? 0 : (c->lane_cursor++ % (unsigned)n_lanes)];
        c->batches_since_sync++;
        hipStream_t st = L.stream;
        const int F = (frame_count - fb < FB) ? frame_count - fb : FB;
        const int S = F * P;
        tm.F = (c->path_order_blocks && (P & 63) == 0) ? F : 0;
        const bool use_beams = beams_ready && F >= c->primary_beams_min_frames;
        const uint32_t f0 = frame_begin + (uint32_t)fb;
        char *cm = L.counters_mem.as<char>();
        auto append_ctr = [&](int b) { return (unsigned long long *)(cm + LINE * (size_t)b); };
        auto cnt_path = [&](int b) { return (const int *)append_ctr(b - 1); };
        auto cnt_shadow = [&](int b) { return (const int *)append_ctr(b) + 1; };
        auto fetch = [&](int launch) { return (int *)(cm + LINE * (size_t)(max_depth + 1)) + (size_t)launch * TR_FETCH_STRIDE * TR_FETCH_LINES; };

        TIRT_HIP(hipStreamWaitEvent(st, c->ev_main, 0));
        hipEvent_t r0, r1;
        TIRT_HIP(hipEventCreate(&r0)); TIRT_HIP(hipEventCreate(&r1));
        TIRT_HIP(hipEventRecord(r0, st));
        std::vector<std::pair<hipEvent_t, hipEvent_t>> evc, evs, evh;
        auto stamp = [&](std::vector<std::pair<hipEvent_t, hipEvent_t>> &v, bool begin) {
            if (!c->time_kernels) return;
            if (begin) { hipEvent_t a, b; (void)hipEventCreate(&a); (void)hipEventCreate(&b); v.push_back({a, b}); (void)hipEventRecord(a, st); }
            else (void)hipEventRecord(v.back().second, st);
        };

        TIRT_HIP(hipMemsetAsync(L.counters_mem.p, 0, lane_counter_bytes(max_depth), st));
        hipLaunchKernelGGL(list ? k_generate<true> : k_generate<false>, dim3((S + B - 1) / B), dim3(B), 0, st, L.ps.st[0], c->cam, tm, P, S, f0, seed, ctr);
        bool busy = false;
        if (c->last_film) { busy = hipEventQuery(c->last_film) == hipErrorNotReady; (void)hipGetLastError(); }
        const BatchPlan plan = plan_batches(c);
        const bool two_big = plan.lanes <= 2 && plan.batch >= ((size_t)24 << 20) && !c->grid_user;
        const int grid_cap = (busy && n_lanes > 1 && !two_big) ? c->tr_grid : c->tr_grid_alone;
        int grid_full = (S + TR_BLOCK - 1) / TR_BLOCK; if (grid_full > grid_cap) grid_full = grid_cap;
        const int sh_cap = two_big ? 2 * c->sh_grid : c->sh_grid;
        int grid_shade = (S + SH_BLOCK - 1) / SH_BLOCK; if (grid_shade > sh_cap) grid_shade = sh_cap;
        v3 eye_v; eye_v.x = c->cam.eye[0]; eye_v.y = c->cam.eye[1]; eye_v.z = c->cam.eye[2];
        const shade_fn_t shade_fn = list ? pick_shade_inst(SHADE_INST, c).fn_list : pick_shade_inst(SHADE_INST, c).fn;
        const shade_spec_fn_t shade_spec_fn = pick_shade_inst(SHADE_SPEC_INST, c).fn;
        for (int b = 0; b < max_depth; b++) {
            const PathSoA &in = L.ps.st[b & 1], &out = L.ps.st[(b + 1) & 1];
            TraceArgs a = {};
            a.bvh = bv;
            a.ox = in.ox; a.oy = in.oy; a.oz = in.oz; a.dx = in.dx; a.dy = in.dy; a.dz = in.dz;
            if (b == 0) { a.ox = a.oy = a.oz = nullptr; for (int k = 0; k < 3; k++) a.eye[k] = c->cam.eye[k]; }
            a.count_ptr = (b == 0) ? nullptr : cnt_path(b); a.count_fixed = S;
            a.hit = L.ps.hit;
            a.spill = L.spill.as<int>(); a.spill_depth = spill_depth; a.ctr = ctr; a.per_ray_counts = nullptr;
            a.fetch = fetch(b);
            a.sox = L.ps.sox; a.soy = L.ps.soy; a.soz = L.ps.soz; a.sdx = L.ps.sdx; a.sdy = L.ps.sdy; a.sdz = L.ps.sdz;
            a.sprim = L.ps.sprim; a.sdst = L.ps.sdst; a.sdist = L.ps.sdist; a.scr = L.ps.scr; a.scg = L.ps.scg; a.scb = L.ps.scb;
            a.rr = in.rr; a.rg = in.rg; a.rb = in.rb; a.fr = L.ps.fr; a.fg = L.ps.fg; a.fb = L.ps.fb;
            if (spec) { a.scw = L.ps.scw; a.rw = (float *)in.flags; a.fw = L.ps.fw; }
            a.scount_ptr = (b == 0) ? nullptr : cnt_shadow(b - 1);
            fill_tunables(c, a);
            a.timeline = timeline_for(c, flags, grid_full);
            if (!(b == 0 && use_beams)) stamp(evc, true);
            if (b == 0 && use_beams) {
                int *const fb_count = (int *)append_ctr(0) + 4;
                float4 *const fb_hit = (float4 *)L.ps.sox;
                pvb_launch_cand(c, st, bv, in.dx, in.dy, in.dz, tm, P, S, L.ps.hit, fb_count, (int *)out.ox, out.dx, out.dy, out.dz, ctr);
                TraceArgs a2 = a;
                a2.dx = out.dx; a2.dy = out.dy; a2.dz = out.dz; a2.count_ptr = fb_count; a2.count_fixed = S; a2.hit = fb_hit; a2.no_ray_count = 1;
                stamp(evc, true);
                if (int rc = launch_trace<KIND_CLOSEST>(c, st, a2, flags, grid_full)) return rc;
                stamp(evc, false);
                pvb_launch_scatter(st, fb_count, (const int *)out.ox, fb_hit, L.ps.hit);
            } else
            if (int rc = (b == 0) ? launch_trace<KIND_CLOSEST>(c, st, a, flags, grid_full) : launch_trace<KIND_MIXED>(c, st, a, flags, grid_full)) return rc;
            if (!(b == 0 && use_beams)) stamp(evc, false);
            c->launches_trace_closest++;
            if (b == 0 && c->aov.p) { if (int rc = aov_launch(c, L, tm, P, F, f0)) return rc; }

            stamp(evh, true);
            if (spec)
                hipLaunchKernelGGL(shade_spec_fn, dim3(grid_shade), dim3(SH_BLOCK), 0, st, ShadeArgs{L.ps, in, out}, sv, *spec, tm, P, f0, seed, b,
                                   (b == max_depth - 1) ? 1 : 0, (b == 0) ? (const int *)nullptr : cnt_path(b), S,
                                   append_ctr(b), ctr, eye_v);
            else
            hipLaunchKernelGGL(shade_fn, dim3(grid_shade), dim3(SH_BLOCK), 0, st, ShadeArgs{L.ps, in, out}, sv, tm, P, f0, seed, b,
                               (b == max_depth - 1) ? 1 : 0, (b == 0) ? (const int *)nullptr : cnt_path(b), S,
                               append_ctr(b), ctr, eye_v);
            stamp(evh, false);
            c->launches_shade++;

            if (b == max_depth - 1) {
                TraceArgs sa = {};
                sa.bvh = bv;
                sa.ox = L.ps.sox; sa.oy = L.ps.soy; sa.oz = L.ps.soz; sa.dx = L.ps.sdx; sa.dy = L.ps.sdy; sa.dz = L.ps.sdz;
                sa.count_ptr = cnt_shadow(b); sa.count_fixed = 0;
                sa.sprim = L.ps.sprim; sa.sdst = L.ps.sdst; sa.sdist = L.ps.sdist; sa.scr = L.ps.scr; sa.scg = L.ps.scg; sa.scb = L.ps.scb;
                sa.rr = out.rr; sa.rg = out.rg; sa.rb = out.rb; sa.fr = L.ps.fr; sa.fg = L.ps.fg; sa.fb = L.ps.fb;
                if (spec) { sa.scw = L.ps.scw; sa.rw = (float *)out.flags; sa.fw = L.ps.fw; }
                sa.spill = L.spill.as<int>(); sa.spill_depth = spill_depth; sa.ctr = ctr; sa.per_ray_counts = nullptr;
                sa.fetch = fetch(max_depth);
                fill_tunables(c, sa);
                stamp(evs, true);
                if (int rc = launch_trace<KIND_SHADOW_ACC>(c, st, sa, flags, grid_full)) return rc;
                stamp(evs, false);
                c->launches_trace_shadow++;
            }
        }
        if (c->last_film) TIRT_HIP(hipStreamWaitEvent(st, c->last_film, 0));
        if (spec) hipLaunchKernelGGL(k_film_spec, dim3((P + B - 1) / B), dim3(B), 0, st, L.ps, L.ps.fw, *spec, tm, P, F, f0, seed, c->hdr.as<float>());
        else hipLaunchKernelGGL(list ? k_film<true> : k_film<false>, dim3((P + B - 1) / B), dim3(B), 0, st, L.ps, tm, P, F, f0, c->hdr.as<float>());
        if (c->mom.p && !spec) { if (int rc = moments_launch(c, L, tm, P, F)) return rc; }
        TIRT_HIP(hipEventRecord(L.film_done, st));
        L.film_recorded = true;
        c->last_film = L.film_done;
        if (use_beams) c->pvb_set[c->pvb_cur].busy = L.film_done;
        TIRT_HIP(hipEventRecord(r1, st));
        if (c->time_kernels) {
            TIRT_HIP(hipStreamSynchronize(st));
            auto drain = [&](std::vector<std::pair<hipEvent_t, hipEvent_t>> &v, double &acc) {
                for (auto &pr : v) { float ms = 0; (void)hipEventElapsedTime(&ms, pr.first, pr.second); acc += ms; (void)hipEventDestroy(pr.first); (void)hipEventDestroy(pr.second); }
                v.clear();
            };
            drain(evc, c->ms_trace_closest); drain(evs, c->ms_trace_shadow); drain(evh, c->ms_shade);
        }
        c->ev_pool.push_back({r0, r1});
        if (c->ev_pool.size() > 64) {
            size_t keep = 0;
            for (auto &pr : c->ev_pool) {
                if (hipEventQuery(pr.second) == hipSuccess) {
                    float ms = 0.0f;
                    if (hipEventElapsedTime(&ms, pr.first, pr.second) == hipSuccess) c->ms_render += ms;
                    (void)hipEventDestroy(pr.first); (void)hipEventDestroy(pr.second);
                } else c->ev_pool[keep++] = pr;
            }
            c->ev_pool.resize(keep);
            (void)hipGetLastError();
        }
    }
    TIRT_HIP(hipGetLastError());
    return TIRT_OK;
}

}
```

Measured before the change: 5652.

## Carry per-path RNG key in path state and pack specular flag into slot

Splits the RNG hash so the per-pixel/frame prefix is computed once in generate and stored as a key in the path SoA. The shade kernel then reads the key and no longer recomputes the slot-to-pixel mapping or the three-step hash per sample. The specular flag is packed into the slot's high bit, which drops the separate flags load and store. A uniform-map generate variant computes the blocked tile mapping with scalar (readfirstlane) math. In exchange each path carries an extra word of state and the path buffer grows.

```diff
diff --git a/ti_raytrace_amd/csrc/tirt_api.hip b/ti_raytrace_amd/csrc/tirt_api.hip
--- a/ti_raytrace_amd/csrc/tirt_api.hip
+++ b/ti_raytrace_amd/csrc/tirt_api.hip
@@ -640,6 +640,7 @@
     if (!strcmp(name, "shade_specialize")) { TIRT_REQUIRE(value == 0.0 || value == 1.0, "shade_specialize: 0 (generic kernel) or 1"); if (flush_pending(c)) return TIRT_ERR_HIP; c->shade_specialize = (int)value; return TIRT_OK; }
     if (!strcmp(name, "shade_grid")) { TIRT_REQUIRE(value >= 1 && value <= 65536, "shade_grid: 1..65536"); c->sh_grid = (int)value; c->grid_user = true; return TIRT_OK; }
     if (!strcmp(name, "path_order_blocks")) { c->path_order_blocks = value != 0.0; return TIRT_OK; }
+    if (!strcmp(name, "generate_uniform_map")) { TIRT_REQUIRE(value == 0.0 || value == 1.0, "generate_uniform_map: 0 or 1"); c->generate_uniform_map = (int)value; return TIRT_OK; }
     if (!strcmp(name, "slices_contiguous")) { c->slices_contiguous = value != 0.0; return TIRT_OK; }
     if (!strcmp(name, "trace_grid_alone")) { TIRT_REQUIRE(value >= 1 && value <= 16384, "trace_grid_alone: 1..16384"); c->tr_grid_alone = (int)value; return TIRT_OK; }
     if (!strcmp(name, "query_chunk_rays")) {
diff --git a/ti_raytrace_amd/csrc/tirt_internal.h b/ti_raytrace_amd/csrc/tirt_internal.h
--- a/ti_raytrace_amd/csrc/tirt_internal.h
+++ b/ti_raytrace_amd/csrc/tirt_internal.h
@@ -137,6 +137,7 @@
     float *rr, *rg, *rb;
     float *brdf_pdf; uint32_t *flags;
     int *slot;
+    uint32_t *key;
 };
 struct PathState {
     PathSoA st[2];
@@ -257,6 +258,7 @@
     struct { bool valid = false; uint32_t begin = 0; int count = 0; uint32_t seed = 0; int max_depth = 0, stack_size = 0, flags = 0; bool spectral = false; } pend;
     int tr_lds_depth = 16, tr_refill_min = 18, tr_node_min = 38, tr_grid = 1280, tr_slice_log2 = 5, sh_grid = 1024;
     int path_order_blocks = 1, slices_contiguous = 0;
+    int generate_uniform_map = 1;
     int tr_grid_alone = 1280;
     tirt::DevBuf counters_mem, spill;
     int cu_count = 256;
diff --git a/ti_raytrace_amd/csrc/tirt_math.h b/ti_raytrace_amd/csrc/tirt_math.h
--- a/ti_raytrace_amd/csrc/tirt_math.h
+++ b/ti_raytrace_amd/csrc/tirt_math.h
@@ -237,17 +237,28 @@
     x ^= x >> 16;
     return x;
 }
-TM_HD uint32_t tm_rand_u32(uint32_t seed, uint32_t pixel, uint32_t frame, uint32_t dim)
+TM_HD uint32_t tm_rand_key(uint32_t seed, uint32_t pixel, uint32_t frame)
 {
     uint32_t h = tm_mix32(seed ^ 0x9e3779b9u);
     h = tm_mix32(h ^ pixel);
     h = tm_mix32(h + frame * 0x85ebca6bu + 0x68bc21ebu);
-    h = tm_mix32(h ^ (dim * 0xc2b2ae35u + 0x02e5be93u));
     return h;
 }
+TM_HD uint32_t tm_rand_key_u32(uint32_t key, uint32_t dim)
+{
+    return tm_mix32(key ^ (dim * 0xc2b2ae35u + 0x02e5be93u));
+}
+TM_HD float tm_rand_k(uint32_t key, uint32_t dim)
+{
+    return (float)(tm_rand_key_u32(key, dim) >> 8) * 5.9604644775390625e-08f;
+}
+TM_HD uint32_t tm_rand_u32(uint32_t seed, uint32_t pixel, uint32_t frame, uint32_t dim)
+{
+    return tm_rand_key_u32(tm_rand_key(seed, pixel, frame), dim);
+}
 TM_HD float tm_rand(uint32_t seed, uint32_t pixel, uint32_t frame, uint32_t dim)
 {
-    return (float)(tm_rand_u32(seed, pixel, frame, dim) >> 8) * 5.9604644775390625e-08f;
+    return tm_rand_k(tm_rand_key(seed, pixel, frame), dim);
 }
 
 #endif
diff --git a/ti_raytrace_amd/csrc/tirt_render.hip b/ti_raytrace_amd/csrc/tirt_render.hip
--- a/ti_raytrace_amd/csrc/tirt_render.hip
+++ b/ti_raytrace_amd/csrc/tirt_render.hip
@@ -36,13 +36,10 @@
     v3 next_o = V(0.0f, 0.0f, 0.0f), next_d = next_o, next_thr = next_o, sh_o = next_o, sh_d = next_o, sh_c = next_o;
     float next_pdf = 0.0f, sh_dist = 0.0f; int next_spec = 0, sh_expect = -2;
 };
-template <unsigned FEAT, bool LIST = false>
-TD void shade_path(const SceneView &sc, const TileMap &tm, int P, uint32_t frame_begin, uint32_t seed, int bounce, int last_bounce, int slot,
+template <unsigned FEAT>
+TD void shade_path(const SceneView &sc, uint32_t key, int bounce, int last_bounce,
                    const v3 origin, const v3 direction, const float4 hrec, v3 throughout, v3 &radiance, float brdf_pdf, int perfect_spec, ShadeStep &s)
 {
-    int f, k; slot_to_frame_pixel(tm, P, slot, f, k);
-    const uint32_t pixel = (uint32_t)mapped_pixel<LIST>(tm, k);
-    const uint32_t frame = frame_begin + (uint32_t)f;
     const uint32_t dim0 = TM_DIM_BOUNCE0 + TM_DIMS_PER_BOUNCE * (uint32_t)bounce;
     const float t = hrec.x;
     if (t < INF_VALUE) {
@@ -76,7 +73,7 @@
             v3 next_dir; float f_or_b = 1.0f, brdf = 1.0f;
             if ((FEAT & SF_GLASS) && mat_type == MAT_GLASS) {
                 perfect_spec = 1;
-                next_dir = glass_sample(m, direction, normal, tm_rand(seed, pixel, frame, dim0 + TM_SLOT_GLASS), f_or_b);
+                next_dir = glass_sample(m, direction, normal, tm_rand_k(key, dim0 + TM_SLOT_GLASS), f_or_b);
                 brdf = 1.0f; brdf_pdf = 1.0f;
             } else {
                 perfect_spec = 0;
@@ -93,10 +90,10 @@
                 DisneySetup ds;
                 if (SHARE_SETUP) ds = disney_setup(md, fnormal, -direction);
                 if (!(FEAT & SF_NO_LIGHT) || sc.light_count > 0) {
-                int lidx = (int)(tm_rand(seed, pixel, frame, dim0 + TM_SLOT_LIGHT) * (float)sc.light_count);
+                int lidx = (int)(tm_rand_k(key, dim0 + TM_SLOT_LIGHT) * (float)sc.light_count);
                 if (lidx >= sc.light_count) lidx = sc.light_count - 1;
-                const float ra = tm_rand(seed, pixel, frame, dim0 + TM_SLOT_LA);
-                const float rb = tm_rand(seed, pixel, frame, dim0 + TM_SLOT_LB);
+                const float ra = tm_rand_k(key, dim0 + TM_SLOT_LA);
+                const float rb = tm_rand_k(key, dim0 + TM_SLOT_LB);
                 v3 light_pos, light_normal;
                 const LightRec lr = light_sample_rec<FEAT>(sc.light_rec, lidx, ra, rb, light_pos, light_normal);
                 const float light_choice_pdf = lr.choice_pdf;
@@ -127,8 +124,8 @@
                     s.sh_o = light_pos; s.sh_d = light_dir; s.sh_c = c; s.sh_expect = expect; s.sh_dist = light_dist;
                 }
                 }
-                const float r_lobe = tm_rand(seed, pixel, frame, dim0 + TM_SLOT_LOBE), r_1 = tm_rand(seed, pixel, frame, dim0 + TM_SLOT_R1),
-                            r_2 = tm_rand(seed, pixel, frame, dim0 + TM_SLOT_R2);
+                const float r_lobe = tm_rand_k(key, dim0 + TM_SLOT_LOBE), r_1 = tm_rand_k(key, dim0 + TM_SLOT_R1),
+                            r_2 = tm_rand_k(key, dim0 + TM_SLOT_R2);
                 next_dir = SHARE_SETUP ? disney_sample_set(ds, direction, fnormal, r_lobe, r_1, r_2) : disney_sample(md, direction, fnormal, r_lobe, r_1, r_2);
                 f_or_b = 1.0f;
                 brdf = SHARE_SETUP ? disney_evaluate_pdf_set(ds, fnormal, -direction, next_dir, brdf_pdf)
@@ -141,7 +138,7 @@
                 if ((FEAT & SF_GLASS) && f_or_b < 0.0f) {
                     const float extinction = m[6];
                     const float R = tm_exp(-t / extinction);
-                    if (tm_rand(seed, pixel, frame, dim0 + TM_SLOT_EXT) >= R) alive = false;
+                    if (tm_rand_k(key, dim0 + TM_SLOT_EXT) >= R) alive = false;
                 }
                 if (alive) {
                     throughout = throughout * (reflect_color * (brdf / brdf_pdf));
@@ -688,23 +685,38 @@
     return launch_trace<KIND_QUERY>(c, st, a, j.flags, grid);
 }
 
-template <bool LIST>
+template <bool LIST, bool UNIFORM = false>
 __global__ void k_generate(PathSoA ps, CameraView cam, TileMap tm, int P, int S, uint32_t frame_begin, uint32_t seed,
                            DevCounters *ctr)
 {
     int s = blockIdx.x * blockDim.x + threadIdx.x;
     if (s >= S) return;
-    int f, k; slot_to_frame_pixel(tm, P, s, f, k);
-    int p = mapped_pixel<LIST>(tm, k);
-    int i = p / tm.H, j = p - i * tm.H;
+    int f, p, i, j;
+    if constexpr (UNIFORM) {
+        const int c = __builtin_amdgcn_readfirstlane(s >> 6), l = s & 63;
+        int kb;
+        if (tm.F > 0) { kb = c / tm.F; f = c - kb * tm.F; }
+        else { const int cpf = P >> 6; f = c / cpf; kb = c - f * cpf; }
+        const int bpt = tm.tile_size >> 6, rows = tm.H >> 3;
+        const int lt = kb / bpt, b = kb - lt * bpt, bc = b / rows, bj = b - bc * rows;
+        i = (lt * tm.tile_count + tm.tile_rank) * (tm.tile_size / tm.H) + (bc << 3) + (l >> 3);
+        j = (bj << 3) + (l & 7);
+        p = i * tm.H + j;
+    } else {
+        int k; slot_to_frame_pixel(tm, P, s, f, k);
+        p = mapped_pixel<LIST>(tm, k);
+        i = p / tm.H; j = p - i * tm.H;
+    }
     uint32_t frame = frame_begin + (uint32_t)f;
+    const uint32_t key = tm_rand_key(seed, (uint32_t)p, frame);
     float jx = 0.0f, jy = 0.0f;
     if (frame != 0) {
-        jx = tm_rand(seed, (uint32_t)p, frame, TM_DIM_JX) - 0.5f;
-        jy = tm_rand(seed, (uint32_t)p, frame, TM_DIM_JY) - 0.5f;
+        jx = tm_rand_k(key, TM_DIM_JX) - 0.5f;
+        jy = tm_rand_k(key, TM_DIM_JY) - 0.5f;
     }
     v3 d = camera_ray_direction(cam, i, j, jx, jy);
     __builtin_nontemporal_store(d.x, &ps.dx[s]); __builtin_nontemporal_store(d.y, &ps.dy[s]); __builtin_nontemporal_store(d.z, &ps.dz[s]);
+    __builtin_nontemporal_store(key, &ps.key[s]);
     if (s == 0) atomicAdd(&ctr->paths, (unsigned long long)S);
 }
 
@@ -725,9 +737,8 @@
 #define SH_COLD(ca) cold_shade_t ca = (cold_shade_t)__builtin_amdgcn_kernarg_segment_ptr(); asm volatile("" : "+s"(ca))
 #define SH_LD(x) __builtin_nontemporal_load(&(x))
 #define SH_ST(x, v) __builtin_nontemporal_store((v), &(x))
-template <unsigned FEAT, int MIN_WAVES, bool LIST = false>
-__global__ __launch_bounds__(SH_BLOCK, MIN_WAVES) void k_shade(ShadeArgs paths_in_kernarg_segment, SceneView sc, TileMap tm, int P,
-                                                   uint32_t frame_begin, uint32_t seed, int bounce, int last_bounce,
+template <unsigned FEAT, int MIN_WAVES>
+__global__ __launch_bounds__(SH_BLOCK, MIN_WAVES) void k_shade(ShadeArgs paths_in_kernarg_segment, SceneView sc, int bounce, int last_bounce,
                                                    const int *count_ptr, int count_fixed, unsigned long long *append_ctr,
                                                    DevCounters *ctr, v3 eye)
 {
@@ -742,20 +753,22 @@
     for (int it = 0; it < rounds; it++) {
         const int q = it * total + blockIdx.x * blockDim.x + threadIdx.x;
         bool live = q < count, want_next = false, want_shadow = false;
-        int slot = 0;
+        int slot = 0; uint32_t key = 0u;
         v3 radiance = V(0.0f, 0.0f, 0.0f), next_o = radiance, next_d = radiance, next_thr = radiance;
         v3 sh_o = radiance, sh_d = radiance, sh_c = radiance;
         float next_pdf = 0.0f, sh_dist = 0.0f; int next_spec = 0, sh_expect = -2;
         if (live) {
             const bool first = bounce == 0;
             SH_COLD(ca);
-            const int *const c_slot = ca->in.slot; const uint32_t *const c_flags = ca->in.flags; const float4 *const c_hit = ca->ps.hit;
+            const uint32_t *const c_slot = (const uint32_t *)ca->in.slot; const float4 *const c_hit = ca->ps.hit;
             const float *const c_ox = ca->in.ox, *const c_oy = ca->in.oy, *const c_oz = ca->in.oz, *const c_dx = ca->in.dx, *const c_dy = ca->in.dy, *const c_dz = ca->in.dz;
             const float *const c_tr = ca->in.tr, *const c_tg = ca->in.tg, *const c_tb = ca->in.tb, *const c_rr = ca->in.rr, *const c_rg = ca->in.rg, *const c_rb = ca->in.rb;
-            const float *const c_pdf = ca->in.brdf_pdf;
-            asm volatile("" :: "s"(c_slot), "s"(c_flags), "s"(c_hit), "s"(c_ox), "s"(c_oy), "s"(c_oz), "s"(c_dx), "s"(c_dy), "s"(c_dz), "s"(c_tr), "s"(c_tg), "s"(c_tb),
-                         "s"(c_rr), "s"(c_rg), "s"(c_rb), "s"(c_pdf));
-            slot = first ? q : SH_LD(c_slot[q]);
+            const float *const c_pdf = ca->in.brdf_pdf; const uint32_t *const c_key = ca->in.key;
+            asm volatile("" :: "s"(c_slot), "s"(c_hit), "s"(c_ox), "s"(c_oy), "s"(c_oz), "s"(c_dx), "s"(c_dy), "s"(c_dz), "s"(c_tr), "s"(c_tg), "s"(c_tb),
+                         "s"(c_rr), "s"(c_rg), "s"(c_rb), "s"(c_pdf), "s"(c_key));
+            const uint32_t slot_spec = first ? ((uint32_t)q | 0x80000000u) : SH_LD(c_slot[q]);
+            slot = (int)(slot_spec & 0x7fffffffu);
+            key = SH_LD(c_key[q]);
             const v3 origin = first ? eye : V(SH_LD(c_ox[q]), SH_LD(c_oy[q]), SH_LD(c_oz[q]));
             const v3 direction = V(SH_LD(c_dx[q]), SH_LD(c_dy[q]), SH_LD(c_dz[q]));
             typedef float f4nt__ __attribute__((ext_vector_type(4)));
@@ -764,9 +777,9 @@
             v3 throughout = first ? V(1.0f, 1.0f, 1.0f) : V(SH_LD(c_tr[q]), SH_LD(c_tg[q]), SH_LD(c_tb[q]));
             radiance = first ? V(0.0f, 0.0f, 0.0f) : V(SH_LD(c_rr[q]), SH_LD(c_rg[q]), SH_LD(c_rb[q]));
             float brdf_pdf = first ? 1.0f : SH_LD(c_pdf[q]);
-            int perfect_spec = first ? 1 : (int)(SH_LD(c_flags[q]) & 1u);
+            int perfect_spec = (int)(slot_spec >> 31);
             ShadeStep ss;
-            shade_path<FEAT, LIST>(sc, tm, P, frame_begin, seed, bounce, last_bounce, slot, origin, direction, hrec, throughout, radiance, brdf_pdf, perfect_spec, ss);
+            shade_path<FEAT>(sc, key, bounce, last_bounce, origin, direction, hrec, throughout, radiance, brdf_pdf, perfect_spec, ss);
             want_next = ss.want_next; want_shadow = ss.want_shadow; if (ss.shaded) n_shaded++;
             next_o = ss.next_o; next_d = ss.next_d; next_thr = ss.next_thr; next_pdf = ss.next_pdf; next_spec = ss.next_spec;
             sh_o = ss.sh_o; sh_d = ss.sh_d; sh_c = ss.sh_c; sh_expect = ss.sh_expect; sh_dist = ss.sh_dist;
@@ -792,14 +805,14 @@
             SH_COLD(ca);
             float *const o_ox = ca->out.ox, *const o_oy = ca->out.oy, *const o_oz = ca->out.oz, *const o_dx = ca->out.dx, *const o_dy = ca->out.dy, *const o_dz = ca->out.dz;
             float *const o_tr = ca->out.tr, *const o_tg = ca->out.tg, *const o_tb = ca->out.tb, *const o_rr = ca->out.rr, *const o_rg = ca->out.rg, *const o_rb = ca->out.rb;
-            float *const o_pdf = ca->out.brdf_pdf; uint32_t *const o_flags = ca->out.flags; int *const o_slot = ca->out.slot;
+            float *const o_pdf = ca->out.brdf_pdf; uint32_t *const o_key = ca->out.key, *const o_slot = (uint32_t *)ca->out.slot;
             asm volatile("" :: "s"(o_ox), "s"(o_oy), "s"(o_oz), "s"(o_dx), "s"(o_dy), "s"(o_dz), "s"(o_tr), "s"(o_tg), "s"(o_tb), "s"(o_rr), "s"(o_rg), "s"(o_rb),
-                         "s"(o_pdf), "s"(o_flags), "s"(o_slot));
+                         "s"(o_pdf), "s"(o_slot), "s"(o_key));
             SH_ST(o_ox[qn], next_o.x); SH_ST(o_oy[qn], next_o.y); SH_ST(o_oz[qn], next_o.z);
             SH_ST(o_dx[qn], next_d.x); SH_ST(o_dy[qn], next_d.y); SH_ST(o_dz[qn], next_d.z);
             SH_ST(o_tr[qn], next_thr.x); SH_ST(o_tg[qn], next_thr.y); SH_ST(o_tb[qn], next_thr.z);
             SH_ST(o_rr[qn], radiance.x); SH_ST(o_rg[qn], radiance.y); SH_ST(o_rb[qn], radiance.z);
-            SH_ST(o_pdf[qn], next_pdf); SH_ST(o_flags[qn], (uint32_t)next_spec); SH_ST(o_slot[qn], slot);
+            SH_ST(o_pdf[qn], next_pdf); SH_ST(o_slot[qn], (uint32_t)slot | ((uint32_t)next_spec << 31)); SH_ST(o_key[qn], key);
         } else if (live) {
             SH_COLD(ca);
             float *const f_r = ca->ps.fr, *const f_g = ca->ps.fg, *const f_b = ca->ps.fb;
@@ -1031,19 +1044,19 @@
     if (threadIdx.x == 0 && s_shaded) atomicAdd(&ctr->shaded, s_shaded);
 }
 
-typedef void (*shade_fn_t)(ShadeArgs, SceneView, TileMap, int, uint32_t, uint32_t, int, int, const int *, int, unsigned long long *, DevCounters *, v3);
+typedef void (*shade_fn_t)(ShadeArgs, SceneView, int, int, const int *, int, unsigned long long *, DevCounters *, v3);
 typedef void (*shade_spec_fn_t)(ShadeArgs, SceneView, SpecView, TileMap, int, uint32_t, uint32_t, int, int, const int *, int, unsigned long long *, DevCounters *, v3);
-struct ShadeInst { unsigned feat; shade_fn_t fn, fn_list; };
+struct ShadeInst { unsigned feat; shade_fn_t fn; };
 struct ShadeSpecInst { unsigned feat; shade_spec_fn_t fn; };
 constexpr unsigned SF_I_SPHERE = SF_LIGHT_SPHERE;
 constexpr unsigned SF_I_MESH = SF_LIGHT_TRI;
 constexpr unsigned SF_I_MAPS = SF_ALL | SF_TEXTURE | SF_TEXTURE_PARAM;
 static const ShadeInst SHADE_INST[] = {
-    {SF_I_SPHERE, k_shade<SF_I_SPHERE, SH_MIN_WAVES_NARROW>, k_shade<SF_I_SPHERE, SH_MIN_WAVES_NARROW, true>},
-    {SF_I_MESH, k_shade<SF_I_MESH, SH_MIN_WAVES_NARROW>, k_shade<SF_I_MESH, SH_MIN_WAVES_NARROW, true>},
-    {SF_ALL, k_shade<SF_ALL, SH_MIN_WAVES>, k_shade<SF_ALL, SH_MIN_WAVES, true>},
-    {SF_ALL | SF_TEXTURE, k_shade<SF_ALL | SF_TEXTURE, SH_MIN_WAVES>, k_shade<SF_ALL | SF_TEXTURE, SH_MIN_WAVES, true>},
-    {SF_I_MAPS, k_shade<SF_I_MAPS, SH_MIN_WAVES_MAPS>, k_shade<SF_I_MAPS, SH_MIN_WAVES_MAPS, true>}};
+    {SF_I_SPHERE, k_shade<SF_I_SPHERE, SH_MIN_WAVES_NARROW>},
+    {SF_I_MESH, k_shade<SF_I_MESH, SH_MIN_WAVES_NARROW>},
+    {SF_ALL, k_shade<SF_ALL, SH_MIN_WAVES>},
+    {SF_ALL | SF_TEXTURE, k_shade<SF_ALL | SF_TEXTURE, SH_MIN_WAVES>},
+    {SF_I_MAPS, k_shade<SF_I_MAPS, SH_MIN_WAVES_MAPS>}};
 static const ShadeSpecInst SHADE_SPEC_INST[] = {
     {SF_I_SPHERE, k_shade_spec<SF_I_SPHERE>}, {SF_I_MESH, k_shade_spec<SF_I_MESH>}, {SF_ALL, k_shade_spec<SF_ALL>}};
 template <class T, size_t N>
@@ -1063,10 +1076,10 @@
     if (i >= n) return;
     const float *a = in + (size_t)i * in_stride;
     float *o = out + (size_t)i * out_stride;
-    const TileMap tm = {0, 1, 0x7fffffff, 1, 0, 0};
+    const uint32_t key = tm_rand_key((uint32_t)__float_as_int(a[0]), (uint32_t)__float_as_int(a[1]), (uint32_t)__float_as_int(a[2]));
     v3 radiance = V(a[18], a[19], a[20]);
     ShadeStep ss;
-    shade_path<FEAT>(sc, tm, 0x7fffffff, (uint32_t)__float_as_int(a[2]), (uint32_t)__float_as_int(a[0]), __float_as_int(a[3]), __float_as_int(a[4]) != 0, __float_as_int(a[1]),
+    shade_path<FEAT>(sc, key, __float_as_int(a[3]), __float_as_int(a[4]) != 0,
                      V(a[5], a[6], a[7]), V(a[8], a[9], a[10]), make_float4(a[11], a[12], a[13], a[14]), V(a[15], a[16], a[17]), radiance, a[21], __float_as_int(a[22]), ss);
     o[0] = radiance.x; o[1] = radiance.y; o[2] = radiance.z; o[3] = __int_as_float(ss.shaded ? 1 : 0); o[4] = __int_as_float(ss.want_next ? 1 : 0);
     o[5] = ss.next_o.x; o[6] = ss.next_o.y; o[7] = ss.next_o.z; o[8] = ss.next_d.x; o[9] = ss.next_d.y; o[10] = ss.next_d.z;
@@ -1145,7 +1158,7 @@
 static size_t lane_counter_bytes(int max_depth)
 { return LINE * (size_t)(max_depth + 1) + sizeof(int) * TR_FETCH_STRIDE * TR_FETCH_LINES * (size_t)(max_depth + 1); }
 
-constexpr int PATH_WORDS = 2 * 15 + 4 + 12 + 3 + 2;
+constexpr int PATH_WORDS = 2 * 16 + 4 + 12 + 3 + 2;
 static size_t path_state_bytes(size_t S) { return sizeof(float) * PATH_WORDS * ((S + 3) & ~(size_t)3); }
 static int ensure_paths(Lane &L, size_t S, int max_depth)
 {
@@ -1160,7 +1173,7 @@
             PathSoA &q = p.st[k];
             q.ox = nxt(); q.oy = nxt(); q.oz = nxt(); q.dx = nxt(); q.dy = nxt(); q.dz = nxt();
             q.tr = nxt(); q.tg = nxt(); q.tb = nxt(); q.rr = nxt(); q.rg = nxt(); q.rb = nxt();
-            q.brdf_pdf = nxt(); q.flags = (uint32_t *)nxt(); q.slot = (int *)nxt();
+            q.brdf_pdf = nxt(); q.flags = (uint32_t *)nxt(); q.slot = (int *)nxt(); q.key = (uint32_t *)nxt();
         }
         p.hit = (float4 *)w; w += 4 * S;
         p.sox = nxt(); p.soy = nxt(); p.soz = nxt(); p.sdx = nxt(); p.sdy = nxt(); p.sdz = nxt();
@@ -1249,7 +1262,9 @@
         };
 
         TIRT_HIP(hipMemsetAsync(L.counters_mem.p, 0, lane_counter_bytes(max_depth), st));
-        hipLaunchKernelGGL(list ? k_generate<true> : k_generate<false>, dim3((S + B - 1) / B), dim3(B), 0, st, L.ps.st[0], c->cam, tm, P, S, f0, seed, ctr);
+        const bool uniform_map = !list && c->generate_uniform_map && tm.blocked && (P & 63) == 0;
+        hipLaunchKernelGGL(list ? k_generate<true> : (uniform_map ? k_generate<false, true> : k_generate<false>), dim3((S + B - 1) / B), dim3(B), 0, st, L.ps.st[0], c->cam, tm, P, S,
+                           f0, seed, ctr);
         bool busy = false;
         if (c->last_film) { busy = hipEventQuery(c->last_film) == hipErrorNotReady; (void)hipGetLastError(); }
         const BatchPlan plan = plan_batches(c);
@@ -1259,7 +1274,7 @@
         const int sh_cap = two_big ? 2 * c->sh_grid : c->sh_grid;
         int grid_shade = (S + SH_BLOCK - 1) / SH_BLOCK; if (grid_shade > sh_cap) grid_shade = sh_cap;
         v3 eye_v; eye_v.x = c->cam.eye[0]; eye_v.y = c->cam.eye[1]; eye_v.z = c->cam.eye[2];
-        const shade_fn_t shade_fn = list ? pick_shade_inst(SHADE_INST, c).fn_list : pick_shade_inst(SHADE_INST, c).fn;
+        const shade_fn_t shade_fn = pick_shade_inst(SHADE_INST, c).fn;
         const shade_spec_fn_t shade_spec_fn = pick_shade_inst(SHADE_SPEC_INST, c).fn;
         for (int b = 0; b < max_depth; b++) {
             const PathSoA &in = L.ps.st[b & 1], &out = L.ps.st[(b + 1) & 1];
@@ -1301,7 +1316,7 @@
                                    (b == max_depth - 1) ? 1 : 0, (b == 0) ? (const int *)nullptr : cnt_path(b), S,
                                    append_ctr(b), ctr, eye_v);
             else
-            hipLaunchKernelGGL(shade_fn, dim3(grid_shade), dim3(SH_BLOCK), 0, st, ShadeArgs{L.ps, in, out}, sv, tm, P, f0, seed, b,
+            hipLaunchKernelGGL(shade_fn, dim3(grid_shade), dim3(SH_BLOCK), 0, st, ShadeArgs{L.ps, in, out}, sv, b,
                                (b == max_depth - 1) ? 1 : 0, (b == 0) ? (const int *)nullptr : cnt_path(b), S,
                                append_ctr(b), ctr, eye_v);
             stamp(evh, false);
```

Result: no change. 5658, median of 3 (+0.1%).
